# nyu-systems/Grendel-GS

Hardware: AMD Instinct MI355X
Metric: training iters/sec (fwd+bwd) (higher is better)
Workload: dtype f32

## Files before the change

### grendel-gs_amd/csrc/binning.hip

```cpp
#include "common.h"

#include <atomic>
#include <chrono>
#include <cstdlib>
#include <cstring>
#include <mutex>

#include "radix.h"
#ifndef GSR_EMIT_DECODE_BATCH
#define GSR_EMIT_DECODE_BATCH 2
#endif
#include "binning_persist.h"
#include "binning_rows.h"
#include "binning_host.h"

namespace {

__global__ void __launch_bounds__(SCAN_THREADS)
scan_gather_lookback_kernel(const uint32_t *__restrict__ src, int packed,
                            const uint32_t *__restrict__ idx, uint32_t *__restrict__ out, uint32_t *__restrict__ out2,
                            long long n, unsigned long long *__restrict__ state, uint32_t *__restrict__ ticket, int nb,
                            uint32_t *__restrict__ host_total, uint32_t seq,
                            const unsigned long long *__restrict__ early) {
    __shared__ uint32_t smem[4];
    __shared__ uint32_t s_bid;
    __shared__ unsigned long long s_excl;
    if (threadIdx.x == 0) s_bid = atomicAdd(ticket, 1u);
    __syncthreads();
    const uint32_t bid = s_bid;
    const int lane = threadIdx.x & 63, wave = threadIdx.x >> 6;
    const long long base = (long long)bid * SCAN_TILE + (long long)threadIdx.x * SCAN_ITEMS;
    uint32_t v[SCAN_ITEMS], v2[SCAN_ITEMS];
    uint32_t s = 0, s2 = 0;
#pragma unroll
    for (int k = 0; k < SCAN_ITEMS; k++) {
        const uint32_t x = (base + k < n) ? src[idx[base + k]] : 0u;
        v[k] = packed ? (x & TT_MASK) : x;
        v2[k] = packed ? (x >> TT_SHIFT) : 0u;
        s += v[k];
        s2 += v2[k];
    }
    uint32_t tot, tot2;
    const uint32_t local = block_exclusive_scan(s, smem, &tot);
    const uint32_t local2 = block_exclusive_scan(s2, smem, &tot2);
    const unsigned long long tot64 = (unsigned long long)tot | ((unsigned long long)tot2 << 31);
    if (wave == 0) {
        if (lane == 0) st_agent64(&state[bid], tot64 | (bid == 0 ? LB64_PRE : LB64_AGG));
        unsigned long long excl = 0;
        if (bid > 0) {
            long long top = (long long)bid - 1;
            while (true) {
                const long long j = top - lane;
                unsigned long long x = j >= 0 ? ld_agent64(&state[j]) : LB64_PRE;
// ... 369 lines not shown
                       tile_hist ? 1 : 0, sorted_ids, v.offsets, v.segoff, (long long)P,
                       reinterpret_cast<unsigned long long *>(v.ctrl + L.C.scan_state),
                       reinterpret_cast<uint32_t *>(v.ctrl + L.C.tickets), nbs, (uint32_t *)nullptr, seq, v.early);
    GSR_LAUNCH_CHECK();
    *ticket = seq;
    return 0;
}

int prepare_persistent(const PrepCall &c, const BinFrame &f, const BinHooks &h, BinDevice &d, uint32_t *ticket) {
    if (!(persist_effective_mode() & PERSIST_P) || g_tie_order.load(std::memory_order_relaxed) != 0) return 1;
    persist_caps(d);
    const int grid_p = lowered(h.grid_p, d.grid_p);
    long long nb = radix_blocks(c.P);
    int items = 4;
    if (nb > grid_p && (nb + 1) / 2 <= grid_p) {
        items = 8;
        nb = (nb + 1) / 2;
    }
    const int G = (int)(nb < grid_p ? nb : grid_p);
    if (G <= 0 || nb > (long long)G * h.max_tpw) return 1;
    const long long admit = persist_admit(d, c.stream);
    if (admit < 0) return 1;
    const int P = c.P;
    const PrepLayout L = prep_layout(P);
    const PrepViews v = views(L, c.prep);
    const PersistLayoutP PL = persist_layout_p(G);
    GSR_HIP(hipMemsetAsync(v.early, 0, (L.ctrl - L.early) + PL.zero_bytes, c.stream));
    uint32_t *host_total = nullptr;
    uint32_t seq = 0;
    const int rc = take_ticket(d, &host_total, &seq);
    if (rc) return rc;
    PrepPersistArgs a{};
    a.P = P; a.gx = f.gx; a.gy = f.gy;
    a.means2D = reinterpret_cast<const float2 *>(c.means2D);
    a.conic_opacity = reinterpret_cast<const float4 *>(c.conic_opacity);
    a.depths = c.depths; a.radii = c.radii; a.mask = c.compute_locally;
    a.tt = v.tt; a.kA = v.kA; a.vA = v.vA; a.kB = v.kB; a.vB = v.vB;
    a.offsets = v.offsets; a.segoff = v.segoff; a.rects = v.rects;
    a.tile_hist = f.yx ? v.thist : nullptr;
    a.cull = f.cull;
    a.hull_out = v.hull;
    a.early = v.early;
    a.zero16 = reinterpret_cast<uint4 *>(c.zero_ptr);
    a.zero16_n = c.zero_bytes / 16;
    a.sync = sync_view(v.ctrl + PL.sync, G);
    a.tstamp = timeline_buffer(h.timeline, 0, G);
    a.grp = at<uint32_t>(v.ctrl, PL.grp); a.cnt = at<uint32_t>(v.ctrl, PL.cnt);
    a.wtot = at<unsigned long long>(v.ctrl, PL.wtot); a.bins = at<uint32_t>(v.ctrl, PL.bins);
    a.depth_buckets = h.depth_buckets ? 1 : 0;
    a.host_total = host_total; a.seq = seq;
    a.done_word = d.done; a.done_seq = (uint32_t)admit;
    a.timeout_ticks = 5000000ull;
    a.force_abort = h.abort_p ? 1 : 0;
    if (items == 4) hipLaunchKernelGGL(bin_prepare_persist_kernel<4>, dim3(G), dim3(PP_THREADS), 0, c.stream, a);
    else hipLaunchKernelGGL(bin_prepare_persist_kernel<8>, dim3(G), dim3(PP_THREADS), 0, c.stream, a);
    GSR_LAUNCH_CHECK();
    *ticket = seq;
    return 0;
}

struct SortCall {
    BinFrame f;
    int P;
    const uint8_t *mask;
    PrepViews pv;
    int64_t D;
    void *scratch;
    uint32_t *point_list;
    int32_t *ranges;
    hipStream_t stream;
    bool bounded;
};

int launch_rows(const SortCall &s, const BinHooks &h, const BinDevice &d) {
    const BinFrame &f = s.f;
    const int P = s.P, gx = f.gx, gy = f.gy;
    const long long D = s.D;
    const RowsLayout R = rows_layout(D, gx, gy);
    auto u32 = [&s](size_t off) { return at<uint32_t>(s.scratch, off); };
    uint32_t *tickets = u32(R.tickets), *seg_key = u32(R.seg_key), *seg_gid = u32(R.seg_gid), *pairoff = u32(R.pairoff);
    uint32_t *tilebase = u32(R.tilebase);
    int32_t *tdiff = at<int32_t>(s.scratch, R.tdiff), *chunk_owner = at<int32_t>(s.scratch, R.chunk_owner);
    int cus = 256;
    (void)hipDeviceGetAttribute(&cus, hipDeviceAttributeMultiprocessorCount, (int)(&d - g_bin_devices));
    const uint32_t *thist = s.pv.thist, *segoff = s.pv.segoff, *offsets = s.pv.offsets;
    constexpr int TILE_B = 8 * ROWS_THREADS_B, TILE_D = 8 * ROWS_THREADS_D;
    auto tickets_of = [](long long tiles) { return (tiles + TICKET_TILES - 1) / TICKET_TILES; };
    const long long nbB = (D + TILE_B - 1) / TILE_B;
    const int fill_b = cus * 2, fill_d = cus * h.rows_fill_d;
    const int grid_b = (int)(tickets_of(nbB) < fill_b ? tickets_of(nbB) : fill_b);
    const long long nbs = (D + SEGSCAN_TILE - 1) / SEGSCAN_TILE;
    const int grid_c = (int)(tickets_of(nbs) < cus * 2 ? tickets_of(nbs) : cus * 2);
    const long long nbt = (D + TILE_D - 1) / TILE_D + gy;
    const int grid_d = (int)(tickets_of(nbt) < fill_d ? tickets_of(nbt) : fill_d);
    hipLaunchKernelGGL((seg_scatter_kernel<8, ROWS_THREADS_B>), dim3(grid_b), dim3(ROWS_THREADS_B), 0, s.stream, P, D,
                       f.ybits, s.pv.rects, s.pv.vA, offsets, segoff, thist + 2 * RADIX_DIGITS, u32(R.seg_state), tickets,
                       seg_key, seg_gid, s.bounded, s.ranges, 2 * gx * gy, s.pv.hull, tdiff,
                       RADIX_REPLICAS * gy * (gx + 1));
    hipLaunchKernelGGL(seg_scan_kernel, dim3(grid_c), dim3(SCAN_THREADS), 0, s.stream, P, D, gx, gy, offsets, segoff,
                       seg_key, pairoff, at<unsigned long long>(s.scratch, R.scan_state), tickets + 1, tdiff, thist,
                       chunk_owner, s.bounded);
    hipLaunchKernelGGL(tile_base_kernel, dim3(gy), dim3(GSR_ONE_DIM_BLOCK), 0, s.stream, P, D, gx, gy, offsets, thist,
                       tdiff, s.mask, tilebase, reinterpret_cast<int2 *>(s.ranges), s.bounded);
    hipLaunchKernelGGL((pair_scatter_kernel<8, ROWS_THREADS_D>), dim3(grid_d), dim3(ROWS_THREADS_D), 0, s.stream, P, D, gx,
                       gy, f.xbits, offsets, segoff, seg_key, seg_gid, pairoff, thist, tilebase, chunk_owner, u32(R.pair_state),
                       tickets + 2, s.point_list, s.bounded);
    GSR_LAUNCH_CHECK();
    return 0;
// ... 147 lines not shown
    if (!d->total_word) return GSR_EINVAL;
    uint32_t total = 0;
    rc = wait_total(reinterpret_cast<hipStream_t>(stream_), slot_of_ticket(*d, ticket), ticket, &total);
    if (rc) return rc;
    if (total == PAIRS_ABORTED) {
        PrepCall c = d->calls[ticket % TOTAL_SLOTS];
        if (!c.persistent) return GSR_EINVAL;
        c.persistent = false;
        uint32_t again = 0;
        rc = prepare_lookback(c, bin_frame(c.width, c.height), *d, &again);
        if (rc) return rc;
        rc = wait_total(c.stream, slot_of_ticket(*d, again), again, &total);
        if (rc) return rc;
        *num_rendered_host = (int64_t)total;
        return GSR_ERETRY;
    }
    *num_rendered_host = (int64_t)total;
    return 0;
}

extern "C" int gsr_bin_prepare(int P, int width, int height, const float *means2D, const float *depths,
                               const int32_t *radii, const float *conic_opacity, const uint8_t *compute_locally,
                               void *prep, size_t prep_bytes, int64_t *num_rendered_host, gsr_stream_t stream_) {
    if (!num_rendered_host) return GSR_EINVAL;
    *num_rendered_host = 0;
    uint32_t ticket = 0;
    const int rc = gsr_bin_prepare_async(P, width, height, means2D, depths, radii, conic_opacity, compute_locally, prep,
                                         prep_bytes, &ticket, stream_);
    if (rc) return rc;
    const int rw = gsr_bin_count_wait(ticket, num_rendered_host, stream_);
    return rw == GSR_ERETRY ? 0 : rw;
}

extern "C" int gsr_bin_sort(int P, int width, int height, const uint8_t *compute_locally, const void *prep,
                            int64_t D, void *scratch, size_t scratch_bytes, uint32_t *point_list, int32_t *ranges,
                            gsr_stream_t stream_) {
    return bin_sort_impl(P, width, height, compute_locally, prep, D, scratch, scratch_bytes, point_list, ranges,
                         reinterpret_cast<hipStream_t>(stream_), false);
}

extern "C" int gsr_bin_sort_bounded(int P, int width, int height, const uint8_t *compute_locally, const void *prep,
                                    int64_t capacity, void *scratch, size_t scratch_bytes, uint32_t *point_list,
                                    int32_t *ranges, gsr_stream_t stream_) {
    if (capacity <= 0) return GSR_EINVAL;
    return bin_sort_impl(P, width, height, compute_locally, prep, capacity, scratch, scratch_bytes, point_list, ranges,
                         reinterpret_cast<hipStream_t>(stream_), true);
}

extern "C" int gsr_bin_speculative_async(int P, int width, int height, const float *means2D, const float *depths,
                                         const int32_t *radii, const float *conic_opacity,
                                         const uint8_t *compute_locally, void *prep, size_t prep_bytes,
                                         int64_t capacity, void *scratch, size_t scratch_bytes, uint32_t *point_list,
                                         int32_t *ranges, uint32_t *ticket, int *sorted, gsr_stream_t stream_) {
    if (!ticket || !sorted) return GSR_EINVAL;
    *sorted = 0;
    if (P < 0 || width <= 0 || height <= 0) return GSR_EINVAL;
    *ticket = 0;
    if (P == 0) return 0;
    if (!means2D || !depths || !radii || !conic_opacity || !compute_locally || !prep) return GSR_EINVAL;
    if (P > RADIX_MAX_N) return GSR_EINVAL;
    if (prep_bytes < prep_bytes_needed(P)) return GSR_ENOSPACE;
    const BinFrame f = bin_frame(width, height);
    if (f.gx > 0xFFFF || f.gy > 0xFFFF) return GSR_EINVAL;
    BinDevice *d = nullptr;
    int rc = bin_device(&d);
    if (!rc) rc = persist_fault_check(*d);
    if (rc) return rc;
    const BinHooks h = read_hooks();
    hipStream_t stream = reinterpret_cast<hipStream_t>(stream_);
    const bool sort = capacity > 0 && scratch && point_list;
    const SortPlan p = sort ? plan_sort(f, capacity, scratch_bytes, true, h.rows_min) : SortPlan{GSR_EINVAL};
    PrepCall c{P, width, height, means2D, depths, radii, conic_opacity, compute_locally, prep, stream, true, nullptr, 0};
    if (!p.err) {
        c.zero_ptr = reinterpret_cast<char *>(scratch) + p.zero_off;
        c.zero_bytes = p.zero_bytes;
    }
    rc = prepare_persistent(c, f, h, *d, ticket);
    if (rc == 1) {
        c.persistent = false;
        rc = prepare_lookback(c, f, *d, ticket);
    }
    if (rc) return rc;
    d->calls[*ticket % TOTAL_SLOTS] = c;
    d->calls[*ticket % TOTAL_SLOTS].zero_ptr = nullptr;
    d->calls[*ticket % TOTAL_SLOTS].zero_bytes = 0;
    if (!sort) return 0;
    if (!ranges) return GSR_EINVAL;
    if (!f.yx) GSR_HIP(hipMemsetAsync(ranges, 0, sizeof(int32_t) * 2 * ((size_t)f.gx * f.gy + 1), stream));
    if (p.err) return p.err;
    rc = sort_run({f, P, compute_locally, views(prep_layout(P), prep), capacity, scratch, point_list, ranges, stream, true},
                  h, *d, p.form);
    if (rc) return rc;
    *sorted = 1;
    return 0;
}

extern "C" int gsr_bin_prepare_async(int P, int width, int height, const float *means2D, const float *depths,
                                     const int32_t *radii, const float *conic_opacity, const uint8_t *compute_locally,
                                     void *prep, size_t prep_bytes, uint32_t *ticket, gsr_stream_t stream_) {
    int sorted = 0;
    return gsr_bin_speculative_async(P, width, height, means2D, depths, radii, conic_opacity, compute_locally, prep,
                                     prep_bytes, 0, nullptr, 0, nullptr, nullptr, ticket, &sorted, stream_);
}

extern "C" int gsr_set_depth_tie_order(int mode) {
    if (mode != 0 && mode != 1) return GSR_EINVAL;
    g_tie_order.store(mode, std::memory_order_relaxed);
    return 0;
}

extern "C" int gsr_set_tile_cull(int mode) {
    if (mode < -1 || mode > 2) return GSR_EINVAL;
    g_tile_cull.store(mode, std::memory_order_relaxed);
    return 0;
}

extern "C" int gsr_set_bin_rowmajor(int mode) {
    if (mode < -1 || mode > 1) return GSR_EINVAL;
    g_rows_override.store(mode, std::memory_order_relaxed);
    return 0;
}

extern "C" int gsr_set_bin_persistent(int mode) {
    if (mode < -1 || mode > 3) return GSR_EINVAL;
    g_persist_override.store(mode, std::memory_order_relaxed);
    std::lock_guard<std::mutex> guard(g_bin_mutex);
    for (BinDevice &d : g_bin_devices) {
        if (!d.done) continue;
        d.solo_seen = reinterpret_cast<volatile uint32_t *>(d.done)[3];
        d.backoff = 0;
    }
    return 0;
}

extern "C" int gsr_bin_persist_status(uint32_t *out4) {
    if (!out4) return GSR_EINVAL;
    BinDevice *d = nullptr;
    const int rc = bin_device(&d);
    if (rc && rc != GSR_EINVAL) return rc;
    out4[0] = out4[1] = out4[2] = out4[3] = 0;
    if (rc || !d->done) return 0;
    const volatile uint32_t *w = d->done;
    out4[0] = w[0]; out4[1] = w[1]; out4[2] = w[2]; out4[3] = w[3];
    return 0;
}

// ... 24 lines not shown
```

### grendel-gs_amd/csrc/binning_host.h

```cpp
#pragma once

namespace {

enum { PERSIST_OFF = 0, PERSIST_P = 1, PERSIST_S = 2 };
constexpr long long PERSIST_SORT_MAX_PAIRS = 6ll << 20;
constexpr long long ROWS_MIN_PAIRS = 5ll << 20;

std::atomic<int> g_persist_override{-1};
std::atomic<int> g_rows_override{-1};
std::atomic<int> g_tile_cull{-1};
std::atomic<int> g_tie_order{0};

int persist_effective_mode() {
    const int o = g_persist_override.load(std::memory_order_relaxed);
    if (o >= 0) return o;
    static const int env_mode = [] {
        const char *e = getenv("GSR_BIN_PERSIST");
        if (!e || !*e || strcmp(e, "1") == 0) return PERSIST_P | PERSIST_S;
        if (strcmp(e, "p") == 0) return (int)PERSIST_P;
        if (strcmp(e, "s") == 0) return (int)PERSIST_S;
        return (int)PERSIST_OFF;
    }();
    return env_mode;
}
bool rows_switch_on() {
    const int mode = g_rows_override.load(std::memory_order_relaxed);
    if (mode >= 0) return mode == 1;
    static const bool env_on = [] {
        const char *e = getenv("GSR_BIN_ROWS");
        return !(e && *e == '0');
    }();
    return env_on;
}
int tile_cull_on(int tiles) {
    int mode = g_tile_cull.load(std::memory_order_relaxed);
    if (mode < 0) {
        static const int env_mode = [] {
            const char *e = getenv("GSR_TILE_CULL");
            if (!e || !*e || strcmp(e, "0") == 0) return 0;
            return strcmp(e, "auto") == 0 ? 2 : 1;
        }();
        mode = env_mode;
    }
    if (mode != 2) return mode;
    static const int min_tiles = [] {
        const char *e = getenv("GSR_TILE_CULL_TILES");
        const int v = e ? atoi(e) : 0;
        return v > 0 ? v : 16384;
    }();
    return tiles > min_tiles ? 1 : 0;
}

int lowered(int v, int dflt) { return v > 0 && v < dflt ? v : dflt; }
int env_int(const char *name) {
    const char *e = getenv(name);
    return e && *e ? atoi(e) : 0;
}
struct BinHooks {
    long long persist_maxd;
    long long rows_min;
    int rows_fill_d;
    int max_tpw;
    int owners;
    int sort_timeout_ms;
    int grid_p, grid_s;
    bool depth_buckets;
    bool abort_p, abort_s;
    bool timeline;
};
BinHooks read_hooks() {
    BinHooks h;
    const int maxd = env_int("GSR_BIN_PERSIST_MAXD");
    h.persist_maxd = maxd > 0 && maxd < 0x7fffffff ? maxd : PERSIST_SORT_MAX_PAIRS;
    const char *e = getenv("GSR_BIN_ROWS_MIN");
    const long long rows_min = e ? atoll(e) : 0;
    h.rows_min = rows_min > 0 ? rows_min : ROWS_MIN_PAIRS;
    h.rows_fill_d = lowered(env_int("GSR_ROWS_FILL_D"), 4);
    h.max_tpw = lowered(env_int("GSR_BIN_MAX_TPW"), PP_MAX_TPW + 1);
    if (h.max_tpw > PP_MAX_TPW) h.max_tpw = 1;
    h.owners = lowered(env_int("GSR_BIN_OWNERS"), PS_OWNERS);
    h.sort_timeout_ms = lowered(env_int("GSR_BIN_SORT_TIMEOUT_MS"), 250);
    h.grid_p = env_int("GSR_BIN_GRID_P");
    h.grid_s = env_int("GSR_BIN_GRID_S");
    e = getenv("GSR_BIN_DEPTH_SORT");
    h.depth_buckets = !(e && strcmp(e, "lsd") == 0);
    e = getenv("GSR_BIN_FORCE_ABORT");
    h.abort_p = e && strchr(e, 'p') != nullptr;
    h.abort_s = e && strchr(e, 's') != nullptr;
    e = getenv("GSR_BIN_TIMELINE");
    h.timeline = e && *e == '1';
    return h;
}

int bits_for(long long n) {
    int b = 1;
    while ((1ll << b) < n) b++;
    return b;
}
int tile_bits(int tiles) { return bits_for((long long)tiles + 1); }
struct BinFrame {
    int width, height, gx, gy, tiles;
    int xbits, ybits;
    bool yx;
    int cull;
};
BinFrame bin_frame(int width, int height) {
    BinFrame f;
    f.width = width; f.height = height;
    f.gx = (width + GSR_BLOCK_X - 1) / GSR_BLOCK_X;
    f.gy = (height + GSR_BLOCK_Y - 1) / GSR_BLOCK_Y;
    f.tiles = f.gx * f.gy;
    f.xbits = bits_for(f.gx); f.ybits = bits_for(f.gy);
    const char *e = getenv("GSR_BINNING");
    f.yx = !(e && strcmp(e, "generic") == 0) && f.gx <= RADIX_DIGITS && f.gy <= RADIX_DIGITS;
    f.cull = f.yx ? tile_cull_on(f.tiles) : 0;
    return f;
}

constexpr int PERSIST_MAX_GRID_P = 1024;
constexpr int PERSIST_MAX_GRID_S = 4096;
template <class T>
T *at(void *base, size_t off) { return reinterpret_cast<T *>(reinterpret_cast<char *>(base) + off); }
GridSync sync_view(void *sync, int G) {
    uint32_t *leaf = at<uint32_t>(sync, 0), *root = leaf + (size_t)((G + GB_FAN - 1) / GB_FAN) * GB_LEAF_STRIDE;
    return {leaf, root, root + GB_LEAF_STRIDE};
}
struct PersistLayoutP {
    size_t sync, grp, bins, cnt, wtot, zero_bytes, total;
};
PersistLayoutP persist_layout_p(int G) {
    PersistLayoutP L;
    const int ngroups = (G + GB_FAN - 1) / GB_FAN;
    size_t o = 0;
    L.sync = o; o += align_up(sizeof(uint32_t) * grid_sync_words(G));
    L.grp = o; o += align_up(sizeof(uint32_t) * (BK_PASS + 1) * (size_t)ngroups * RADIX_DIGITS);
    L.bins = o; o += align_up(sizeof(uint32_t) * (BK_BINS + 2));
    L.zero_bytes = o;
    L.cnt = o; o += align_up(sizeof(uint32_t) * (BK_PASS + 1) * (size_t)G * RADIX_DIGITS);
    L.wtot = o; o += align_up(sizeof(unsigned long long) * (size_t)G);
    L.total = o;
    return L;
}
struct PersistLayoutS {
// ... 97 lines not shown
    L.C = ctrl_layout(D, passes < 2 ? 2 : passes, false);
    const size_t need = persist_layout_s(persist_grid_bound(D, PERSIST_MAX_GRID_S)).total;
    o += L.C.total > need ? L.C.total : need;
    if (f.yx) {
        const size_t rows = rows_layout(D, f.gx, f.gy).total;
        if (rows > o) o = rows;
    }
    L.total = o;
    return L;
}
struct SortViews {
    uint32_t *kA, *vA, *kB, *vB, *ghist, *tickets, *state;
    char *ctrl;
};
SortViews views(const SortLayout &L, void *b) {
    return {at<uint32_t>(b, L.kA), at<uint32_t>(b, L.vA), at<uint32_t>(b, L.kB), at<uint32_t>(b, L.vB),
            at<uint32_t>(b, L.ctrl + L.C.ghist), at<uint32_t>(b, L.ctrl + L.C.tickets),
            at<uint32_t>(b, L.ctrl + L.C.radix_state), at<char>(b, L.ctrl)};
}

enum SortForm { SORT_ROWS, SORT_YX, SORT_GENERIC };
struct SortPlan {
    int err;
    SortForm form;
    size_t zero_off, zero_bytes;
};
SortPlan plan_sort(const BinFrame &f, int64_t D, size_t scratch_bytes, bool bounded, long long rows_min) {
    if (D > RADIX_MAX_N) return {GSR_EINVAL};
    const SortLayout S = sort_layout(f, D);
    if (scratch_bytes < S.total) return {GSR_ENOSPACE};
    if (bounded && !f.yx) return {GSR_EINVAL};
    if (f.yx && !f.cull && D >= rows_min && rows_switch_on()) {
        const RowsLayout R = rows_layout(D, f.gx, f.gy);
        return {0, SORT_ROWS, R.ctrl, R.ctrl_bytes};
    }
    if (!f.yx) return {0, SORT_GENERIC, S.ctrl, S.C.total};
    const size_t zp = persist_layout_s(persist_grid_bound(D, PERSIST_MAX_GRID_S)).zero_bytes;
    return {0, SORT_YX, S.ctrl, S.C.total > zp ? S.C.total : zp};
}

constexpr int TOTAL_SLOTS = 64, MAX_DEVICES = 64;

struct PrepCall {
    int P, width, height;
    const float *means2D, *depths;
    const int32_t *radii;
    const float *conic_opacity;
    const uint8_t *compute_locally;
    void *prep;
    hipStream_t stream;
    bool persistent;
    void *zero_ptr;
    size_t zero_bytes;
};

struct BinDevice {
    uint32_t *total_word;
    bool caps_init;
    int grid_p, grid_s;
    uint32_t *done;
    uint32_t faults_seen;
    uint32_t solo_seen;
    int backoff;
    bool faulted;
    uint32_t seq;
    hipStream_t stream;
    bool any;
    PrepCall calls[TOTAL_SLOTS];
};
std::mutex g_bin_mutex;
BinDevice g_bin_devices[MAX_DEVICES];
uint32_t g_ticket_seq = 0;

int bin_device(BinDevice **out) {
    int dev = 0;
    GSR_HIP(hipGetDevice(&dev));
    if (dev < 0 || dev >= MAX_DEVICES) return GSR_EINVAL;
    *out = &g_bin_devices[dev];
    return 0;
}

void persist_caps(BinDevice &d) {
    std::lock_guard<std::mutex> guard(g_bin_mutex);
    if (d.caps_init) return;
    d.caps_init = true;
    const int dev = (int)(&d - g_bin_devices);
    int cus = 0, per_p = 0, per_p8 = 0, per_s = 0;
    if (hipDeviceGetAttribute(&cus, hipDeviceAttributeMultiprocessorCount, dev) == hipSuccess && cus > 0 &&
        hipOccupancyMaxActiveBlocksPerMultiprocessor(&per_p, bin_prepare_persist_kernel<4>, PP_THREADS, 0) == hipSuccess &&
        hipOccupancyMaxActiveBlocksPerMultiprocessor(&per_p8, bin_prepare_persist_kernel<8>, PP_THREADS, 0) == hipSuccess &&
        hipOccupancyMaxActiveBlocksPerMultiprocessor(&per_s, bin_sort_persist_kernel, PS_THREADS, 0) == hipSuccess) {
        d.grid_p = (per_p >= 1 && per_p8 >= 1) ? (cus < PERSIST_MAX_GRID_P ? cus : PERSIST_MAX_GRID_P) : 0;
        const long long gs = (long long)cus * (per_s < 4 ? per_s : 4);
        d.grid_s = per_s >= 1 ? (int)(gs < PERSIST_MAX_GRID_S ? gs : PERSIST_MAX_GRID_S) : 0;
    }
    void *p = nullptr;
    if (hipHostMalloc(&p, 64, hipHostMallocDefault) == hipSuccess) {
        memset(p, 0, 64);
        d.done = reinterpret_cast<uint32_t *>(p);
    } else {
        d.grid_p = d.grid_s = 0;
    }
    (void)hipGetLastError();
}

int take_ticket(BinDevice &d, uint32_t **host, uint32_t *seq_out) {
    std::lock_guard<std::mutex> guard(g_bin_mutex);
    if (!d.total_word) {
        void *p = nullptr;
        GSR_HIP(hipHostMalloc(&p, sizeof(uint32_t) * 2 * TOTAL_SLOTS, hipHostMallocDefault));
        memset(p, 0, sizeof(uint32_t) * 2 * TOTAL_SLOTS);
        d.total_word = reinterpret_cast<uint32_t *>(p);
    }
    const uint32_t seq = ++g_ticket_seq ? g_ticket_seq : ++g_ticket_seq;
    *seq_out = seq;
    *host = d.total_word + 2 * (seq % TOTAL_SLOTS);
    return 0;
}
uint32_t *slot_of_ticket(const BinDevice &d, uint32_t seq) { return d.total_word + 2 * (seq % TOTAL_SLOTS); }
int wait_total(hipStream_t stream, uint32_t *host_total, uint32_t seq, uint32_t *total) {
    volatile uint32_t *w = host_total;
    const auto t0 = std::chrono::steady_clock::now();
    for (long spins = 0;; spins++) {
        if (w[1] == seq) {
            std::atomic_thread_fence(std::memory_order_acquire);
            *total = w[0];
            return 0;
        }
        if ((spins & 1023) == 1023 &&
            std::chrono::steady_clock::now() - t0 > std::chrono::milliseconds(2))
            break;
    }
    GSR_HIP(hipStreamSynchronize(stream));
    *total = w[0];
    return w[1] == seq ? 0 : GSR_EINVAL;
}

long long persist_admit(BinDevice &d, hipStream_t stream) {
    hipStreamCaptureStatus cs = hipStreamCaptureStatusNone;
    if (hipStreamIsCapturing(stream, &cs) == hipSuccess && cs != hipStreamCaptureStatusNone) return 0;
    (void)hipGetLastError();
    std::lock_guard<std::mutex> guard(g_bin_mutex);
    if (d.faulted) return -1;
    if (d.any && d.stream != stream) {
        const volatile uint32_t *done = reinterpret_cast<volatile uint32_t *>(d.done);
// ... 54 lines not shown
```

### grendel-gs_amd/csrc/binning_persist.h

```cpp
#pragma once

namespace {

constexpr int TT_SHIFT = 20;
constexpr uint32_t TT_MASK = (1u << TT_SHIFT) - 1u;
constexpr uint32_t GB_ABORT = 0x80000000u;
constexpr int GB_FAN = 32;
constexpr int GB_LEAF_STRIDE = 32;
constexpr uint32_t PAIRS_ABORTED = 0xFFFFFFFFu;

struct GridSync {
    uint32_t *leaf;
    uint32_t *root;
    uint32_t *flags;
};
__host__ __device__ inline size_t grid_sync_words(int G) {
    return (size_t)(2 * ((G + GB_FAN - 1) / GB_FAN) + 1) * GB_LEAF_STRIDE;
}

__device__ __forceinline__ bool grid_barrier_try_abort(const GridSync gs, uint32_t complete) {
    uint32_t r = __hip_atomic_load(gs.root, __ATOMIC_RELAXED, __HIP_MEMORY_SCOPE_AGENT);
    while (true) {
        if (r & GB_ABORT) return true;
        if (r == complete) return false;
        if (__hip_atomic_compare_exchange_strong(gs.root, &r, r | GB_ABORT, __ATOMIC_RELAXED, __ATOMIC_RELAXED,
                                                 __HIP_MEMORY_SCOPE_AGENT))
            return true;
    }
}
__device__ __forceinline__ bool grid_barrier(const GridSync gs, uint32_t G, uint32_t &epoch, uint64_t timeout_ticks,
                                             uint32_t *s_flag, bool force_abort = false) {
    asm volatile("s_waitcnt vmcnt(0)" ::: "memory");
    __syncthreads();
    if (threadIdx.x == 0) {
        epoch++;
        const uint32_t g = blockIdx.x / GB_FAN, ngroups = (G + GB_FAN - 1) / GB_FAN;
        const uint32_t gsz = min((uint32_t)GB_FAN, G - g * GB_FAN);
        const uint32_t complete = epoch * ngroups;
        if (force_abort && grid_barrier_try_abort(gs, complete))
            for (uint32_t k = 0; k < ngroups; k++) st_agent(&gs.flags[k * GB_LEAF_STRIDE], 0xFFFFFFFFu);
        const uint32_t old =
            __hip_atomic_fetch_add(&gs.leaf[g * GB_LEAF_STRIDE], 1u, __ATOMIC_RELAXED, __HIP_MEMORY_SCOPE_AGENT);
        if (old + 1u == epoch * gsz) {
            const uint32_t r = __hip_atomic_fetch_add(gs.root, 1u, __ATOMIC_RELAXED, __HIP_MEMORY_SCOPE_AGENT);
            if ((r & ~GB_ABORT) + 1u == complete)
                for (uint32_t k = 0; k < ngroups; k++)
                    st_agent(&gs.flags[k * GB_LEAF_STRIDE], (r & GB_ABORT) ? 0xFFFFFFFFu : epoch);
        }
        uint64_t t0 = __builtin_amdgcn_s_memrealtime();
        uint32_t f;
        while ((f = ld_agent(&gs.flags[g * GB_LEAF_STRIDE])) < epoch) {
            __builtin_amdgcn_s_sleep(1);
            if (__builtin_amdgcn_s_memrealtime() - t0 > timeout_ticks) {
                if (grid_barrier_try_abort(gs, complete)) {
                    for (uint32_t k = 0; k < ngroups; k++) st_agent(&gs.flags[k * GB_LEAF_STRIDE], 0xFFFFFFFFu);
                    f = 0xFFFFFFFFu;
                    break;
                }
// ... 67 lines not shown
    return (G + GB_FAN - 1) / GB_FAN <= 2 * Q && GB_FAN - 1 <= 8 * Q;
}
template <int THREADS>
__device__ __forceinline__ void counts_issue(const uint32_t *__restrict__ cnt, const uint32_t *__restrict__ grp,
                                             uint32_t G, uint32_t w, CountLoads &cl) {
    constexpr uint32_t Q = THREADS / RADIX_DIGITS;
    const uint32_t q = threadIdx.x / RADIX_DIGITS, d = threadIdx.x % RADIX_DIGITS;
    const uint32_t g = w / GB_FAN, ngroups = (G + GB_FAN - 1) / GB_FAN;
#pragma unroll
    for (int i = 0; i < 2; i++) {
        const uint32_t k = q + Q * i;
        cl.xg[i] = k < ngroups ? ld_agent(&grp[k * RADIX_DIGITS + d]) : 0u;
    }
#pragma unroll
    for (int i = 0; i < 8; i++) {
        const uint32_t k = g * GB_FAN + q + Q * i;
        cl.xc[i] = k < w ? ld_agent(&cnt[(size_t)k * RADIX_DIGITS + d]) : 0u;
    }
}
template <int THREADS>
__device__ __forceinline__ void counts_finish(const CountLoads &cl, uint32_t w, uint32_t *__restrict__ red,
                                              uint32_t &before, uint32_t &total) {
    constexpr uint32_t Q = THREADS / RADIX_DIGITS;
    const uint32_t q = threadIdx.x / RADIX_DIGITS;
    const uint32_t g = w / GB_FAN;
    uint32_t b = 0, t = 0;
#pragma unroll
    for (int i = 0; i < 2; i++) {
        t += cl.xg[i];
        if (q + Q * i < g) b += cl.xg[i];
    }
#pragma unroll
    for (int i = 0; i < 8; i++) b += cl.xc[i];
    red[threadIdx.x] = b;
    red[THREADS + threadIdx.x] = t;
    __syncthreads();
    before = total = 0;
    if (threadIdx.x < RADIX_DIGITS) {
#pragma unroll
        for (uint32_t i = 0; i < Q; i++) {
            before += red[i * RADIX_DIGITS + threadIdx.x];
            total += red[THREADS + i * RADIX_DIGITS + threadIdx.x];
        }
    }
    __syncthreads();
}

__device__ __forceinline__ void publish_counts(uint32_t *__restrict__ cnt, uint32_t *__restrict__ grp, uint32_t w,
                                               uint32_t d, uint32_t c) {
    st_agent(&cnt[(size_t)w * RADIX_DIGITS + d], c);
    if (c) __hip_atomic_fetch_add(&grp[(w / GB_FAN) * RADIX_DIGITS + d], c, __ATOMIC_RELAXED, __HIP_MEMORY_SCOPE_AGENT);
}

struct alignas(16) TileRect {
    uint32_t xs, ys;
    unsigned long long mask;
};
static_assert(sizeof(TileRect) == 16, "one 16-byte gather");

__device__ __forceinline__ unsigned long long gsr_full_mask(int n) { return n >= 64 ? ~0ull : ((1ull << n) - 1ull); }

__device__ __forceinline__ unsigned long long gsr_tile_mask(const float2 xy, const float4 co, int minx, int miny, int maxx,
                                                            int maxy) {
    const int w = maxx - minx, h = maxy - miny;
    if (w * h > 64) return ~0ull;
    const unsigned long long all = gsr_full_mask(w * h);
    const float A = co.x, B = co.y, C = co.z;
    const float det = A * C - B * B;
    if (!(A > 0.f && C > 0.f && det > 1e-6f * A * C) || !(co.w >= 1.0f / 255.0f)) return all;
    const float lim = (2.0f * 0.6931471805599453f) * __builtin_amdgcn_logf(255.0f * co.w) * 1.002f + 0.01f;
    const float rA = __builtin_amdgcn_rcpf(A), rC = __builtin_amdgcn_rcpf(C);
    const float dxs = __builtin_amdgcn_sqrtf(lim * C * __builtin_amdgcn_rcpf(det));
    const float dys = B * dxs * rC;
    unsigned long long mask = 0ull;
    for (int r = 0; r < h; r++) {
        const float t0 = (float)((miny + r) * GSR_BLOCK_Y) - xy.y, t1 = t0 + (float)(GSR_BLOCK_Y - 1);
        float dxR, dxL;
        bool emptyR = false, emptyL = false;
        if (-dys >= t0 && -dys <= t1) {
            dxR = dxs;
        } else {
            const float t = -dys < t0 ? t0 : t1;
            const float disc = lim * A - det * t * t;
            emptyR = disc < 0.f;
            dxR = (-B * t + __builtin_amdgcn_sqrtf(fmaxf(disc, 0.f))) * rA;
        }
        if (dys >= t0 && dys <= t1) {
            dxL = -dxs;
        } else {
            const float t = dys < t0 ? t0 : t1;
            const float disc = lim * A - det * t * t;
            emptyL = disc < 0.f;
            dxL = (-B * t - __builtin_amdgcn_sqrtf(fmaxf(disc, 0.f))) * rA;
        }
        int xa = 0, xb = w;
        if (emptyR && emptyL) continue;
        if (!emptyR && !emptyL) {
            dxR += 0.02f + 1e-4f * fabsf(dxR);
            dxL -= 0.02f + 1e-4f * fabsf(dxL);
            xa = minx;
            xb = maxx;
            gsr_clamp_span(xy.x + dxL, xy.x + dxR, xa, xb);
            xa -= minx;
            xb -= minx;
            if (xb <= xa) continue;
        }
        mask |= gsr_full_mask(xb - xa) << (r * w + xa);
    }
    return mask & all;
}

__device__ __forceinline__ uint32_t gsr_select_bit(unsigned long long m, uint32_t t) {
    uint32_t v = (uint32_t)m, base = 0;
    const uint32_t c = __popc(v);
    if (t >= c) { t -= c; v = (uint32_t)(m >> 32); base = 32; }
    const uint32_t c16 = __popc(v & 0xFFFFu);
    if (t >= c16) { t -= c16; v >>= 16; base += 16; }
    const uint32_t c8 = __popc(v & 0xFFu);
    if (t >= c8) { t -= c8; v >>= 8; base += 8; }
    const uint32_t c4 = __popc(v & 0xFu);
    if (t >= c4) { t -= c4; v >>= 4; base += 4; }
    const uint32_t c2 = __popc(v & 3u);
    if (t >= c2) { t -= c2; v >>= 2; base += 2; }
    if (t >= (v & 1u)) base += 1;
    return base;
}

__device__ __forceinline__ uint32_t gsr_rect_tiles(const float2 xy, const float4 co, int minx, int miny, int maxx, int maxy,
                                                   bool cull, int32_t (*dxy)[RADIX_DIGITS + 1], TileRect &out) {
    const int w = maxx - minx, h = maxy - miny;
    out.xs = (uint32_t)minx | ((uint32_t)maxx << 16);
    out.ys = (uint32_t)miny | ((uint32_t)maxy << 16);
    out.mask = ~0ull;
    if (!cull || w * h > 64) {
        if (dxy) {
            atomicAdd(&dxy[0][minx], h);
            atomicAdd(&dxy[0][maxx], -h);
            atomicAdd(&dxy[1][miny], w);
            atomicAdd(&dxy[1][maxy], -w);
            atomicAdd(&dxy[2][miny], 1);
            atomicAdd(&dxy[2][maxy], -1);
        }
        return (uint32_t)(w * h);
    }
    const unsigned long long mask = gsr_tile_mask(xy, co, minx, miny, maxx, maxy);
    out.mask = mask;
    if (dxy) {
        const unsigned long long rowm = gsr_full_mask(w);
        int prev_cnt = 0, run_a0 = 0, run_len = 0, run_mult = 0;
        for (int r = 0; r < h; r++) {
            unsigned long long bits = (mask >> (r * w)) & rowm;
            const int cnt = __popcll(bits);
            if (cnt != prev_cnt) atomicAdd(&dxy[1][miny + r], cnt - prev_cnt);
            prev_cnt = cnt;
            while (bits) {
                const int a0 = __ffsll((long long)bits) - 1;
                const unsigned long long rest = ~(bits >> a0);
                const int len = rest ? __ffsll((long long)rest) - 1 : 64 - a0;
                if (run_mult && a0 == run_a0 && len == run_len) {
                    run_mult++;
                } else {
                    if (run_mult) {
                        atomicAdd(&dxy[0][minx + run_a0], run_mult);
                        atomicAdd(&dxy[0][minx + run_a0 + run_len], -run_mult);
                    }
                    run_a0 = a0; run_len = len; run_mult = 1;
                }
                bits &= ~(gsr_full_mask(len) << a0);
            }
        }
        if (run_mult) {
            atomicAdd(&dxy[0][minx + run_a0], run_mult);
            atomicAdd(&dxy[0][minx + run_a0 + run_len], -run_mult);
        }
        if (prev_cnt) atomicAdd(&dxy[1][maxy], -prev_cnt);
    }
    return (uint32_t)__popcll(mask);
}

template <int ITEMS, int THREADS>
struct PersistSmem {
    uint16_t wtab[THREADS / 64][RADIX_DIGITS];
    uint32_t gbase[RADIX_DIGITS];
    unsigned long long scan64[THREADS / 64];
    uint32_t scan_tmp[THREADS / 64];
    uint32_t flag;
    uint32_t skey[ITEMS * THREADS], sval[ITEMS * THREADS];
};

template <int ITEMS, int THREADS>
__device__ __forceinline__ void clear_wtab(PersistSmem<ITEMS, THREADS> &sm) {
    uint32_t *p = reinterpret_cast<uint32_t *>(&sm.wtab[0][0]);
    for (int i = threadIdx.x; i < (THREADS / 64) * RADIX_DIGITS / 2; i += THREADS) p[i] = 0u;
}

// ... 145 lines not shown

__device__ __forceinline__ uint32_t clamp_pair_count(unsigned long long d) {
    return d >= 0xFFFFFFFEull ? 0xFFFFFFFEu : (uint32_t)d;
}
__device__ __forceinline__ void publish_pair_count(unsigned long long *early, unsigned long long mine, uint32_t nwg,
                                                   uint32_t *host_total, uint32_t seq) {
    __hip_atomic_fetch_add(early, mine, __ATOMIC_RELAXED, __HIP_MEMORY_SCOPE_AGENT);
    uint32_t *ticket = reinterpret_cast<uint32_t *>(early + 1);
    const uint32_t t = __hip_atomic_fetch_add(ticket, 1u, __ATOMIC_ACQ_REL, __HIP_MEMORY_SCOPE_AGENT);
    if (t + 1u == nwg && host_total) {
        const unsigned long long d = __hip_atomic_load(early, __ATOMIC_RELAXED, __HIP_MEMORY_SCOPE_AGENT);
        __hip_atomic_store(host_total, clamp_pair_count(d), __ATOMIC_RELAXED, __HIP_MEMORY_SCOPE_SYSTEM);
        __hip_atomic_store(host_total + 1, seq, __ATOMIC_RELEASE, __HIP_MEMORY_SCOPE_SYSTEM);
    }
}

#define GSR_TS(k)                                                                                       \
    do {                                                                                                \
        if (a.tstamp && threadIdx.x == 0) a.tstamp[(size_t)blockIdx.x * 32 + (k)] = __builtin_amdgcn_s_memrealtime(); \
    } while (0)

constexpr int PP_THREADS = 1024, PP_WAVES = PP_THREADS / 64;
constexpr int PP_MAX_TPW = 8;

struct PrepPersistArgs {
    int P, gx, gy;
    const float2 *means2D;
    const float *depths;
    const int32_t *radii;
    const float4 *conic_opacity;
    const uint8_t *mask;
    uint32_t *tt, *kA, *vA, *kB, *vB, *offsets;
    uint32_t *segoff;
    TileRect *rects;
    uint32_t *tile_hist;
    int cull;
    int32_t *hull_out;
    unsigned long long *early;
    uint4 *zero16;
    size_t zero16_n;
    GridSync sync;
    uint32_t *cnt;
    uint32_t *grp;
    unsigned long long *wtot;
    uint32_t *bins;
    int depth_buckets;
    uint32_t *host_total;
    uint32_t seq;
    uint32_t *done_word;
    uint32_t done_seq;
    uint64_t timeout_ticks;
    int force_abort;
    unsigned long long *tstamp;
};

struct PPExtra {
    int32_t dxy[3][RADIX_DIGITS + 1];
    int s_lo, s_hi;
};

constexpr int BK_ITEMS = 8;
constexpr int BK_CAP = BK_ITEMS * PP_THREADS;
constexpr int BK_PASS = RADIX_MAX_PASSES;
struct PPBucket {
    uint8_t map[BK_BINS];
    uint32_t lo, n, live;
};

template <int ITEMS, int THREADS>
__device__ __forceinline__ void bucket_scatter_write(PersistSmem<ITEMS, THREADS> &sm, long long n, const BucketDigit digit,
                                                     uint32_t first, uint32_t run, uint32_t *__restrict__ keys_out,
                                                     uint32_t *__restrict__ vals_out, uint32_t *__restrict__ ids_out) {
    constexpr int TILE = ITEMS * THREADS;
    if (threadIdx.x < RADIX_DIGITS) sm.gbase[threadIdx.x] = first - run;
    __syncthreads();
    const int count = n < TILE ? (int)n : TILE;
#pragma unroll
    for (int r = 0; r < ITEMS; r++) {
        const int i = r * THREADS + threadIdx.x;
        if (i < count) {
            const uint32_t k = sm.skey[i];
            const uint32_t dg = digit(k);
            const uint32_t dst = sm.gbase[dg] + (uint32_t)i;
            if (dg == BK_TAIL) {
                ids_out[dst] = sm.sval[i];
            } else {
                st_agent(&keys_out[dst], k);
                st_agent(&vals_out[dst], sm.sval[i]);
            }
        }
    }
    __syncthreads();
}

template <int THREADS>
__device__ __forceinline__ void bucket_sort_span(PersistSmem<BK_ITEMS, THREADS> &s, const uint32_t *__restrict__ kin,
                                                 const uint32_t *__restrict__ vin, uint32_t lo, uint32_t n,
                                                 uint32_t *__restrict__ red) {
    constexpr int WAVES = THREADS / 64;
    const int lane = threadIdx.x & 63, wave = threadIdx.x >> 6;
    const uint32_t wbase = (uint32_t)wave * (BK_ITEMS * 64);
    uint32_t key[BK_ITEMS], val[BK_ITEMS];
    uint32_t mn = 0xFFFFFFFFu, mx = 0u;
#pragma unroll
    for (int r = 0; r < BK_ITEMS; r++) {
        const uint32_t i = wbase + r * 64 + lane;
// ... 9 lines not shown
    }
#pragma unroll
    for (int d = 32; d >= 1; d >>= 1) {
        mn = min(mn, (uint32_t)__shfl_xor(mn, d, 64));
        mx = max(mx, (uint32_t)__shfl_xor(mx, d, 64));
    }
    if (lane == 0) {
        red[wave] = mn;
        red[WAVES + wave] = mx;
    }
    __syncthreads();
#pragma unroll
    for (int wv = 0; wv < WAVES; wv++) {
        mn = min(mn, red[wv]);
        mx = max(mx, red[WAVES + wv]);
    }
    const uint32_t diff = mx > mn ? mx - mn : 0u;
    const int nbits = diff ? 32 - __clz(diff) : 0;
#pragma unroll
    for (int r = 0; r < BK_ITEMS; r++) key[r] -= mn;
    if (nbits == 0) {
#pragma unroll
        for (int r = 0; r < BK_ITEMS; r++) {
            const uint32_t i = wbase + r * 64 + lane;
            if (i < n) s.sval[i] = val[r];
        }
        __syncthreads();
        return;
    }
    const int passes = (nbits + 7) / 8, pb = (nbits + passes - 1) / passes;
    for (int shift = 0; shift < nbits; shift += pb) {
        clear_wtab(s);
        __syncthreads();
        count_wave_digits(s, key, (long long)wbase, (long long)n, shift, (1u << pb) - 1u);
        __syncthreads();
        uint32_t tot, run;
        scatter_rank(s, key, val, 0ll, (long long)n, shift, pb, tot, run);
        __syncthreads();
        if (shift + pb < nbits) {
#pragma unroll
            for (int r = 0; r < BK_ITEMS; r++) {
                const uint32_t i = wbase + r * 64 + lane;
                if (i < n) {
                    key[r] = s.skey[i];
                    val[r] = s.sval[i];
                }
            }
            __syncthreads();
        }
    }
}


template <int PP_ITEMS>
__global__ void __launch_bounds__(PP_THREADS)
bin_prepare_persist_kernel(const PrepPersistArgs a) {
    constexpr int PP_TILE = PP_THREADS * PP_ITEMS;
    __shared__ PersistSmem<BK_ITEMS, PP_THREADS> sm8;
    PersistSmem<PP_ITEMS, PP_THREADS> &sm = *reinterpret_cast<PersistSmem<PP_ITEMS, PP_THREADS> *>(&sm8);
    __shared__ PPExtra ex;
    __shared__ PPBucket bk;
    __shared__ uint32_t red2[2 * PP_THREADS];
    const uint32_t G = gridDim.x, w = blockIdx.x;
    const int lane = threadIdx.x & 63, wave = threadIdx.x >> 6;
    const long long P = a.P;
    const long long nb = (P + PP_TILE - 1) / PP_TILE;
    const long long t0 = (long long)w * nb / G, t1 = (long long)(w + 1) * nb / G;
    const bool keep = (t1 - t0) == 1;
    const bool try_buckets = a.depth_buckets && nb == (long long)G && counts_fit_registers<PP_THREADS>(G);
    const uint32_t d = threadIdx.x;
    uint32_t epoch = 0;
    GSR_TS(0);
    uint32_t key[PP_ITEMS], val[PP_ITEMS];
    for (size_t i = (size_t)w * PP_THREADS + threadIdx.x; i < a.zero16_n; i += (size_t)G * PP_THREADS)
        a.zero16[i] = make_uint4(0u, 0u, 0u, 0u);

    if (threadIdx.x <= RADIX_DIGITS) ex.dxy[0][threadIdx.x] = ex.dxy[1][threadIdx.x] = ex.dxy[2][threadIdx.x] = 0;
    if (threadIdx.x == 0) { ex.s_lo = a.gy; ex.s_hi = 0; }
    clear_wtab(sm);
    __syncthreads();
    {
        const int total = a.gx * a.gy;
        const int per = (total + PP_THREADS - 1) / PP_THREADS;
        const int b0 = threadIdx.x * per, b1 = min(b0 + per, total);
        int first = 0x7fffffff, last = -1;
#pragma unroll 8
        for (int b = b0; b < b1; b++) {
            const int on = a.mask[b] != 0;
            first = min(first, on ? b : 0x7fffffff);
            last = max(last, on ? b : -1);
        }
        if (last >= 0) {
            atomicMin(&ex.s_lo, first / a.gx);
            atomicMax(&ex.s_hi, last / a.gx + 1);
        }
    }
    __syncthreads();
    const int hull0 = ex.s_lo, hull1 = ex.s_hi;
    if (w == 0 && threadIdx.x == 0) {
        a.hull_out[0] = hull1 > hull0 ? hull0 : 0;
        a.hull_out[1] = hull1 > hull0 ? hull1 : 0;
    }
    uint32_t mytot = 0;
    unsigned long long nsum = 0;
    uint32_t kmn = 0xFFFFFFFFu, kmx = 0u;
    for (long long t = t0; t < t1; t++) {
        const long long wbase = t * PP_TILE + (long long)wave * (PP_ITEMS * 64);
#pragma unroll
        for (int r0 = 0; r0 < PP_ITEMS; r0 += 4) {
        int rad[4];
        float2 xy[4];
        float4 co[4];
        float dep[4];
#pragma unroll
        for (int q4 = 0; q4 < 4; q4++) {
            const int r = r0 + q4;
            const long long i = wbase + r * 64 + lane;
            const long long ic = i < P ? i : P - 1;
            rad[q4] = a.radii[ic];
            xy[q4] = a.means2D[ic];
            co[q4] = a.conic_opacity[ic];
            dep[q4] = a.depths[ic];
        }
#pragma unroll
        for (int q4 = 0; q4 < 4; q4++) {
            const int r = r0 + q4;
            const long long i = wbase + r * 64 + lane;
            key[r] = 0xFFFFFFFFu;
            val[r] = (uint32_t)i;
            if (i < P) {
                uint32_t n = 0;
                TileRect rect{0u, 0u, 0ull};
                if (rad[q4] > 0) {
                    float exx, eyy;
                    if (gsr_alpha_extent(co[q4], exx, eyy)) {
                        int minx, miny, maxx, maxy;
                        gsr_get_rect(xy[q4].x, xy[q4].y, rad[q4], a.gx, a.gy, minx, miny, maxx, maxy);
                        miny = max(miny, hull0);
                        maxy = min(maxy, hull1);
                        gsr_narrow_span(xy[q4].x, exx, minx, maxx);
                        gsr_narrow_span(xy[q4].y, eyy, miny, maxy);
                        if (maxx > minx && maxy > miny)
                            n = gsr_rect_tiles(xy[q4], co[q4], minx, miny, maxx, maxy, a.cull != 0,
                                               a.tile_hist ? ex.dxy : nullptr, rect);
                    }
                }
                if (n) {
                    key[r] = __float_as_uint(dep[q4]);
                    kmn = min(kmn, key[r]);
                    kmx = max(kmx, key[r]);
                }
                nsum += n;
                st_agent(&a.tt[i], (a.tile_hist && n) ? (n | (((rect.ys >> 16) - (rect.ys & 0xFFFFu)) << TT_SHIFT)) : n);
                a.rects[i] = rect;
                if (!keep) {
                    st_agent(&a.kA[i], key[r]);
                    st_agent(&a.vA[i], val[r]);
                }
            }
        }
        }
        if (try_buckets) continue;
        count_wave_digits(sm, key, wbase, P, 0, 0xFFu);
        __syncthreads();
        if (d < RADIX_DIGITS) {
#pragma unroll
            for (int wv = 0; wv < PP_WAVES; wv++) mytot += sm.wtab[wv][d];
        }
        if (!keep) {
            __syncthreads();
            clear_wtab(sm);
            __syncthreads();
        }
    }
    if (!try_buckets && d < RADIX_DIGITS) publish_counts(a.cnt, a.grp, w, d, mytot);
    {
        nsum = wave_sum64_local(nsum);
        {
            const int ol = opaque_lane();
#pragma unroll
            for (int o = 32; o >= 1; o >>= 1) {
                kmn = min(kmn, xor_lane(kmn, ol, o));
                kmx = max(kmx, xor_lane(kmx, ol, o));
            }
        }
        __syncthreads();
        if (lane == 0) {
            sm.scan64[wave] = nsum;
            red2[wave] = kmn;
            red2[PP_WAVES + wave] = kmx;
        }
        __syncthreads();
        if (threadIdx.x == 0) {
            unsigned long long tot = 0;
            for (int wv = 0; wv < PP_WAVES; wv++) {
                tot += sm.scan64[wv];
                kmn = min(kmn, red2[wv]);
                kmx = max(kmx, red2[PP_WAVES + wv]);
            }
            if (tot) __hip_atomic_fetch_add(a.early, tot, __ATOMIC_RELAXED, __HIP_MEMORY_SCOPE_AGENT);
            if (try_buckets && kmn <= kmx) {
                __hip_atomic_fetch_max(&a.bins[BK_BINS], ~kmn, __ATOMIC_RELAXED, __HIP_MEMORY_SCOPE_AGENT);
                __hip_atomic_fetch_max(&a.bins[BK_BINS + 1], kmx, __ATOMIC_RELAXED, __HIP_MEMORY_SCOPE_AGENT);
            }
        }
    }
    if (a.tile_hist) {
        const uint32_t xcc = __builtin_amdgcn_s_getreg(20 | (3 << 11)) & 7u;
        for (int p = 0; p < 3; p++) {
            const uint32_t v = threadIdx.x < RADIX_DIGITS ? (uint32_t)ex.dxy[p][threadIdx.x] : 0u;
            uint32_t all;
            const uint32_t c = block_exclusive_scan_n<PP_WAVES>(v, sm.scan_tmp, &all) + v;
            if (threadIdx.x < RADIX_DIGITS && c)
                __hip_atomic_fetch_add(&a.tile_hist[(xcc * RADIX_MAX_PASSES + p) * RADIX_DIGITS + threadIdx.x], c,
                                       __ATOMIC_RELAXED, __HIP_MEMORY_SCOPE_WORKGROUP);
        }
    }
    GSR_TS(1);
    if (!grid_barrier(a.sync, G, epoch, a.timeout_ticks, &sm.flag, a.force_abort != 0)) {
        if (threadIdx.x == 0) {
            a.offsets[P] = PAIRS_ABORTED;
            __hip_atomic_store(a.host_total, PAIRS_ABORTED, __ATOMIC_RELAXED, __HIP_MEMORY_SCOPE_SYSTEM);
            __hip_atomic_store(a.host_total + 1, a.seq, __ATOMIC_RELEASE, __HIP_MEMORY_SCOPE_SYSTEM);
            if (a.done_seq) __hip_atomic_store(a.done_word, a.done_seq, __ATOMIC_RELEASE, __HIP_MEMORY_SCOPE_SYSTEM);
        }
        return;
    }
    GSR_TS(2);
    if (w == 0 && threadIdx.x == 0) {
        const unsigned long long dsum = __hip_atomic_load(a.early, __ATOMIC_RELAXED, __HIP_MEMORY_SCOPE_AGENT);
        __hip_atomic_store(a.host_total, clamp_pair_count(dsum), __ATOMIC_RELAXED, __HIP_MEMORY_SCOPE_SYSTEM);
        __hip_atomic_store(a.host_total + 1, a.seq, __ATOMIC_RELEASE, __HIP_MEMORY_SCOPE_SYSTEM);
    }
    const uint64_t forever = 100000000ull;
    const uint32_t ngroups = (G + GB_FAN - 1) / GB_FAN;
    if (try_buckets) {
        static_assert(BK_BINS == 4 * PP_THREADS, "four bins per thread");
        const long long wbase0 = t0 * PP_TILE + (long long)wave * (PP_ITEMS * 64);
        const uint32_t kmin = ~ld_agent(&a.bins[BK_BINS]), kmax = ld_agent(&a.bins[BK_BINS + 1]);
        const uint32_t NB = min(G, BK_TAIL);
        bool buckets = kmin <= kmax && kmax != 0xFFFFFFFFu;
        if (buckets) {
            const uint32_t range = kmax - kmin;
            const int sh = max((range ? 32 - __clz(range) : 0) - BK_BIN_BITS, 0);
            const BucketDigit digit{bk.map, kmin, sh};
            uint32_t *const lbin = sm8.skey;
            for (int i = threadIdx.x; i < BK_BINS; i += PP_THREADS) lbin[i] = 0u;
            __syncthreads();
#pragma unroll
            for (int r = 0; r < PP_ITEMS; r++)
                if (key[r] != 0xFFFFFFFFu) atomicAdd(&lbin[(key[r] - kmin) >> sh], 1u);
            __syncthreads();
            for (int i = threadIdx.x; i < BK_BINS; i += PP_THREADS) {
                const uint32_t c = lbin[i];
                if (c) __hip_atomic_fetch_add(&a.bins[i], c, __ATOMIC_RELAXED, __HIP_MEMORY_SCOPE_AGENT);
            }
            GSR_TS(21);
            if (!grid_barrier(a.sync, G, epoch, forever, &sm.flag)) { barrier_fault(a.done_word, 0x200u + epoch); return; }
            GSR_TS(22);
            {
                uint32_t c4[4], s4 = 0, live;
#pragma unroll
                for (int k = 0; k < 4; k++) {
                    c4[k] = ld_agent(&a.bins[threadIdx.x * 4 + k]);
                    s4 += c4[k];
                }
                uint32_t start = block_exclusive_scan_n<PP_WAVES>(s4, sm.scan_tmp, &live);
#pragma unroll
                for (int k = 0; k < 4; k++) {
                    bk.map[threadIdx.x * 4 + k] = (uint8_t)(start * NB / live);
                    start += c4[k];
                }
            }
            __syncthreads();
            count_wave_digits(sm, key, wbase0, P, digit);
            __syncthreads();
            if (d < RADIX_DIGITS) {
                mytot = 0;
#pragma unroll
                for (int wv = 0; wv < PP_WAVES; wv++) mytot += sm.wtab[wv][d];
                publish_counts(a.cnt + (size_t)BK_PASS * G * RADIX_DIGITS, a.grp + (size_t)BK_PASS * ngroups * RADIX_DIGITS, w,
                               d, mytot);
            }
            GSR_TS(23);
            if (!grid_barrier(a.sync, G, epoch, forever, &sm.flag)) { barrier_fault(a.done_word, 0x200u + epoch); return; }
            GSR_TS(24);
            uint32_t tot, run, before, total, all;
            counts_before<PP_THREADS>(a.cnt + (size_t)BK_PASS * G * RADIX_DIGITS,
                                      a.grp + (size_t)BK_PASS * ngroups * RADIX_DIGITS, G, w,
                                      reinterpret_cast<uint32_t *>(red2), before, total);
            if (__syncthreads_or(d < BK_TAIL && total > (uint32_t)BK_CAP)) {
                buckets = false;
            } else {
                scatter_rank(sm, key, val, t0 * PP_TILE, P, digit, 8, tot, run);
                const uint32_t dstart = block_exclusive_scan_n<PP_WAVES>(total, sm.scan_tmp, &all);
                if (d == w) {
                    bk.lo = dstart;
                    bk.n = w < NB ? total : 0u;
                }
                if (d == BK_TAIL) bk.live = dstart;
                bucket_scatter_write(sm, P - t0 * PP_TILE, digit, dstart + before, run, a.kB, a.vB, a.vA);
            }
        }
        if (buckets) {
            GSR_TS(25);
            if (!grid_barrier(a.sync, G, epoch, forever, &sm.flag)) { barrier_fault(a.done_word, 0x200u + epoch); return; }
            GSR_TS(26);
            const uint32_t lo = bk.lo, n = bk.n, live = bk.live;
            bucket_sort_span<PP_THREADS>(sm8, a.kB, a.vB, lo, n, reinterpret_cast<uint32_t *>(red2));
#pragma unroll
            for (int r = 0; r < BK_ITEMS; r++) {
                const uint32_t i = r * PP_THREADS + threadIdx.x;
// ... 618 lines not shown
```

### grendel-gs_amd/csrc/build.py

```python
import os
import subprocess
import sys
from concurrent.futures import ThreadPoolExecutor

HERE = os.path.dirname(os.path.abspath(__file__))
ROOT = os.path.dirname(HERE)
OUT_DIR = os.path.join(ROOT, "diff_gaussian_rasterization")
SO = os.path.join(OUT_DIR, "libgsraster.so")
UNITS = ["preprocess", "binning", "composite", "contrib", "invdepth", "features", "absgrad", "loss", "bilagrid", "metrics", "optim", "activations", "filter3d", "knn", "compact", "mcmc", "exchange", "api"]
HEADERS = [os.path.join(HERE, "common.h"), os.path.join(HERE, "composite_math.h"), os.path.join(HERE, "radix.h"), os.path.join(HERE, "binning_persist.h"), os.path.join(HERE, "binning_rows.h"), os.path.join(HERE, "binning_host.h"),
           os.path.join(os.path.dirname(ROOT), "include", "gsraster.h")]
FLAGS = ["--offload-arch=gfx950", "-O3", "-std=c++17", "-fPIC", "-munsafe-fp-atomics", "-Wall",
         "-Wno-unused-function"]


def _hipcc():
    for c in (os.environ.get("HIPCC"), "/opt/rocm/bin/hipcc", "hipcc"):
        if c and (os.path.isabs(c) and os.path.exists(c) or not os.path.isabs(c)):
            return c
    return "hipcc"


def _stale(target, deps):
    if not os.path.exists(target):
        return True
    t = os.path.getmtime(target)
    return any(os.path.getmtime(d) > t for d in deps if os.path.exists(d))


def build(force=False, verbose=False):
    units = [u for u in UNITS if os.path.exists(os.path.join(HERE, u + ".hip"))]
    hipcc = _hipcc()
    extra = os.environ.get("GSR_DEFINES", "").split()
    if extra:
        force = True

    def compile_one(u):
        src, obj = os.path.join(HERE, u + ".hip"), os.path.join(HERE, u + ".o")
        if force or _stale(obj, [src] + HEADERS):
            cmd = [hipcc] + FLAGS + extra + ["-c", src, "-o", obj]
            if verbose:
                print(" ".join(cmd), flush=True)
            r = subprocess.run(cmd, capture_output=True, text=True)
            if r.returncode != 0:
                raise RuntimeError(f"hipcc failed on {u}.hip:\n{r.stdout}\n{r.stderr}")
            if verbose and r.stderr.strip():
                print(r.stderr, file=sys.stderr)
        return obj

    with ThreadPoolExecutor(max_workers=len(units)) as ex:
        objs = list(ex.map(compile_one, units))
    if force or _stale(SO, objs):
        cmd = [hipcc, "--offload-arch=gfx950", "-shared", "-fPIC"] + objs + ["-o", SO]
        if verbose:
            print(" ".join(cmd), flush=True)
        r = subprocess.run(cmd, capture_output=True, text=True)
        if r.returncode != 0:
            raise RuntimeError(f"link failed:\n{r.stdout}\n{r.stderr}")
    return SO


if __name__ == "__main__":
    print(build(force="--force" in sys.argv, verbose=True))
# ... 1 lines not shown
```

### grendel-gs_amd/csrc/common.h

```cpp
#pragma once
#include <hip/hip_runtime.h>
#include <stdint.h>

#include "../../include/gsraster.h"

#define GSR_WAVE 64

#define GSR_LAUNCH_CHECK()                         \
    do {                                           \
        hipError_t e__ = hipGetLastError();        \
        if (e__ != hipSuccess) return (int)e__;    \
    } while (0)

#define GSR_HIP(expr)                              \
    do {                                           \
        hipError_t e__ = (expr);                   \
        if (e__ != hipSuccess) return (int)e__;    \
    } while (0)

static inline int gsr_div_up(long long a, long long b) { return (int)((a + b - 1) / b); }

__device__ __forceinline__ int gsr_xcd_span_of_block(int b, int nwg) {
#ifdef GSR_NO_XCD_MAP
    return b;
#else
    const int xcd = b & 7, q = nwg >> 3, r = nwg & 7;
    return (xcd < r ? xcd * (q + 1) : r * (q + 1) + (xcd - r) * q) + (b >> 3);
#endif
}

__device__ __forceinline__ int gsr_xcd_span_of_block_band(int b, int nwg, int first, int hull) {
#ifdef GSR_NO_XCD_MAP
    return b;
#else
    const int xcd = b & 7, j = b >> 3;
    const int hl = (hull - xcd + 7) >> 3;
    const int hs = xcd * (hull >> 3) + min(xcd, hull & 7);
    if (j < hl) return first + hs + j;
    const int ts = xcd * (nwg >> 3) + min(xcd, nwg & 7);
    const int n = (ts - hs) + (j - hl);
    return n < first ? n : n + hull;
#endif
}

__device__ __forceinline__ void gsr_get_rect(float px, float py, int radius, int gx, int gy, int &minx, int &miny,
                                             int &maxx, int &maxy) {
    const float r = (float)radius;
    minx = min(gx, max(0, (int)((px - r) / GSR_BLOCK_X)));
    miny = min(gy, max(0, (int)((py - r) / GSR_BLOCK_Y)));
    maxx = min(gx, max(0, (int)((px + r + (GSR_BLOCK_X - 1)) / GSR_BLOCK_X)));
    maxy = min(gy, max(0, (int)((py + r + (GSR_BLOCK_Y - 1)) / GSR_BLOCK_Y)));
}

__device__ __forceinline__ bool gsr_alpha_extent(const float4 co, float &ex, float &ey) {
    ex = ey = 1e30f;
    if (!(co.w >= 1.0f / 255.0f)) return false;
    const float tau = __logf(255.0f * co.w);
    const float det = co.x * co.z - co.y * co.y;
    if (det > 0.f && tau >= 0.f) {
        const float s = 2.0f * tau / det;
        ex = sqrtf(s * co.z) * 1.01f + 0.5f;
        ey = sqrtf(s * co.x) * 1.01f + 0.5f;
    }
    return true;
}

__device__ __forceinline__ void gsr_clamp_span(float left, float right, int &lo, int &hi) {
    if (left != left || right != right) return;
    const float flo = (float)lo, fhi = (float)hi;
    const float a = ceilf((left - (float)(GSR_BLOCK_X - 1)) * (1.0f / GSR_BLOCK_X));
    const float b = floorf(right * (1.0f / GSR_BLOCK_X)) + 1.0f;
    lo = (int)fminf(fmaxf(a, flo), fhi);
    hi = (int)fminf(fmaxf(b, flo), fhi);
}
static_assert(GSR_BLOCK_X == GSR_BLOCK_Y, "gsr_clamp_span serves both axes");
__device__ __forceinline__ void gsr_narrow_span(float c, float e, int &lo, int &hi) {
    if (e < 1e30f) gsr_clamp_span(c - e, c + e, lo, hi);
}

__device__ __forceinline__ float gsr_edge_min_q(float a, float b, float c, float rc, float u, float v0, float v1) {
    const float vs = fminf(v1, fmaxf(v0, -b * u * rc));
    return a * u * u + (2.0f * b * u + c * vs) * vs;
}
__device__ __forceinline__ bool gsr_can_touch_box(const float2 xy, const float4 co, float x0, float y0, float x1,
                                                  float y1) {
    if (!(co.w >= 1.0f / 255.0f)) return false;
    const float lim = (2.0f * 0.6931471805599453f) * __builtin_amdgcn_logf(255.0f * co.w) * 1.002f + 0.01f;
    const float l = x0 - xy.x, r = x1 - xy.x, t = y0 - xy.y, bt = y1 - xy.y;
    if (l <= 0.f && r >= 0.f && t <= 0.f && bt >= 0.f) return true;
    if (!(co.x > 0.f && co.z > 0.f)) return true;
    const float rcz = __builtin_amdgcn_rcpf(co.z), rcx = __builtin_amdgcn_rcpf(co.x);
    float q = gsr_edge_min_q(co.x, co.y, co.z, rcz, l, t, bt);
    q = fminf(q, gsr_edge_min_q(co.x, co.y, co.z, rcz, r, t, bt));
    q = fminf(q, gsr_edge_min_q(co.z, co.y, co.x, rcx, t, l, r));
    q = fminf(q, gsr_edge_min_q(co.z, co.y, co.x, rcx, bt, l, r));
    return !(q > lim);
}

__device__ __forceinline__ void gsr_adam1(float &p, float g, float &m, float &v, float lr_c, float b1, float b2,
                                          float omb1, float omb2, float inv_sqrt_bc2, float eps) {
    m = __builtin_fmaf(b1, m, __fmul_rn(omb1, g));
    v = __builtin_fmaf(b2, v, __fmul_rn(__fmul_rn(omb2, g), g));
    const float denom = __builtin_fmaf(__fsqrt_rn(v), inv_sqrt_bc2, eps);
    p = __builtin_fmaf(-lr_c, __fdiv_rn(m, denom), p);
}

int gsr_launch_preprocess_forward(int P, int D, int M, const float *means3D, const float *scales, float scale_modifier,
                                  const float *rotations, const float *shs, const float *shs_rest,
                                  const float *opacities,
                                  const float *viewmatrix, const float *projmatrix, const float *campos, int W, int H,
                                  float tanfovx, float tanfovy, float *means2D, float *depths, int32_t *radii,
                                  float *cov3D, float *conic_opacity, float *rgb, uint8_t *clamped, int aa,
                                  hipStream_t stream);
int gsr_launch_preprocess_backward(int P, int D, int M, const float *means3D, const float *scales,
                                   float scale_modifier, const float *rotations, const float *shs,
// ... 60 lines not shown
```

### grendel-gs_amd/csrc/preprocess.hip

```cpp
#include "common.h"

#include <atomic>
#include <initializer_list>
#include <type_traits>

#pragma clang fp contract(off)

namespace {

__constant__ const float SH_C0 = 0.28209479177387814f;
__constant__ const float SH_C1 = 0.4886025119029199f;
__constant__ const float SH_C2[5] = {1.0925484305920792f, -1.0925484305920792f, 0.31539156525252005f,
                                     -1.0925484305920792f, 0.5462742152960396f};
__constant__ const float SH_C3[7] = {-0.5900435899266435f, 2.890611442640554f, -0.4570457994644658f,
                                     0.3731763325901154f, -0.4570457994644658f, 1.445305721320277f,
                                     -0.5900435899266435f};

struct Cam {
    float v[16];
    float p[16];
    float c[3];
};

__device__ __forceinline__ Cam load_cam(const float *__restrict__ view, const float *__restrict__ proj,
                                        const float *__restrict__ campos) {
    Cam cam;
#pragma unroll
    for (int i = 0; i < 16; i++) {
        cam.v[i] = view[i];
        cam.p[i] = proj[i];
    }
    cam.c[0] = campos[0];
    cam.c[1] = campos[1];
    cam.c[2] = campos[2];
    return cam;
}

__device__ __forceinline__ void quat_to_R(const float4 q, float R[3][3]) {
    const float r = q.x, x = q.y, y = q.z, z = q.w;
    R[0][0] = 1.f - 2.f * (y * y + z * z);
    R[0][1] = 2.f * (x * y - r * z);
    R[0][2] = 2.f * (x * z + r * y);
    R[1][0] = 2.f * (x * y + r * z);
    R[1][1] = 1.f - 2.f * (x * x + z * z);
    R[1][2] = 2.f * (y * z - r * x);
    R[2][0] = 2.f * (x * z - r * y);
    R[2][1] = 2.f * (y * z + r * x);
    R[2][2] = 1.f - 2.f * (x * x + y * y);
}

__device__ __forceinline__ void compute_T(const float t[3], const float *v, float fx, float fy, float tanfovx,
                                          float tanfovy, float T[2][3], float tc[3], bool &xin, bool &yin) {
    const float limx = 1.3f * tanfovx, limy = 1.3f * tanfovy;
// ... 999 lines not shown
    if (i < P)
        preprocess_backward_body<DEG, true, true, AA>(in, sp, sg, i, s_rest + threadIdx.x * REST_W,
                                                      s_rest + threadIdx.x * REST_W, 16, scale_modifier, f_dc, view,
                                                      proj, campos, W, H, tanfovx, tanfovy, nullptr, nullptr, nullptr,
                                                      nullptr, nullptr);
    __syncthreads();
    rest_adam_out(s_rest, f_rest, ad, P);
    __syncthreads();
    k11_adam_small_lds(s_rest, ad, P, i, xyz, scaling, rotation, f_dc, opacity, sp, sg);
}
template <int DEG, bool AA>
__global__ void __launch_bounds__(K11_BLOCK, K11_WAVES_PER_EU)
preprocess_backward_adam_kernel(int P, float *__restrict__ xyz, float *__restrict__ scaling, float scale_modifier,
                                float *__restrict__ rotation, float *__restrict__ f_dc, float *__restrict__ f_rest,
                                float *__restrict__ opacity, const float *__restrict__ view,
                                const float *__restrict__ proj, const float *__restrict__ campos, int W, int H,
                                float tanfovx, float tanfovy, const int32_t *__restrict__ radii,
                                const float *__restrict__ cov3D, const uint8_t *__restrict__ clamped,
                                const float *__restrict__ dL_dmeans2D, const float *__restrict__ dL_dconic_opacity,
                                const float *__restrict__ dL_drgb, int gstride, const K11Adam ad_in) {
    preprocess_backward_adam_body<DEG, AA>(P, xyz, scaling, scale_modifier, rotation, f_dc, f_rest, opacity, view, proj,
                                           campos, W, H, tanfovx, tanfovy, radii, cov3D, clamped, dL_dmeans2D,
                                           dL_dconic_opacity, dL_drgb, gstride, GradNone{}, ad_in);
}
template <int DEG, bool AA>
__global__ void __launch_bounds__(K11_BLOCK, K11_WAVES_PER_EU)
preprocess_backward_adam_sums_kernel(int P, float *__restrict__ xyz, float *__restrict__ scaling, float scale_modifier,
                                     float *__restrict__ rotation, float *__restrict__ f_dc,
                                     float *__restrict__ f_rest, float *__restrict__ opacity,
                                     const float *__restrict__ view, const float *__restrict__ proj,
                                     const float *__restrict__ campos, int W, int H, float tanfovx, float tanfovy,
                                     const int32_t *__restrict__ radii, const float *__restrict__ cov3D,
                                     const uint8_t *__restrict__ clamped, const GradSums sums, const K11Adam ad_in) {
    preprocess_backward_adam_body<DEG, AA>(P, xyz, scaling, scale_modifier, rotation, f_dc, f_rest, opacity, view, proj,
                                           campos, W, H, tanfovx, tanfovy, radii, cov3D, clamped, nullptr, nullptr,
                                           nullptr, 0, sums, ad_in);
}

constexpr int CAM_STRIDE = 40;

__device__ __forceinline__ Cam load_cam_packed(const float *__restrict__ c) {
    Cam cam;
#pragma unroll
    for (int i = 0; i < 16; i++) {
        cam.v[i] = c[i];
        cam.p[i] = c[16 + i];
    }
    cam.c[0] = c[32];
    cam.c[1] = c[33];
    cam.c[2] = c[34];
    return cam;
}

template <int DEG, bool AA>
__global__ void __launch_bounds__(GSR_ONE_DIM_BLOCK)
preprocess_forward_batched_kernel(int P, int B, int M, const float *__restrict__ xyz, const float *__restrict__ scaling,
                                  float scale_modifier, const float *__restrict__ rotation,
                                  const float *__restrict__ f_dc, const float *__restrict__ f_rest,
                                  const float *__restrict__ opacity, const float *__restrict__ cams, int W, int H,
                                  float2 *__restrict__ means2D, float *__restrict__ depths,
                                  int32_t *__restrict__ radii, float *__restrict__ cov3D,
                                  float4 *__restrict__ conic_opacity, float *__restrict__ rgb,
                                  uint8_t *__restrict__ clamped) {
    const int i = blockIdx.x * blockDim.x + threadIdx.x;
    constexpr int NC = (DEG + 1) * (DEG + 1);
    if (i >= P) return;
    const int gx = (W + GSR_BLOCK_X - 1) / GSR_BLOCK_X, gy = (H + GSR_BLOCK_Y - 1) / GSR_BLOCK_Y;
    const float p[3] = {xyz[3 * (size_t)i], xyz[3 * (size_t)i + 1], xyz[3 * (size_t)i + 2]};
    float qnr, qn;
    const float4 q = quat_normalize(*reinterpret_cast<const float4 *>(rotation + 4 * (size_t)i), qnr, qn);
    const float s[3] = {scale_modifier * expf(scaling[3 * (size_t)i]), scale_modifier * expf(scaling[3 * (size_t)i + 1]),
                        scale_modifier * expf(scaling[3 * (size_t)i + 2])};
    const float op = sigmoidf(opacity[i]);
    float S[3][3];
    cov3d_from_scale_rot(q, s, S);
    cov3D[6 * (size_t)i + 0] = S[0][0]; cov3D[6 * (size_t)i + 1] = S[0][1]; cov3D[6 * (size_t)i + 2] = S[0][2];
    cov3D[6 * (size_t)i + 3] = S[1][1]; cov3D[6 * (size_t)i + 4] = S[1][2]; cov3D[6 * (size_t)i + 5] = S[2][2];
    float shl[NC * 3];
    shl[0] = f_dc[3 * (size_t)i];
    shl[1] = f_dc[3 * (size_t)i + 1];
    shl[2] = f_dc[3 * (size_t)i + 2];
    {
        const float *rp = f_rest + (size_t)i * (M - 1) * 3;
#pragma unroll
        for (int k = 3; k < NC * 3; k++) shl[k] = rp[k - 3];
    }
    for (int bc = 0; bc < B; bc++) {
        const float *cp = cams + (size_t)bc * CAM_STRIDE;
        const Cam cam = load_cam_packed(cp);
        const float tanfovx = cp[35], tanfovy = cp[36];
        const float fx = W / (2.0f * tanfovx), fy = H / (2.0f * tanfovy);
        int radius = 0;
        float2 xy = make_float2(0.f, 0.f);
        float depth = 0.f;
        float4 co = make_float4(0.f, 0.f, 0.f, 0.f);
        float col[3] = {0.f, 0.f, 0.f};
        bool cl[3] = {false, false, false};
        float t[3];
        view_transform(cam.v, p, t);
        do {
            if (t[2] <= 0.2f) break;
            Geom2D g;
            if (!project_geometry<AA>(cam, tanfovx, tanfovy, fx, fy, W, H, gx, gy, p, t, S, g)) break;
            shade<DEG>(cam.c, p, shl, col, cl);
            radius = g.rad;
            xy = g.xy;
            depth = t[2];
            co = make_float4(g.conic[0], g.conic[1], g.conic[2], AA ? op * g.rho : op);
        } while (false);
        const size_t o = (size_t)bc * P + i;
        radii[o] = radius;
        means2D[o] = xy;
        depths[o] = depth;
        conic_opacity[o] = co;
#pragma unroll
        for (int k = 0; k < 3; k++) {
            rgb[3 * o + k] = col[k];
            clamped[3 * o + k] = cl[k] ? 1 : 0;
        }
    }
}

#ifndef GSR_K11_CAMQ
#define GSR_K11_CAMQ 2
#endif
constexpr int K11_CAMQ = GSR_K11_CAMQ;
#ifndef GSR_K11B_WAVES
#define GSR_K11B_WAVES 2
#endif
constexpr int K11B_WAVES_PER_EU = GSR_K11B_WAVES;
struct K11CamSH {
    int32_t rad;
    float grgb[3];
    uint8_t cl[3];
};
struct K11CamGeo {
    int32_t rad;
    float4 gco;
    float2 g2;
};
__device__ __forceinline__ K11CamSH k11_cam_load_sh(size_t o, const int32_t *__restrict__ radii,
                                                    const uint8_t *__restrict__ clamped,
                                                    const float *__restrict__ dL_drgb, int gstride) {
    K11CamSH c;
    c.rad = radii[o];
#pragma unroll
    for (int e = 0; e < 3; e++) {
        c.grgb[e] = dL_drgb[(gstride ? gstride : 3) * o + e];
        c.cl[e] = clamped[3 * o + e];
    }
    return c;
}
__device__ __forceinline__ K11CamGeo k11_cam_load_geo(size_t o, const int32_t *__restrict__ radii,
                                                      const float *__restrict__ dL_dmeans2D,
                                                      const float *__restrict__ dL_dconic_opacity, int gstride) {
    K11CamGeo c;
    c.rad = radii[o];
    c.gco = grad_ld4(dL_dconic_opacity, o, gstride);
    c.g2 = grad_ld2(dL_dmeans2D, o, gstride);
    return c;
}
__device__ __forceinline__ K11CamSH k11_cam_load_sh_sums(size_t o, bool live, const uint8_t *__restrict__ clamped,
                                                         const double *__restrict__ a) {
    K11CamSH c;
    c.rad = live ? 1 : 0;
#pragma unroll
    for (int e = 0; e < 3; e++) {
        c.grgb[e] = 0.f;
        c.cl[e] = 0;
    }
    if (live) {
#pragma unroll
        for (int e = 0; e < 3; e++) {
// ... 700 lines not shown
#undef GSR_FWD
    GSR_LAUNCH_CHECK();
    return 0;
}

int gsr_launch_preprocess_backward(int P, int D, int M, const float *means3D, const float *scales,
                                   float scale_modifier, const float *rotations, const float *shs,
                                   const float *shs_rest, const float *opacities_raw, const float *viewmatrix, const float *projmatrix, const float *campos, int W,
                                   int H, float tanfovx, float tanfovy, const int32_t *radii, const float *cov3D,
                                   const uint8_t *clamped, const float *dL_dmeans2D, const float *dL_dconic_opacity,
                                   const float *dL_drgb, int grad_row_stride, float *dL_dmeans3D, float *dL_dscales, float *dL_drotations,
                                   float *dL_dshs, float *dL_dshs_rest, float *dL_dopacities, int aa,
                                   hipStream_t stream) {
    if (P == 0) return 0;
    const dim3 grid(gsr_div_up(P, K11_BLOCK)), block(K11_BLOCK);
#define GSR_BWD(RAWF)                                                                                              \
    GSR_DISPATCH_DEG_AA(D, aa, hipLaunchKernelGGL((preprocess_backward_kernel<DEG, RAWF, AA>), grid, block, 0,     \
                                           stream, P, M,                                                           \
                                           means3D, scales, scale_modifier, rotations, shs, shs_rest,              \
                                           opacities_raw, viewmatrix, projmatrix, campos, W, H, tanfovx, tanfovy,  \
                                           radii, cov3D, clamped, dL_dmeans2D, dL_dconic_opacity, dL_drgb,           \
                                           grad_row_stride,                                                          \
                                           dL_dmeans3D, dL_dscales, reinterpret_cast<float4 *>(dL_drotations),     \
                                           dL_dshs, dL_dshs_rest, dL_dopacities))
    if (shs_rest) { GSR_BWD(true); } else { GSR_BWD(false); }
#undef GSR_BWD
    GSR_LAUNCH_CHECK();
    return 0;
}

int gsr_launch_local2j(int P, int W, int H, int ws, const float *means2D, const int32_t *radii, const int32_t *div,
                       uint8_t *out, hipStream_t stream) {
    if (P == 0) return 0;
    hipLaunchKernelGGL(local2j_kernel, dim3(gsr_div_up(P, GSR_ONE_DIM_BLOCK)), dim3(GSR_ONE_DIM_BLOCK), 0, stream, P,
                       W, H, ws, reinterpret_cast<const float2 *>(means2D), radii, div, out);
    GSR_LAUNCH_CHECK();
    return 0;
}

extern "C" int gsr_preprocess_forward_raw_batched(int P, int B, int sh_degree, int sh_coeffs, const float *xyz,
                                                  const float *scaling, float scale_modifier, const float *rotation,
                                                  const float *features_dc, const float *features_rest,
                                                  const float *opacity, const float *cams, int width, int height,
                                                  float *means2D, float *depths, int32_t *radii, float *cov3D,
                                                  float *conic_opacity, float *rgb, uint8_t *clamped,
                                                  gsr_stream_t stream) {
    if (P < 0 || B < 1 || sh_degree < 0 || sh_degree > 3 || sh_coeffs < 2 ||
        sh_coeffs < (sh_degree + 1) * (sh_degree + 1) || width <= 0 || height <= 0)
        return GSR_EINVAL;
    if (P == 0) return 0;
    if (!xyz || !scaling || !rotation || !features_dc || !features_rest || !opacity || !cams || !means2D || !depths ||
        !radii || !cov3D || !conic_opacity || !rgb || !clamped)
        return GSR_EINVAL;
    const dim3 grid(gsr_div_up(P, GSR_ONE_DIM_BLOCK)), block(GSR_ONE_DIM_BLOCK);
    GSR_DISPATCH_DEG_AA(sh_degree, gsr_antialiasing_mode(),
                     hipLaunchKernelGGL((preprocess_forward_batched_kernel<DEG, AA>), grid, block, 0,
                                        reinterpret_cast<hipStream_t>(stream), P, B, sh_coeffs, xyz, scaling,
                                        scale_modifier, rotation, features_dc, features_rest, opacity, cams, width,
                                        height, reinterpret_cast<float2 *>(means2D), depths, radii, cov3D,
                                        reinterpret_cast<float4 *>(conic_opacity), rgb, clamped));
    GSR_LAUNCH_CHECK();
    return 0;
}

extern "C" int gsr_preprocess_backward_raw_batched(int P, int B, int sh_degree, int sh_coeffs, const float *xyz,
                                                   const float *scaling, float scale_modifier, const float *rotation,
                                                   const float *features_dc, const float *features_rest,
                                                   const float *opacity, const float *cams, int width, int height,
                                                   const int32_t *radii, const float *cov3D, const uint8_t *clamped,
                                                   const float *dL_dmeans2D, const float *dL_dconic_opacity,
                                                   const float *dL_drgb, int grad_row_stride, float *dL_dxyz, float *dL_dscaling,
                                                   float *dL_drotation, float *dL_dfeatures_dc,
                                                   float *dL_dfeatures_rest, float *dL_dopacity, gsr_stream_t stream) {
    if (P < 0 || B < 1 || sh_degree < 0 || sh_degree > 3 || sh_coeffs < 2 ||
        sh_coeffs < (sh_degree + 1) * (sh_degree + 1) || width <= 0 || height <= 0)
        return GSR_EINVAL;
    if (P == 0) return 0;
    if (!xyz || !scaling || !rotation || !features_dc || !features_rest || !opacity || !cams || !radii || !cov3D ||
        !clamped || !dL_dmeans2D || !dL_dconic_opacity || !dL_drgb || !dL_dxyz || !dL_dscaling || !dL_drotation ||
        !dL_dfeatures_dc || !dL_dfeatures_rest || !dL_dopacity)
        return GSR_EINVAL;
    const dim3 grid(gsr_div_up(P, K11_BLOCK)), block(K11_BLOCK);
    GSR_DISPATCH_DEG_AA(sh_degree, gsr_antialiasing_mode(),
                     hipLaunchKernelGGL((preprocess_backward_batched_kernel<DEG, AA>), grid, block, 0,
                                        reinterpret_cast<hipStream_t>(stream), P, B, sh_coeffs, xyz, scaling,
                                        scale_modifier, rotation, features_dc, features_rest, opacity, cams, width,
                                        height, radii, cov3D, clamped, dL_dmeans2D, dL_dconic_opacity, dL_drgb,
                                        grad_row_stride, dL_dxyz,
                                        dL_dscaling, reinterpret_cast<float4 *>(dL_drotation), dL_dfeatures_dc,
                                        dL_dfeatures_rest, dL_dopacity));
    GSR_LAUNCH_CHECK();
    return 0;
}

static bool k11_adam_fill(K11Adam &ad, std::initializer_list<const void *> device_arrays, float *const *exp_avgs,
                          float *const *exp_avg_sqs, const double *lrs, const double *beta1s, const double *beta2s,
                          const double *epss, const int64_t *steps, float grad_scale, const float *dyn_dev,
                          const uint32_t *skip_flag_dev) {
    for (const void *a : device_arrays)
        if (!a) return true;
    if (!exp_avgs || !exp_avg_sqs || !beta1s || !beta2s || !epss || (!dyn_dev && (!lrs || !steps))) return true;
    ad.dyn = dyn_dev;
    ad.skip = skip_flag_dev;
    ad.grad_scale = grad_scale;
    for (int t = 0; t < 6; t++) {
        if (!exp_avgs[t] || !exp_avg_sqs[t] || (!dyn_dev && steps[t] < 1)) return true;
        const double bc1 = dyn_dev ? 1.0 : 1.0 - pow(beta1s[t], (double)steps[t]);
        const double bc2 = dyn_dev ? 1.0 : 1.0 - pow(beta2s[t], (double)steps[t]);
        ad.m[t] = exp_avgs[t];
        ad.v[t] = exp_avg_sqs[t];
        ad.lr_c[t] = dyn_dev ? 0.f : (float)(lrs[t] / bc1);
        ad.b1[t] = (float)beta1s[t];
        ad.b2[t] = (float)beta2s[t];
        ad.omb1[t] = (float)(1.0 - beta1s[t]);
        ad.omb2[t] = (float)(1.0 - beta2s[t]);
        ad.inv_sqrt_bc2[t] = (float)(1.0 / sqrt(bc2));
// ... 202 lines not shown
```

### grendel-gs_amd/diff_gaussian_rasterization/__init__.py

```python
import contextlib
import ctypes
import os
from typing import NamedTuple

import torch
import torch.nn as nn
import torch.utils._pytree

from . import _lib
from ._lib import check, lib

__all__ = ["GaussianRasterizationSettings", "GaussianRasterizer", "_C", "load_image_tiles_by_pos",
           "merge_image_tiles_by_pos", "set_timing_mode", "fused_l1_ssim_band", "fused_band_loss", "fused_band_loss_exposure", "fused_activations", "pack_camera",
           "preprocess_gaussians_raw_batched", "knn_mean_dist2", "group_rows", "gather_rows", "densify_plan", "densify_move", "exchange_need",
           "exchange_count", "exchange_pack", "exchange_pack_slab", "exchange_unpack", "zeros_async", "scatter_add_rows", "absgrad_rows", "densify_stats",
           "set_tie_order", "scatter_rows", "local_pixels", "GraphCapture", "capturing", "image_metrics", "metrics_from_sums",
           "bilagrid_slice", "bilagrid_tv"]

BLOCK_X, BLOCK_Y, ONE_DIM_BLOCK_SIZE = 16, 16, 256

_TIMING_MODE = "auto"
_last_backward_ms = 0.0


# ... 684 lines not shown
                cache = {}
            need = int(lib.gsr_sparse_step_workspace_bytes(P))
            ws = cache.get("sparse_ws")
            if ws is None or ws[0] != P or ws[1].device != xyz.device or ws[1].numel() * 8 < need:
                ws = (P, torch.empty((need + 7) // 8, dtype=torch.int64, device=xyz.device),
                      torch.zeros(1, dtype=torch.int32, device=xyz.device))
                cache["sparse_ws"] = ws
                cache["num_active"] = ws[2]
            name, timed = "gsr_preprocess_backward_adam_raw_batched_sparse", "preprocess_backward_adam_sparse"
            args += [dyn, flag, _ptr(ws[1]), ws[1].numel() * 8, None, _ptr(ws[2])]
        elif cap_ctx is not None:
            name, timed = "gsr_preprocess_backward_adam_raw_batched_dyn", None
            args += [tf, dyn, flag]
        else:
            name, timed = "gsr_preprocess_backward_adam_raw_batched", "preprocess_backward_adam"
            args += [tf]
        _lib_antialiasing(_meta_aa(self.meta))
        with _on(xyz.device), (kernel_timer.range(timed, N=P, B=B, M=M) if cap_ctx is None else _NULL_RANGE):
            check(getattr(lib, name)(*args, _stream()), name)


def _launch_k11(params, cams, radii, cov3D, clamped, g_means2D, g_conic_opacity, g_rgb, gstride, meta, tanfov0,
                cuda_args_list):
    xyz, scaling, rotation, f_dc, f_rest, opacity = params
    deg, smod, W, H, M = meta[:5]
    _lib_antialiasing(_meta_aa(meta))
    P, B = xyz.shape[0], cams.shape[0]
    dev = xyz.device
    d_xyz = torch.empty((P, 3), dtype=torch.float32, device=dev)
    d_scaling = torch.empty((P, 3), dtype=torch.float32, device=dev)
    d_rot = torch.empty((P, 4), dtype=torch.float32, device=dev)
    d_dc = torch.empty((P, 1, 3), dtype=torch.float32, device=dev)
    d_rest = torch.empty((P, M - 1, 3), dtype=torch.float32, device=dev)
    d_opac = torch.empty((P, 1), dtype=torch.float32, device=dev)
    with _on(dev), kernel_timer.range("preprocess_backward", N=P, B=B, M=M), \
            zhx_range(cuda_args_list, "b20 preprocess time"):
        if B == 1 and tanfov0 is not None:
            base = cams.data_ptr()
            check(lib.gsr_preprocess_backward_raw(
                P, deg, M, _ptr(xyz), _ptr(scaling), smod, _ptr(rotation), _ptr(f_dc), _ptr(f_rest),
                _ptr(opacity), ctypes.c_void_p(base), ctypes.c_void_p(base + 64), ctypes.c_void_p(base + 128), W,
                H, float(tanfov0[0]), float(tanfov0[1]), _ptr(radii), _ptr(cov3D), _ptr(clamped),
                _ptr(g_means2D), _ptr(g_conic_opacity), _ptr(g_rgb), gstride, _ptr(d_xyz), _ptr(d_scaling),
                _ptr(d_rot), _ptr(d_dc), _ptr(d_rest), _ptr(d_opac), _stream()), "gsr_preprocess_backward_raw")
        else:
            check(lib.gsr_preprocess_backward_raw_batched(
                P, B, deg, M, _ptr(xyz), _ptr(scaling), smod, _ptr(rotation), _ptr(f_dc), _ptr(f_rest),
                _ptr(opacity), _ptr(cams), W, H, _ptr(radii), _ptr(cov3D), _ptr(clamped), _ptr(g_means2D),
                _ptr(g_conic_opacity), _ptr(g_rgb), gstride, _ptr(d_xyz), _ptr(d_scaling), _ptr(d_rot),
                _ptr(d_dc), _ptr(d_rest), _ptr(d_opac), _stream()), "gsr_preprocess_backward_raw_batched")
    return d_xyz, d_scaling, d_rot, d_dc, d_rest, d_opac


class _PreprocessGaussiansRawBatched(torch.autograd.Function):

    @staticmethod
    def forward(ctx, xyz, scaling, rotation, features_dc, features_rest, opacity, cams, sh_degree, scale_modifier,
                width, height, tanfov0, cuda_args_list=None):
        xyz, scaling, rotation = _f32c(xyz, "xyz"), _f32c(scaling, "scaling"), _f32c(rotation, "rotation")
        features_dc, features_rest = _f32c(features_dc, "features_dc"), _f32c(features_rest, "features_rest")
        opacity, cams = _f32c(opacity, "opacity"), _f32c(cams, "cams")
        ctx.tanfov0 = tanfov0
        ctx.cuda_args_list = cuda_args_list
        ctx.set_materialize_grads(False)
        P, B = xyz.shape[0], cams.shape[0]
        if cams.dim() != 2 or cams.shape[1] != 40:
            raise ValueError("cams must be [B, 40]")
        M = 1 + features_rest.shape[1]
        dev = xyz.device
        aa = _ANTIALIASING[0]
        if aa and ctx.needs_input_grad[6]:
            _refuse_camera_grad_under_antialiasing("preprocess_gaussians_raw_batched")
        _lib_antialiasing(aa)
        means2D = torch.empty((B, P, 2), dtype=torch.float32, device=dev)
        depths = torch.empty((B, P), dtype=torch.float32, device=dev)
        radii = torch.empty((B, P), dtype=torch.int32, device=dev)
        cov3D = torch.empty((P, 6), dtype=torch.float32, device=dev)
        conic_opacity = torch.empty((B, P, 4), dtype=torch.float32, device=dev)
        rgb = torch.empty((B, P, 3), dtype=torch.float32, device=dev)
        clamped = torch.empty((B, P, 3), dtype=torch.uint8, device=dev)
        with _on(dev), kernel_timer.range("preprocess_forward", N=P, B=B, M=M), \
                zhx_range(cuda_args_list, "10 preprocess time"):
            check(lib.gsr_preprocess_forward_raw_batched(
                P, B, int(sh_degree), M, _ptr(xyz), _ptr(scaling), float(scale_modifier), _ptr(rotation),
                _ptr(features_dc), _ptr(features_rest), _ptr(opacity), _ptr(cams), int(width), int(height),
                _ptr(means2D), _ptr(depths), _ptr(radii), _ptr(cov3D), _ptr(conic_opacity), _ptr(rgb), _ptr(clamped),
                _stream()), "gsr_preprocess_forward_raw_batched")
        ctx.meta = (int(sh_degree), float(scale_modifier), int(width), int(height), M, aa)
        ctx.m2_ptr = means2D.data_ptr()
        ctx.save_for_backward(xyz, scaling, rotation, features_dc, features_rest, opacity, cams, radii, cov3D, clamped)
        outs = []
        for k in range(B):
            outs += [means2D[k], rgb[k], conic_opacity[k], radii[k], depths[k]]
        ctx.mark_non_differentiable(*[o for i, o in enumerate(outs) if i % 5 >= 3])
        return tuple(outs)

    @staticmethod
    def backward(ctx, *grads):
        xyz, scaling, rotation, f_dc, f_rest, opacity, cams, radii, cov3D, clamped = ctx.saved_tensors
        deg, smod, W, H, M = ctx.meta[:5]
        P, B = xyz.shape[0], cams.shape[0]
        dev = xyz.device

        def assemble(col, cols):
            gs = [grads[5 * k + col] for k in range(B)]
            if B == 1:
                return torch.zeros((1, P, cols), dtype=torch.float32, device=dev) if gs[0] is None \
                    else gs[0].float().contiguous()
            if all(g is not None and g.dtype == torch.float32 and g.is_contiguous() for g in gs):
                base, step = gs[0]._base, P * cols * 4
                if base is not None and all(g._base is base and g.data_ptr() == gs[0].data_ptr() + k * step
                                            for k, g in enumerate(gs)):
                    return gs[0]
            out = torch.zeros((B, P, cols), dtype=torch.float32, device=dev)
            for k, g in enumerate(gs):
                if g is not None:
                    out[k].copy_(g)
            return out

        params = (xyz, scaling, rotation, f_dc, f_rest, opacity)
        entries = [_take_deferred(ctx.m2_ptr + 8 * k * P, grads[5 * k]) if _DEFERRED else None for k in range(B)]
        deferred = None
        if any(e is not None for e in entries):
            for k, e in enumerate(entries):
                for col, (off, cols) in enumerate(((0, 2), (2, 3), (5, 4))):
                    g = grads[5 * k + col]
                    if e is not None and g is not None and not e.is_view(g, off, cols):
                        raise RuntimeError(
                            "diff_gaussian_rasterization: the rounding of a view's gradient record was deferred, but "
                            "another gradient reached means2D / rgb / conic_opacity of that view and autograd has added "
                            "it to the unrounded record; call set_deferred_rounding(False) for such a graph")
            whole = all(e is not None and all(grads[5 * k + c] is not None for c in range(3))
                        for k, e in enumerate(entries))
            sink = deferred_backward_sink()
            if whole and not ctx.needs_input_grad[6] and B <= DEFER_MAX_CAMERAS and M == 16 and sink is not None and \
                    not getattr(sink, "sparse", False) and deferred_rounding() and sink.accepts(params):
                deferred = entries
            else:
                for e in entries:
                    if e is not None:
# ... 121 lines not shown


class GraphCapture:

    def __init__(self, flag, dyn, pair_slack=1.25):
        self.flag, self.dyn, self.pair_slack = flag, dyn, pair_slack
        self.pairs = []
        self.counts = None
        self.slab_caps_dev = None
        self._words, self._next = torch.zeros((8192,), dtype=torch.int32).pin_memory(), 0
        self.stamp_ring = None
        self.stamps = []

    def stamp(self, kind, tag):
        if self.stamp_ring is None:
            return
        ring, slots, per = self.stamp_ring
        idx = len(self.stamps)
        if idx >= per:
            raise RuntimeError("graph capture: out of timestamp words")
        check(lib.gsr_stamp(self.dyn.data_ptr() + 48, ring.data_ptr(), slots, per, idx, _stream()), "gsr_stamp")
        self.stamps.append((kind, tag))

    def take_pinned(self, n):
        if self._next + n > self._words.numel():
            raise RuntimeError("graph capture: out of pinned result words")
        v = self._words[self._next:self._next + n]
        self._next += n
        return v

    def pair_capacity(self, dev):
        idx = dev.index if dev.index is not None else torch.cuda.current_device()
        seen = max([v for (d, _s), v in _MAX_PAIRS.items() if d == idx], default=0)
        if seen <= 0:
            raise RuntimeError("graph capture: no eager iteration has sorted a view on this device yet")
        return _bucket(4 * int(seen * self.pair_slack + 4096)) // 4


def capturing():
    return _CAPTURE[0]


_DEBUG_RANGES = []


def _debug_overlap(name, t):
    a0, a1 = t.data_ptr(), t.data_ptr() + t.numel() * t.element_size()
    for n, p, sz in _DEBUG_RANGES:
        if a0 < p + sz and p < a1:
            print(f"[graphed] OVERLAP: eager {name} [{a0:#x}, {a1:#x}) with captured {n} [{p:#x}, {p + sz:#x})",
                  file=__import__("sys").stderr, flush=True)


def _bin_workspaces(means2D, depths, radii, conic_opacity, compute_locally, width, height):
    P = means2D.shape[0]
    dev = means2D.device
    tiles = ((width + BLOCK_X - 1) // BLOCK_X) * ((height + BLOCK_Y - 1) // BLOCK_Y)
    ranges = torch.empty((tiles + 1, 2), dtype=torch.int32, device=dev)[:tiles]
    prep_bytes = lib.gsr_bin_prepare_bytes(P, width, height)
    prep = torch.empty((max(prep_bytes, 4),), dtype=torch.uint8, device=dev)
    args = (P, width, height, _ptr(means2D), _ptr(depths), _ptr(radii), _ptr(conic_opacity), _ptr(compute_locally),
            _ptr(prep), prep_bytes)
    return P, dev, ranges, prep, args


def _bin_gaussians_captured(cap_ctx, means2D, depths, radii, conic_opacity, compute_locally, width, height):
    P, dev, ranges, prep, args = _bin_workspaces(means2D, depths, radii, conic_opacity, compute_locally, width, height)
    stream = _stream()
    ticket = ctypes.c_uint32(0)
    check(lib.gsr_bin_prepare_async(*args, ctypes.byref(ticket), stream), "gsr_bin_prepare_async")
    cap = cap_ctx.pair_capacity(dev)
    if int(lib.gsr_bin_sort_capacity(P, lib.gsr_bin_sort_bytes(P, cap, width, height), width, height)) < cap:
        raise RuntimeError("graph capture: frames above 256 x 256 tiles have no bounded tile sort")
    sort_bytes = lib.gsr_bin_sort_bytes(P, cap, width, height)
    scratch = torch.empty((max(sort_bytes, 4),), dtype=torch.uint8, device=dev)
    point_list = torch.empty((cap,), dtype=torch.int32, device=dev)
    check(lib.gsr_bin_sort_bounded(P, width, height, _ptr(compute_locally), _ptr(prep), cap, _ptr(scratch), sort_bytes,
                                   _ptr(point_list), _ptr(ranges), stream), "gsr_bin_sort_bounded")
    off = int(lib.gsr_bin_total_offset(P, width, height))
    host = cap_ctx.take_pinned(1)
    check(lib.gsr_flag_if_greater(prep.data_ptr() + off, cap, _ptr(cap_ctx.flag), FLAG_PAIRS, host.data_ptr(), stream),
          "gsr_flag_if_greater")
    cap_ctx.pairs.append((host, cap))
    if os.environ.get("GSR_GRAPH_DEBUG") == "1":
        _DEBUG_RANGES.extend([("prep", prep.data_ptr(), prep.numel()), ("scratch", scratch.data_ptr(), scratch.numel()),
                              ("point_list", point_list.data_ptr(), 4 * point_list.numel())])
    return point_list, ranges, cap


class PendingPairs:

    def __init__(self, ticket, sorted_, cap, P, width, height, mask, prep, ranges, dev, stream, key, cuda_args):
        self.ticket, self.sorted, self.cap = ticket, sorted_, cap
        self.P, self.width, self.height = P, width, height
        self.mask, self.prep, self.ranges = mask, prep, ranges
        self.dev, self.stream, self.key, self.cuda_args = dev, stream, key, cuda_args
        self.D = None

    def finish(self):
        same = (not _NO_STREAM_CACHE) and self.stream is current_stream(self.dev)
        with _on(self.dev), (_NULL_RANGE if same else torch.cuda.stream(self.stream)):
            stream = _stream()
            D = ctypes.c_int64(0)
            rc = lib.gsr_bin_count_wait(self.ticket, ctypes.byref(D), stream)
            if rc != GSR_ERETRY:
                check(rc, "gsr_bin_count_wait")
            self.D = D = int(D.value)
            if D > _MAX_PAIRS.get(self.key, 0):
                _MAX_PAIRS[self.key] = D
            if rc == 0 and self.sorted and D <= self.cap:
                self.prep = None
                return D, None
            sort_bytes = lib.gsr_bin_sort_bytes(self.P, D, self.width, self.height)
            scratch = _sort_scratch(max(sort_bytes, 4), self.dev)
            point_list = torch.empty((_bucket(max(D, 1) * 4) // 4,), dtype=torch.int32, device=self.dev)[:max(D, 1)]
            with zhx_range(self.cuda_args, "50 SortPairs time"):
                check(lib.gsr_bin_sort(self.P, self.width, self.height, _ptr(self.mask), _ptr(self.prep), D,
                                       _ptr(scratch), sort_bytes, _ptr(point_list), _ptr(self.ranges), stream),
                      "gsr_bin_sort")
            self.prep = None
            return D, point_list


def bin_gaussians(means2D, depths, radii, conic_opacity, compute_locally, width, height, cuda_args=None, defer=False):
    if _CAPTURE[0] is not None:
        return _bin_gaussians_captured(_CAPTURE[0], means2D, depths, radii, conic_opacity, compute_locally, width, height)
    P, dev, ranges, prep, args = _bin_workspaces(means2D, depths, radii, conic_opacity, compute_locally, width, height)
    if _DEBUG_RANGES:
        _debug_overlap("prep", prep)
        _debug_overlap("means2D", means2D)
    stream = _stream()
    key = (dev.index if dev.index is not None else torch.cuda.current_device(), int(stream.value or 0))
    cap, point_list = 0, None
    kept = _SORT_SCRATCH.get(key)
    if _SPECULATIVE_SORT[0] and kept is not None:
        cap = min(int(lib.gsr_bin_sort_capacity(P, kept.numel(), width, height)), _bucket(4 * _MAX_PAIRS.get(key, 0)) // 4)
        if cap > 0:
            point_list = torch.empty((cap,), dtype=torch.int32, device=dev)
    ticket, sorted_ = ctypes.c_uint32(0), ctypes.c_int(0)
    if _zhx_on(cuda_args):
        with zhx_range(cuda_args, "24 updateDistributedStatLocally.updateTileTouched time"):
            check(lib.gsr_bin_prepare_async(*args, ctypes.byref(ticket), stream), "gsr_bin_prepare_async")
        if cap > 0 and ticket.value != 0:
            with zhx_range(cuda_args, "50 SortPairs time"):
                check(lib.gsr_bin_sort_bounded(P, width, height, _ptr(compute_locally), _ptr(prep), cap, _ptr(kept),
                                               kept.numel(), _ptr(point_list), _ptr(ranges), stream),
                      "gsr_bin_sort_bounded")
            sorted_.value = 1
    else:
        check(lib.gsr_bin_speculative_async(*args, cap if cap > 0 else 0, _ptr(kept) if cap > 0 else None,
                                            kept.numel() if cap > 0 else 0, _ptr(point_list) if cap > 0 else None,
                                            _ptr(ranges), ctypes.byref(ticket), ctypes.byref(sorted_), stream),
              "gsr_bin_speculative_async")
    pend = PendingPairs(ticket.value, bool(sorted_.value), cap, P, width, height, compute_locally, prep, ranges, dev,
                        current_stream(dev), key, cuda_args)
    if kernel_timer.enabled and ticket.value:
        off = int(lib.gsr_bin_segments_offset(P, width, height))
        _LAST_SEGMENTS[0] = int(prep[off:off + 4].view(torch.int32).item())
    if defer and sorted_.value:
        return point_list, ranges, pend
    D, again = pend.finish()
    if again is not None:
        return again, ranges, D
    return point_list[:max(D, 1)], ranges, D


class _RenderGaussians(torch.autograd.Function):
    @staticmethod
    def forward(ctx, means2D, conic_opacity, rgb, depths, radii, compute_locally, raster_settings, cuda_args,
                token=None):
        ctx.set_materialize_grads(False)
        rs = raster_settings
        means2D, conic_opacity, rgb = _f32c(means2D, "means2D"), _f32c(conic_opacity, "conic_opacity"), _f32c(rgb, "rgb")
        depths = _f32c(depths, "depths")
        if not radii.is_cuda:
            raise RuntimeError("diff_gaussian_rasterization: `radii` must live on the gfx950 device")
        radii = radii.to(torch.int32).contiguous()
        H, W = int(rs.image_height), int(rs.image_width)
        gx, gy = (W + BLOCK_X - 1) // BLOCK_X, (H + BLOCK_Y - 1) // BLOCK_Y
        P = means2D.shape[0]
        dev = means2D.device
        if compute_locally is None:
            mask = torch.ones((gy * gx,), dtype=torch.uint8, device=dev)
        else:
            if compute_locally.numel() != gx * gy:
                raise ValueError(f"compute_locally must have TILE_Y*TILE_X = {gy}x{gx} entries")
            mask = compute_locally.to(device=dev).contiguous().view(-1)
            mask = mask.view(torch.uint8) if mask.dtype == torch.bool else mask.to(torch.uint8)
        bg = _f32c(rs.bg, "bg")
        timing = (cuda_args.get("_gsr_timing") if isinstance(cuda_args, dict) else None) or _timing_mode()
        if _CAPTURE[0] is not None:
            timing = "off"
        stats = cuda_args.get("stats_collector") if isinstance(cuda_args, dict) else None
        contrib = cuda_args.get("contributions") if isinstance(cuda_args, dict) else None
        if contrib is not None:
            if _CAPTURE[0] is not None:
                raise RuntimeError("diff_gaussian_rasterization: cuda_args['contributions'] is not available under graph "
                                   "capture (the statistics need the view's final lists)")
            if not isinstance(contrib, ContributionStats) or contrib.P != P or \
                    contrib.hits.get_device() != means2D.get_device():
                raise ValueError(f"cuda_args['contributions'] must be a ContributionStats of {P} rows on {dev}")
        invd = bool(cuda_args.get("invdepth")) if isinstance(cuda_args, dict) else False
        if invd and _CAPTURE[0] is not None:
            raise RuntimeError("diff_gaussian_rasterization: cuda_args['invdepth'] is not available under graph capture "
                               "(the map needs the view's final lists)")
        feat = bool(cuda_args.get("features")) if isinstance(cuda_args, dict) else False
# ... 1452 lines not shown
```

### grendel-gs_amd/diff_gaussian_rasterization/_lib.py

```python
import ctypes
import os

_HERE = os.path.dirname(os.path.abspath(__file__))
LIB_PATH = os.environ.get("GSRASTER_LIB") or os.path.join(_HERE, "libgsraster.so")

c_int, c_float, c_void_p, c_size_t, c_int64 = (ctypes.c_int, ctypes.c_float, ctypes.c_void_p, ctypes.c_size_t,
                                                ctypes.c_int64)

_K11_ADAM_PREFIX = ([c_int] * 4 + [c_void_p, c_void_p, c_float] + [c_void_p] * 5 + [c_int, c_int] + [c_void_p] * 6 +
                    [c_int] + [c_void_p] * 7 + [c_float])

SIGNATURES = {
    "gsr_error_string": (ctypes.c_char_p, [c_int]),
    "gsr_abi_version": (c_int, []),
    "gsr_get_block_xy": (c_int, [ctypes.POINTER(c_int)] * 3),
    "gsr_preprocess_forward": (c_int, [c_int, c_int, c_int, c_void_p, c_void_p, c_float, c_void_p, c_void_p, c_void_p,
                                       c_void_p, c_void_p, c_void_p, c_int, c_int, c_float, c_float, c_void_p,
                                       c_void_p, c_void_p, c_void_p, c_void_p, c_void_p, c_void_p, c_void_p]),
    "gsr_preprocess_backward": (c_int, [c_int, c_int, c_int, c_void_p, c_void_p, c_float, c_void_p, c_void_p,
                                        c_void_p, c_void_p, c_void_p, c_int, c_int, c_float, c_float] +
                                [c_void_p] * 6 + [c_int] + [c_void_p] * 6),
    "gsr_set_antialiasing": (c_int, [c_int]),
    "gsr_preprocess_backward_aa": (c_int, [c_int, c_int, c_int, c_void_p, c_void_p, c_float, c_void_p, c_void_p,
                                           c_void_p, c_void_p, c_void_p, c_void_p, c_int, c_int, c_float, c_float] +
# ... 51 lines not shown
    "gsr_scatter_add_rows": (c_int, [c_int64, c_void_p, c_void_p, c_void_p, c_void_p]),
    "gsr_knn_workspace_bytes": (c_size_t, [c_int]),
    "gsr_knn_mean_dist2": (c_int, [c_int, c_void_p, c_void_p, c_void_p, c_size_t, c_void_p]),
    "gsr_densify_stats": (c_int, [c_int64, c_void_p, c_void_p, c_int64, c_void_p, c_void_p, c_void_p, c_void_p]),
    "gsr_group_rows_bytes": (c_size_t, [c_int64]),
    "gsr_group_rows": (c_int, [c_int64, c_int, c_void_p, c_void_p, c_void_p, c_void_p, c_size_t, c_void_p]),
    "gsr_gather_rows": (c_int, [c_int64, c_void_p, c_int, c_void_p, c_void_p, c_void_p, c_void_p, c_void_p,
                                c_void_p]),
    "gsr_scatter_rows": (c_int, [c_int64, c_void_p, c_int, c_void_p, c_void_p, c_void_p, c_void_p, c_void_p,
                                 c_void_p]),
    "gsr_densify_plan_bytes": (c_size_t, [c_int64]),
    "gsr_densify_plan": (c_int, [c_int64, c_void_p, c_void_p, c_void_p, c_void_p, c_void_p, c_size_t, c_void_p]),
    "gsr_densify_move": (c_int, [c_int64, c_void_p, c_void_p, c_int64, c_int64, c_int64, c_int64, c_int, c_int] +
                         [c_void_p] * 7 + [c_int64, c_void_p, c_void_p, c_void_p]),
    "gsr_mcmc_relocate_bytes": (c_size_t, [c_int64]),
    "gsr_mcmc_relocate_plan": (c_int, [c_int64, c_int64, c_void_p, c_float, ctypes.c_uint64, ctypes.c_uint32, c_void_p,
                                       c_void_p, c_void_p, c_void_p, c_size_t, c_void_p]),
    "gsr_mcmc_relocate_apply": (c_int, [c_int64, c_int64, c_void_p, c_void_p, c_void_p, c_float, c_int, c_int] +
                                [c_void_p] * 5),
    "gsr_mcmc_noise": (c_int, [c_int64, c_void_p, c_void_p, c_void_p, c_void_p, c_float, c_void_p, ctypes.c_uint64,
                               ctypes.c_uint32, c_void_p]),
    "gsr_mcmc_normals": (c_int, [c_int64, ctypes.c_uint64, ctypes.c_uint32, c_void_p, c_void_p]),
    "gsr_mcmc_reg_grad": (c_int, [c_int64, c_void_p, c_void_p, c_float, c_float, c_void_p, c_void_p, c_void_p]),
    "gsr_adam_step": (c_int, [c_int64, c_void_p, c_void_p, c_void_p, c_void_p, ctypes.c_double, ctypes.c_double,
                              ctypes.c_double, ctypes.c_double, c_int64, c_float, c_void_p]),
    "gsr_adam_step_multi": (c_int, [c_int] + [c_void_p] * 10 + [c_float, c_void_p]),
    "gsr_preprocess_forward_raw": (c_int, [c_int, c_int, c_int, c_void_p, c_void_p, c_float] + [c_void_p] * 7 +
                                   [c_int, c_int, c_float, c_float] + [c_void_p] * 8),
    "gsr_preprocess_backward_raw": (c_int, [c_int, c_int, c_int, c_void_p, c_void_p, c_float] + [c_void_p] * 7 +
                                    [c_int, c_int, c_float, c_float] + [c_void_p] * 6 + [c_int] + [c_void_p] * 7),
    "gsr_preprocess_forward_raw_batched": (c_int, [c_int, c_int, c_int, c_int, c_void_p, c_void_p, c_float] +
                                           [c_void_p] * 5 + [c_int, c_int] + [c_void_p] * 8),
    "gsr_preprocess_backward_raw_batched": (c_int, [c_int, c_int, c_int, c_int, c_void_p, c_void_p, c_float] +
                                            [c_void_p] * 5 + [c_int, c_int] + [c_void_p] * 6 + [c_int] +
                                            [c_void_p] * 7),
    "gsr_preprocess_backward_adam_raw_batched": (c_int, _K11_ADAM_PREFIX + [c_void_p, c_void_p]),
    "gsr_preprocess_backward_adam_raw_batched_dyn": (c_int, _K11_ADAM_PREFIX + [c_void_p] * 4),
    "gsr_preprocess_backward_adam_raw_batched_sums": (c_int, [c_int] * 4 + [c_void_p, c_void_p, c_float] +
                                                      [c_void_p] * 5 + [c_int, c_int] + [c_void_p] * 12 + [c_float] +
                                                      [c_void_p] * 4),
    "gsr_sparse_step_workspace_bytes": (c_size_t, [c_int]),
    "gsr_preprocess_backward_adam_raw_batched_sparse": (c_int, _K11_ADAM_PREFIX + [c_void_p, c_void_p, c_void_p,
                                                                                    c_size_t, c_void_p, c_void_p,
                                                                                    c_void_p]),
    "gsr_preprocess_backward_cams_bytes": (c_size_t, [c_int, c_int]),
    "gsr_preprocess_backward_cams": (c_int, [c_int, c_int, c_int, c_int, c_void_p, c_void_p, c_int, c_void_p, c_int,
                                             c_void_p, c_int, c_int] + [c_void_p] * 6 + [c_int, c_void_p, c_size_t,
                                                                                         c_void_p, c_void_p]),
    "gsr_bin_total_offset": (c_size_t, [c_int, c_int, c_int]),
    "gsr_bin_segments_offset": (c_size_t, [c_int, c_int, c_int]),
    "gsr_bin_speculative_async": (c_int, [c_int, c_int, c_int, c_void_p, c_void_p, c_void_p, c_void_p, c_void_p,
                                          c_void_p, c_size_t, c_int64, c_void_p, c_size_t, c_void_p, c_void_p,
                                          ctypes.POINTER(ctypes.c_uint32), ctypes.POINTER(c_int), c_void_p]),
    "gsr_set_bin_persistent": (c_int, [c_int]),
    "gsr_set_tile_cull": (c_int, [c_int]),
    "gsr_set_bin_rowmajor": (c_int, [c_int]),
    "gsr_bin_persist_status": (c_int, [ctypes.POINTER(ctypes.c_uint32)]),
    "gsr_bin_timeline": (c_int, [c_int, c_void_p, c_int, ctypes.POINTER(c_int)]),
    "gsr_flag_if_greater": (c_int, [c_void_p, ctypes.c_uint32, c_void_p, ctypes.c_uint32, c_void_p, c_void_p]),
    "gsr_render_seg_bytes": (c_size_t, [c_int, c_int]),
    "gsr_render_forward": (c_int, [c_int, c_int, c_int] + [c_void_p] * 11 + [c_size_t, c_int, c_int, c_void_p, c_size_t,
                                                                           c_void_p]),
    "gsr_render_backward": (c_int, [c_int, c_int, c_int] + [c_void_p] * 13 + [c_size_t, c_int, c_int, c_int, c_void_p,
                                                                            c_void_p, c_void_p]),
    "gsr_render_backward_sums": (c_int, [c_int, c_int, c_int] + [c_void_p] * 12 + [c_size_t, c_int, c_int, c_void_p,
                                                                                 c_void_p, c_void_p]),
    "gsr_render_record_materialize": (c_int, [c_int, c_void_p, c_void_p, c_void_p, c_int, c_void_p]),
    "gsr_set_deferred_rounding": (c_int, [c_int]),
    "gsr_deferred_rounding": (c_int, []),
    "gsr_composite_walked": (c_int, [ctypes.POINTER(ctypes.c_ulonglong), c_int]),
    "gsr_render_contrib": (c_int, [c_int, c_int, c_int] + [c_void_p] * 6 + [c_int, c_int] + [c_void_p] * 4),
    "gsr_contrib_merge_rows": (c_int, [c_int64] + [c_void_p] * 8),
    "gsr_render_invdepth": (c_int, [c_int, c_int, c_int] + [c_void_p] * 7 + [c_int, c_int, c_void_p, c_void_p]),
    "gsr_render_invdepth_backward": (c_int, [c_int, c_int, c_int] + [c_void_p] * 10 + [c_int, c_int] + [c_void_p] * 3),
    "gsr_depth_backward_means3d": (c_int, [c_int] + [c_void_p] * 3 + [c_int, c_void_p, c_int, c_void_p]),
    "gsr_render_features": (c_int, [c_int] * 4 + [c_void_p] * 7 + [c_int, c_int, c_void_p, c_void_p]),
    "gsr_render_features_backward": (c_int, [c_int] * 4 + [c_void_p] * 9 + [c_int, c_int] + [c_void_p] * 4),
    "gsr_render_absgrad": (c_int, [c_int, c_int, c_int] + [c_void_p] * 10 + [c_int, c_int] + [c_void_p] * 3),
    "gsr_absgrad_merge_rows": (c_int, [c_int64] + [c_void_p] * 4),
    "gsr_publish_flag": (c_int, [c_void_p, c_void_p, c_void_p, ctypes.c_uint32, c_void_p]),
    "gsr_exchange_check": (c_int, [c_void_p, c_void_p, c_int, c_int, c_int, ctypes.c_uint64, c_int, c_void_p,
                                   ctypes.c_uint32, ctypes.c_uint32, c_void_p, c_void_p]),
    "gsr_activate_forward": (c_int, [c_int, c_int] + [c_void_p] * 10),
    "gsr_activate_backward": (c_int, [c_int, c_int] + [c_void_p] * 13),
    "gsr_filter3d_num_partials": (c_int, [c_int]),
    "gsr_filter3d_distance": (c_int, [c_int, c_int, c_void_p, c_void_p, c_int, c_int] + [c_void_p] * 4),
    "gsr_filter3d_finalize": (c_int, [c_int] + [c_void_p] * 3 + [c_int, c_void_p, c_float, c_void_p, c_void_p]),
    "gsr_filter3d_apply_forward": (c_int, [c_int] + [c_void_p] * 6),
    "gsr_filter3d_apply_backward": (c_int, [c_int] + [c_void_p] * 8),
    "gsr_bilagrid_slice_forward": (c_int, [c_int] * 4 + [c_void_p, c_int64, c_void_p, c_int, c_int, c_int, c_void_p,
                                           c_int64, c_void_p]),
    "gsr_bilagrid_num_partials": (c_int64, [c_int] * 5),
    "gsr_bilagrid_slice_backward": (c_int, [c_int] * 4 + [c_void_p, c_int64, c_void_p, c_int, c_int, c_int, c_void_p,
                                            c_int64, c_void_p, c_int64, c_void_p, c_void_p, c_void_p]),
    "gsr_bilagrid_tv_num_partials": (c_int, [c_int] * 4),
    "gsr_bilagrid_tv": (c_int, [c_int] * 4 + [c_void_p, c_float, c_void_p, c_void_p, c_void_p, c_void_p]),
}

ABI_VERSION = 15


def _load():
    if not os.path.exists(LIB_PATH):
        raise ImportError(
            f"{LIB_PATH} not found: the gfx950 HIP library has not been built "
            "(run `python __graft_entry__.py build` or `python grendel-gs_amd/csrc/build.py`). "
# ... 20 lines not shown
```

### grendel-gs_amd/gaussian_renderer/__init__.py

```python
import math
import os

import numpy as np
import torch
import torch.distributed as dist

import utils.general_utils as utils
from diff_gaussian_rasterization import GaussianRasterizationSettings, GaussianRasterizer

import diff_gaussian_rasterization as _dgr

import contextlib

_NULL = contextlib.nullcontext()


def _keep_grad_view(t):
    import weakref
    ref, first = weakref.ref(t), [True]

    def hook(g):
        x = ref()
        if x is not None:
            g = _dgr.lazy_record_view(g)
# ... 702 lines not shown
        ca["_gsr_timing"] = timing
        cuda_args_list.append(ca)
        settings = GaussianRasterizationSettings(
            image_height=int(camera.image_height),
            image_width=int(camera.image_width),
            tanfovx=math.tan(camera.FoVx * 0.5),
            tanfovy=math.tan(camera.FoVy * 0.5),
            bg=bg_color,
            scale_modifier=scaling_modifier,
            viewmatrix=camera.world_view_transform,
            projmatrix=camera.full_proj_transform,
            sh_degree=pc.active_sh_degree,
            campos=camera.camera_center,
            prefiltered=False,
            debug=pipe.debug,
        )
        rasterizers.append(GaussianRasterizer(raster_settings=settings))
    if len({(r.raster_settings.image_height, r.raster_settings.image_width) for r in rasterizers}) != 1:
        raise ValueError("all cameras of a batch must have one image size (the reference keeps ONE global image size, "
                         "utils/general_utils.py:89-93, set from the first training camera, scene/__init__.py:93-97)")
    packed = []
    pose_grad = False
    for camera, rast in zip(batched_viewpoint_cameras, rasterizers):
        if _dgr._camera_requires_grad(rast.raster_settings):
            pose_grad = True
            packed.append(_dgr.pack_camera(rast.raster_settings))
            continue
        rs_k = rast.raster_settings
        key = (float(rs_k.tanfovx), float(rs_k.tanfovy)) + tuple(
            (t.data_ptr(), t._version) for t in (rs_k.viewmatrix, rs_k.projmatrix, rs_k.campos))
        cached = getattr(camera, "_gsr_packed", None)
        if cached is None or cached[0] != key or cached[1].device != raw[0].device:
            cached = (key, _dgr.pack_camera(rast.raster_settings))
            try:
                camera._gsr_packed = cached
            except AttributeError:
                pass
        packed.append(cached[1])
    rs0 = rasterizers[0].raster_settings
    if len(packed) == 1:
        cams_block = packed[0].view(1, -1)
    elif pose_grad or _dgr.capturing() is not None:
        cams_block = torch.stack(packed)
    else:
        skey = tuple(id(t) for t in packed)
        hit = _CAMERA_BLOCKS.get(skey)
        if hit is not None and all(a is b and a._version == v for a, b, v in zip(hit[1], packed, hit[2])):
            cams_block = hit[0]
        else:
            cams_block = torch.stack(packed)
            if len(_CAMERA_BLOCKS) > 1024:
                _CAMERA_BLOCKS.clear()
            _CAMERA_BLOCKS[skey] = (cams_block, tuple(packed), tuple(t._version for t in packed))
    m2_all, rgb_all, co_all, radii_all, depths_all = _dgr.preprocess_gaussians_raw_batched(
        *raw, cams_block, pc.active_sh_degree,
        scaling_modifier, rs0.image_width, rs0.image_height, tanfov0=(rs0.tanfovx, rs0.tanfovy),
        cuda_args_list=cuda_args_list)
    for k in range(len(rasterizers)):
        means2D = m2_all[k]
        if mode == "train":
            _keep_grad_view(means2D)
        params.append([means2D, rgb_all[k], co_all[k], radii_all[k], depths_all[k]])
    if timers is not None:
        timers.stop("forward_preprocess_gaussians")

    pkg = {
        "batched_locally_preprocessed_mean2D": [p[0] for p in params],
        "batched_locally_preprocessed_visibility_filter": _LazyPerCamera([p[3] for p in params], lambda r: r > 0),
        "batched_locally_preprocessed_radii": [p[3] for p in params],
        "batched_rasterizers": rasterizers,
        "batched_cuda_args": cuda_args_list,
    }
    W = utils.DEFAULT_GROUP.size()
    if W == 1 and not (_EXCHANGE_OPTIONS["forced"] and dist.is_initialized()):
        redistributed = tuple([p[c] for p in params] for c in range(5))
        sizes = [[[p[0].shape[0] for p in params]]]
        _fill(pkg, redistributed, sizes)
        if mode == "train" and not pose_grad and not _INVDEPTH[0] and not _FILTER3D[0] and not _FEATURES[0] and \
                len(cuda_args_list) <= _dgr.DEFER_MAX_CAMERAS:
            for ca in cuda_args_list:
                ca["_gsr_defer_record"] = True
        if _INVDEPTH[0]:
            pkg["_invdepth_xyz"] = raw[0]
        if feats is not None:
            pkg["_features_rows"] = feats
        return pkg
    if W * len(params) > 512:
        raise ValueError(f"world size x batch size = {W * len(params)} exceeds the 512 (destination, camera) segments "
                         "one exchange launch carries (include/gsraster.h: gsr_exchange_count)")
    if timers is not None:
        timers.start("forward_all_to_all_communication")
    mine = [k for k, st in enumerate(batched_strategies) if utils.GLOBAL_RANK in st.gpu_ids]

    def exchange(known=None):
        *redistributed, sizes, (events, token), pending = _batched_exchange_final(
            [p[0] for p in params], rgb_all, co_all, radii_all, depths_all, rasterizers, batched_strategies,
            speculate=False if _legacy else None, pipeline=False if _legacy else None, _known=known)
        _fill(pkg, redistributed, sizes)
        pkg["_exchange_events"] = events
        for ca in cuda_args_list:
            ca.pop("_exchange_token", None)
        if token is not None and mine:
            cuda_args_list[mine[-1]]["_exchange_token"] = token
        pkg["_exchange_token"] = token
        if _ABSGRAD[0]:
            pkg["_absgrad_routes"] = _LAST_ROUTES[0]
# ... 24 lines not shown
    if timers is not None:
        timers.stop("forward_all_to_all_communication")
    return pkg


def _fill(pkg, redistributed, sizes):
    for name, value in zip(("means2D", "rgb", "conic_opacity", "radii", "depths"), redistributed):
        pkg[f"batched_{name}_redistributed"] = value
    pkg["gpui_to_gpuj_imgk_size"] = sizes


def _render_cameras(pkg, batched_strategies):
    timers = utils.get_timers()
    images, masks, late = [], [], []
    invdepth = [None] * len(batched_strategies)
    features = [None] * len(batched_strategies)
    mine = [k for k, st in enumerate(batched_strategies) if utils.GLOBAL_RANK in st.gpu_ids]
    dev0 = pkg["batched_means2D_redistributed"][mine[0]].device if mine else None
    two = (_EXCHANGE_OPTIONS["camera_streams"] > 1 and len(mine) > 1 and dev0 is not None and dev0.type == "cuda"
           and _dgr.capturing() is None)
    if two:
        main = torch.cuda.current_stream(dev0)
        sides = [_side_stream(dev0, "camera0"), _side_stream(dev0, "camera1")]
        for s_ in sides:
            s_.wait_stream(main)
    turn = 0
    for k, strategy in enumerate(batched_strategies):
        if utils.GLOBAL_RANK not in strategy.gpu_ids:
            images.append(None)
            masks.append(None)
            continue
        compute_locally = strategy.get_compute_locally()
        extended = strategy.get_extended_compute_locally()
        cuda_args = pkg["batched_cuda_args"][k]
        with (torch.cuda.stream(sides[turn & 1]) if two else _NULL):
            turn += 1
            ev = pkg.get("_exchange_events", None)
            if ev is not None and ev[k] is not None:
                _dgr.current_stream().wait_event(ev[k])
            means2D = pkg["batched_means2D_redistributed"][k]
            rgb = pkg["batched_rgb_redistributed"][k]
            conic_opacity = pkg["batched_conic_opacity_redistributed"][k]
            if timers is not None:
                timers.start("forward_render_gaussians")
            if means2D.shape[0] < 10:
                image = means2D.sum() + conic_opacity.sum() + rgb.sum()
                if cuda_args.get("_exchange_token") is not None:
                    image = image + 0.0 * cuda_args["_exchange_token"].sum()
                st = cuda_args["stats_collector"]
                st["forward_render_time"] = st["backward_render_time"] = st["forward_loss_time"] = 0.0
            else:
                rows_of = getattr(strategy, "_my_rows", None)
                cuda_args["_gsr_band"] = rows_of() if rows_of is not None else None
                cuda_args["_gsr_pending"] = late
                try:
                    image, _, _, _ = pkg["batched_rasterizers"][k].render_gaussians(
                        means2D=means2D, conic_opacity=conic_opacity, rgb=rgb,
                        depths=pkg["batched_depths_redistributed"][k], radii=pkg["batched_radii_redistributed"][k],
                        compute_locally=compute_locally, extended_compute_locally=extended, cuda_args=cuda_args)
                finally:
                    cuda_args.pop("_gsr_pending", None)
                if cuda_args.get("invdepth"):
                    invdepth[k] = _invdepth_map(pkg, k, cuda_args, means2D, conic_opacity)
                    if two:
                        invdepth[k].record_stream(main)
                if cuda_args.get("features"):
                    features[k] = pkg["batched_rasterizers"][k].render_features(means2D, conic_opacity,
                                                                                 pkg["_features_rows"], cuda_args)
                    if two:
                        features[k].record_stream(main)
            if two:
                image.record_stream(main)
            if timers is not None:
                timers.stop("forward_render_gaussians")
        images.append(image)
        masks.append(compute_locally)
    if two:
        for s_ in sides:
            main.wait_stream(s_)
    if any(ca.get("invdepth") for ca in pkg["batched_cuda_args"]):
        pkg["batched_invdepth"] = invdepth
    if any(ca.get("features") for ca in pkg["batched_cuda_args"]):
        pkg["batched_features"] = features
    return images, masks, late


def _settle(late):
    for settle in late:
        settle()
    del late[:]


settle = _settle


def render_final(batched_screenspace_pkg, batched_strategies, tile_size=16, late=None):
    pkg = batched_screenspace_pkg
    images, masks, mine = _render_cameras(pkg, batched_strategies)
    if late is not None and pkg.get("_exchange_pending") is None:
        late.extend(mine)
        return images, masks
    late = mine
    _settle(late)
    verify = pkg.get("_exchange_pending")
    if verify is not None and not verify():
        images, masks, late = _render_cameras(pkg, batched_strategies)
# ... 99 lines not shown
```

### include/gsraster.h

```cpp
#ifndef GSRASTER_H
#define GSRASTER_H

#include <stddef.h>
#include <stdint.h>

#ifdef __cplusplus
extern "C" {
#endif

#define GSR_BLOCK_X 16
#define GSR_BLOCK_Y 16
#define GSR_ONE_DIM_BLOCK 256

#define GSR_EINVAL (-1)
#define GSR_ENOSPACE (-2)
#define GSR_ERETRY (-3)
#define GSR_EFAULT (-4)

typedef void *gsr_stream_t;

const char *gsr_error_string(int code);

int gsr_abi_version(void);

int gsr_get_block_xy(int *block_x, int *block_y, int *one_dim_block);

int gsr_preprocess_forward(int P, int sh_degree, int sh_coeffs, const float *means3D, const float *scales,
                           float scale_modifier, const float *rotations, const float *shs, const float *opacities,
                           const float *viewmatrix, const float *projmatrix, const float *campos, int width,
                           int height, float tanfovx, float tanfovy, float *means2D, float *depths, int32_t *radii,
                           float *cov3D, float *conic_opacity, float *rgb, uint8_t *clamped, gsr_stream_t stream);

int gsr_preprocess_backward(int P, int sh_degree, int sh_coeffs, const float *means3D, const float *scales,
                            float scale_modifier, const float *rotations, const float *shs, const float *viewmatrix,
                            const float *projmatrix, const float *campos, int width, int height, float tanfovx,
                            float tanfovy, const int32_t *radii, const float *cov3D, const uint8_t *clamped,
                            const float *dL_dmeans2D, const float *dL_dconic_opacity, const float *dL_drgb,
                            int grad_row_stride, float *dL_dmeans3D, float *dL_dscales, float *dL_drotations,
                            float *dL_dshs, float *dL_dopacities, gsr_stream_t stream);

int gsr_set_antialiasing(int mode);
int gsr_preprocess_backward_aa(int P, int sh_degree, int sh_coeffs, const float *means3D, const float *scales,
                               float scale_modifier, const float *rotations, const float *shs, const float *opacities,
                               const float *viewmatrix, const float *projmatrix, const float *campos, int width,
                               int height, float tanfovx, float tanfovy, const int32_t *radii, const float *cov3D,
                               const uint8_t *clamped, const float *dL_dmeans2D, const float *dL_dconic_opacity,
                               const float *dL_drgb, int grad_row_stride, float *dL_dmeans3D, float *dL_dscales,
                               float *dL_drotations, float *dL_dshs, float *dL_dopacities, gsr_stream_t stream);

int gsr_get_local2j_ids_bool(int P, int width, int height, int world_size, const float *means2D,
                             const int32_t *radii, const int32_t *dist_global_strategy, uint8_t *out,
                             gsr_stream_t stream);

size_t gsr_bin_prepare_bytes(int P, int width, int height);
int gsr_bin_prepare(int P, int width, int height, const float *means2D, const float *depths, const int32_t *radii,
                    const float *conic_opacity, const uint8_t *compute_locally, void *prep, size_t prep_bytes,
                    int64_t *num_rendered_host, gsr_stream_t stream);
size_t gsr_bin_sort_bytes(int P, int64_t num_rendered, int width, int height);
int gsr_bin_sort(int P, int width, int height, const uint8_t *compute_locally, const void *prep,
                 int64_t num_rendered, void *scratch, size_t scratch_bytes, uint32_t *point_list, int32_t *ranges,
                 gsr_stream_t stream);
int gsr_set_depth_tie_order(int mode);
int gsr_bin_prepare_async(int P, int width, int height, const float *means2D, const float *depths, const int32_t *radii,
                          const float *conic_opacity, const uint8_t *compute_locally, void *prep, size_t prep_bytes,
                          uint32_t *ticket, gsr_stream_t stream);
int gsr_bin_count_wait(uint32_t ticket, int64_t *num_rendered_host, gsr_stream_t stream);
int64_t gsr_bin_sort_capacity(int P, size_t scratch_bytes, int width, int height);
int gsr_bin_speculative_async(int P, int width, int height, const float *means2D, const float *depths,
                              const int32_t *radii, const float *conic_opacity, const uint8_t *compute_locally, void *prep,
                              size_t prep_bytes, int64_t capacity, void *scratch, size_t scratch_bytes,
                              uint32_t *point_list, int32_t *ranges, uint32_t *ticket, int *sorted, gsr_stream_t stream);
int gsr_set_bin_persistent(int mode);
int gsr_set_bin_rowmajor(int mode);
int gsr_set_tile_cull(int mode);
int gsr_bin_persist_status(uint32_t *out4);
int gsr_bin_timeline(int which, unsigned long long *out, int max_words, int *grid);
size_t gsr_bin_total_offset(int P, int width, int height);
size_t gsr_bin_segments_offset(int P, int width, int height);

int gsr_stamp(const uint32_t *seq_dev, uint64_t *host_ring_pinned, uint32_t slots, uint32_t per_slot, uint32_t index,
              gsr_stream_t stream);
int gsr_band_mask(int grid_x, int grid_y, int B, const int32_t *band_rows_dev, int stride_words, uint8_t *mask,
                  gsr_stream_t stream);
int gsr_publish_flag(const uint32_t *flag_dev, const uint32_t *seq_dev, uint32_t *host_ring_pinned, uint32_t slots,
                     gsr_stream_t stream);
int gsr_flag_if_greater(const uint32_t *value_dev, uint32_t limit, uint32_t *flag_dev, uint32_t bit,
                        uint32_t *host_copy_pinned, gsr_stream_t stream);
int gsr_exchange_check(const int32_t *all_counts_dev, const int32_t *caps_dev, int W, int B, int me,
                       uint64_t rendered_mask, int few, uint32_t *flag_dev, uint32_t bit_over, uint32_t bit_few,
                       int32_t *host_copy_pinned, gsr_stream_t stream);
int gsr_bin_sort_bounded(int P, int width, int height, const uint8_t *compute_locally, const void *prep,
                         int64_t capacity, void *scratch, size_t scratch_bytes, uint32_t *point_list, int32_t *ranges,
                         gsr_stream_t stream);

size_t gsr_render_seg_bytes(int width, int height);
int gsr_render_forward(int P, int width, int height, const int32_t *ranges, const uint32_t *point_list,
                       const float *means2D, const float *conic_opacity, const float *rgb,
                       const uint8_t *compute_locally, const float *bg, float *out_color, float *final_T,
                       int32_t *n_contrib, void *seg_ws, size_t seg_bytes, int row_lo, int row_hi, void *zero_ptr,
                       size_t zero_bytes, gsr_stream_t stream);
int gsr_render_backward(int P, int width, int height, const int32_t *ranges, const uint32_t *point_list,
                        const float *means2D, const float *conic_opacity, const float *rgb,
                        const uint8_t *compute_locally, const float *bg, const float *final_T,
                        const int32_t *n_contrib, const float *dL_dpixels, float *dL_record, const float *out_color,
                        void *seg_ws, size_t seg_bytes, int row_lo, int row_hi, int record_is_zero, double *acc64,
                        uint8_t *touched, gsr_stream_t stream);
int gsr_render_backward_sums(int P, int width, int height, const int32_t *ranges, const uint32_t *point_list,
                             const float *means2D, const float *conic_opacity, const float *rgb,
                             const uint8_t *compute_locally, const float *bg, const float *final_T,
                             const int32_t *n_contrib, const float *dL_dpixels, const float *out_color, void *seg_ws,
                             size_t seg_bytes, int row_lo, int row_hi, double *acc64, uint8_t *touched,
                             gsr_stream_t stream);
int gsr_render_record_materialize(int P, const double *acc64, const uint8_t *touched, float *dL_record,
                                  int record_is_zero, gsr_stream_t stream);
int gsr_set_deferred_rounding(int mode);
int gsr_deferred_rounding(void);
int gsr_composite_walked(unsigned long long *out2, int reset);

int gsr_render_contrib(int P, int width, int height, const int32_t *ranges, const uint32_t *point_list,
                       const float *means2D, const float *conic_opacity, const uint8_t *compute_locally,
                       const int32_t *n_contrib, int row_lo, int row_hi, int64_t *hits, float *wmax, double *wsum,
                       gsr_stream_t stream);
int gsr_contrib_merge_rows(int64_t n, const int32_t *idx, const int64_t *src_hits, const float *src_wmax,
                           const double *src_wsum, int64_t *dst_hits, float *dst_wmax, double *dst_wsum,
// ... 135 lines not shown
#define GSR_DENSIFY_ROLE_MOMENT 1
#define GSR_DENSIFY_ROLE_XYZ 2
#define GSR_DENSIFY_ROLE_SCALING 3
size_t gsr_densify_plan_bytes(int64_t P);
int gsr_densify_plan(int64_t P, const uint8_t *cls, int32_t *ranks, int32_t *split_rows, int64_t *counts,
                     void *workspace, size_t workspace_bytes, gsr_stream_t stream);
int gsr_densify_move(int64_t P, const uint8_t *cls, const int32_t *ranks, int64_t n_orig, int64_t n_clone,
                     int64_t n_child, int64_t n_split, int copies, int num_tensors, const void *const *srcs,
                     void *const *dsts, const void *const *alts, const int32_t *widths, const int32_t *roles,
                     const int64_t *src_strides, const int64_t *dst_strides, int64_t dst_rows, const float *rotation,
                     const float *samples, gsr_stream_t stream);

#define GSR_MCMC_ROLE_COPY 0
#define GSR_MCMC_ROLE_MOMENT 1
#define GSR_MCMC_ROLE_OPACITY 2
#define GSR_MCMC_ROLE_SCALING 3
#define GSR_MCMC_N_MAX 51
size_t gsr_mcmc_relocate_bytes(int64_t rows);
int gsr_mcmc_relocate_plan(int64_t P, int64_t n_add, const float *opacity_act, float min_opacity, uint64_t seed,
                           uint32_t event, int32_t *src, int32_t *count, int64_t *totals, void *workspace,
                           size_t workspace_bytes, gsr_stream_t stream);
int gsr_mcmc_relocate_apply(int64_t P, int64_t n_add, const int32_t *src, const int32_t *count,
                            const float *opacity_act, float min_opacity, int n_max, int num_tensors,
                            void *const *tensors, const int32_t *widths, const int64_t *strides, const int32_t *roles,
                            gsr_stream_t stream);
int gsr_mcmc_noise(int64_t P, float *xyz, const float *scaling_raw, const float *rotation_raw,
                   const float *opacity_raw, float scaler, const float *xi, uint64_t seed, uint32_t step,
                   gsr_stream_t stream);
int gsr_mcmc_normals(int64_t n, uint64_t seed, uint32_t step, float *out, gsr_stream_t stream);
int gsr_mcmc_reg_grad(int64_t P, const float *opacity_raw, const float *scaling_raw, float c_opacity, float c_scale,
                      float *grad_opacity, float *grad_scaling, gsr_stream_t stream);

int gsr_preprocess_forward_raw(int P, int sh_degree, int sh_coeffs, const float *xyz, const float *scaling,
                               float scale_modifier, const float *rotation, const float *features_dc,
                               const float *features_rest, const float *opacity, const float *viewmatrix,
                               const float *projmatrix, const float *campos, int width, int height, float tanfovx,
                               float tanfovy, float *means2D, float *depths, int32_t *radii, float *cov3D,
                               float *conic_opacity, float *rgb, uint8_t *clamped, gsr_stream_t stream);
int gsr_preprocess_backward_raw(int P, int sh_degree, int sh_coeffs, const float *xyz, const float *scaling,
                                float scale_modifier, const float *rotation, const float *features_dc,
                                const float *features_rest, const float *opacity, const float *viewmatrix,
                                const float *projmatrix, const float *campos, int width, int height, float tanfovx,
                                float tanfovy, const int32_t *radii, const float *cov3D, const uint8_t *clamped,
                                const float *dL_dmeans2D, const float *dL_dconic_opacity, const float *dL_drgb,
                                int grad_row_stride, float *dL_dxyz, float *dL_dscaling, float *dL_drotation, float *dL_dfeatures_dc,
                                float *dL_dfeatures_rest, float *dL_dopacity, gsr_stream_t stream);

int gsr_preprocess_forward_raw_batched(int P, int B, int sh_degree, int sh_coeffs, const float *xyz,
                                       const float *scaling, float scale_modifier, const float *rotation,
                                       const float *features_dc, const float *features_rest, const float *opacity,
                                       const float *cams, int width, int height, float *means2D, float *depths,
                                       int32_t *radii, float *cov3D, float *conic_opacity, float *rgb,
                                       uint8_t *clamped, gsr_stream_t stream);
int gsr_preprocess_backward_raw_batched(int P, int B, int sh_degree, int sh_coeffs, const float *xyz,
                                        const float *scaling, float scale_modifier, const float *rotation,
                                        const float *features_dc, const float *features_rest, const float *opacity,
                                        const float *cams, int width, int height, const int32_t *radii,
                                        const float *cov3D, const uint8_t *clamped, const float *dL_dmeans2D,
                                        const float *dL_dconic_opacity, const float *dL_drgb, int grad_row_stride, float *dL_dxyz,
                                        float *dL_dscaling, float *dL_drotation, float *dL_dfeatures_dc,
                                        float *dL_dfeatures_rest, float *dL_dopacity, gsr_stream_t stream);

size_t gsr_preprocess_backward_cams_bytes(int P, int B);
int gsr_preprocess_backward_cams(int P, int B, int sh_degree, int sh_coeffs, const float *means3D, const float *sh_dc,
                                 int sh_dc_stride, const float *sh_rest, int sh_rest_stride, const float *cams,
                                 int width, int height, const int32_t *radii, const float *cov3D,
                                 const uint8_t *clamped, const float *dL_dmeans2D, const float *dL_dconic_opacity,
                                 const float *dL_drgb, int grad_row_stride, void *workspace, size_t workspace_bytes,
                                 float *dL_dcams, gsr_stream_t stream);

int gsr_preprocess_backward_adam_raw_batched(int P, int B, int sh_degree, int sh_coeffs, float *xyz, float *scaling,
                                             float scale_modifier, float *rotation, float *features_dc,
                                             float *features_rest, float *opacity, const float *cams, int width,
                                             int height, const int32_t *radii, const float *cov3D,
                                             const uint8_t *clamped, const float *dL_dmeans2D,
                                             const float *dL_dconic_opacity, const float *dL_drgb,
                                             int grad_row_stride, float *const *exp_avgs, float *const *exp_avg_sqs,
                                             const double *lrs, const double *beta1s, const double *beta2s,
                                             const double *epss, const int64_t *steps, float grad_scale,
                                             const float *tanfov0, gsr_stream_t stream);
int gsr_preprocess_backward_adam_raw_batched_dyn(int P, int B, int sh_degree, int sh_coeffs, float *xyz, float *scaling,
                                                 float scale_modifier, float *rotation, float *features_dc,
                                                 float *features_rest, float *opacity, const float *cams, int width,
                                                 int height, const int32_t *radii, const float *cov3D,
                                                 const uint8_t *clamped, const float *dL_dmeans2D,
                                                 const float *dL_dconic_opacity, const float *dL_drgb,
                                                 int grad_row_stride, float *const *exp_avgs,
                                                 float *const *exp_avg_sqs, const double *lrs, const double *beta1s,
                                                 const double *beta2s, const double *epss, const int64_t *steps,
                                                 float grad_scale, const float *tanfov0, const float *dyn_dev,
                                                 const uint32_t *skip_flag_dev, gsr_stream_t stream);
int gsr_preprocess_backward_adam_raw_batched_sums(int P, int B, int sh_degree, int sh_coeffs, float *xyz, float *scaling,
                                                  float scale_modifier, float *rotation, float *features_dc,
                                                  float *features_rest, float *opacity, const float *cams, int width,
                                                  int height, const int32_t *radii, const float *cov3D,
                                                  const uint8_t *clamped, const double *const *acc64,
                                                  const uint8_t *const *touched, float *const *exp_avgs,
                                                  float *const *exp_avg_sqs, const double *lrs, const double *beta1s,
                                                  const double *beta2s, const double *epss, const int64_t *steps,
                                                  float grad_scale, const float *tanfov0, const float *dyn_dev,
                                                  const uint32_t *skip_flag_dev, gsr_stream_t stream);

size_t gsr_sparse_step_workspace_bytes(int P);
int gsr_preprocess_backward_adam_raw_batched_sparse(int P, int B, int sh_degree, int sh_coeffs, float *xyz,
                                                    float *scaling, float scale_modifier, float *rotation,
                                                    float *features_dc, float *features_rest, float *opacity,
// ... 47 lines not shown
```

Baseline: 852.0.

## Record tile rects and counts in preprocess to skip recompute in binning prepare

The forward preprocess kernel now writes each Gaussian's tile rectangle, tile-count word, and per-block key min/max and pair-count rows straight into the binning prep buffer. A new REC variant of the persistent prepare kernel reduces those rows instead of redoing rect and extent math and the row-hull scan, and builds the depth-bucket histogram in the same pass. This removes repeated per-Gaussian geometry work and a reduction phase from binning. In exchange it adds extra preprocess writes, Python-side plumbing that applies only to single-camera, single-rank cases, and a new template instance that can affect grid sizing.

```diff
diff --git a/grendel-gs_amd/csrc/binning.hip b/grendel-gs_amd/csrc/binning.hip
--- a/grendel-gs_amd/csrc/binning.hip
+++ b/grendel-gs_amd/csrc/binning.hip
@@ -1,4 +1,5 @@
 #include "common.h"
+#include "tile_rect.h"
 
 #include <atomic>
 #include <chrono>
@@ -474,8 +475,16 @@
     a.done_word = d.done; a.done_seq = (uint32_t)admit;
     a.timeout_ticks = 5000000ull;
     a.force_abort = h.abort_p ? 1 : 0;
-    if (items == 4) hipLaunchKernelGGL(bin_prepare_persist_kernel<4>, dim3(G), dim3(PP_THREADS), 0, c.stream, a);
-    else hipLaunchKernelGGL(bin_prepare_persist_kernel<8>, dim3(G), dim3(PP_THREADS), 0, c.stream, a);
+    if (use_k1_record(c, f, h, nb, G)) {
+        a.k1_rows = reinterpret_cast<const uint4 *>(c.k1_rows);
+        a.k1_nrows = c.k1_nrows;
+        if (items == 4) hipLaunchKernelGGL((bin_prepare_persist_kernel<4, true>), dim3(G), dim3(PP_THREADS), 0, c.stream, a);
+        else hipLaunchKernelGGL((bin_prepare_persist_kernel<8, true>), dim3(G), dim3(PP_THREADS), 0, c.stream, a);
+    } else if (items == 4) {
+        hipLaunchKernelGGL(bin_prepare_persist_kernel<4>, dim3(G), dim3(PP_THREADS), 0, c.stream, a);
+    } else {
+        hipLaunchKernelGGL(bin_prepare_persist_kernel<8>, dim3(G), dim3(PP_THREADS), 0, c.stream, a);
+    }
     GSR_LAUNCH_CHECK();
     *ticket = seq;
     return 0;
@@ -729,6 +738,17 @@
                                          const uint8_t *compute_locally, void *prep, size_t prep_bytes,
                                          int64_t capacity, void *scratch, size_t scratch_bytes, uint32_t *point_list,
                                          int32_t *ranges, uint32_t *ticket, int *sorted, gsr_stream_t stream_) {
+    return gsr_bin_speculative_record_async(P, width, height, means2D, depths, radii, conic_opacity, compute_locally, prep,
+                                            prep_bytes, capacity, scratch, scratch_bytes, point_list, ranges, ticket,
+                                            sorted, nullptr, 0, stream_);
+}
+
+extern "C" int gsr_bin_speculative_record_async(int P, int width, int height, const float *means2D, const float *depths,
+                                                const int32_t *radii, const float *conic_opacity,
+                                                const uint8_t *compute_locally, void *prep, size_t prep_bytes,
+                                                int64_t capacity, void *scratch, size_t scratch_bytes,
+                                                uint32_t *point_list, int32_t *ranges, uint32_t *ticket, int *sorted,
+                                                const uint32_t *record_rows, int record_rows_n, gsr_stream_t stream_) {
     if (!ticket || !sorted) return GSR_EINVAL;
     *sorted = 0;
     if (P < 0 || width <= 0 || height <= 0) return GSR_EINVAL;
@@ -747,7 +767,8 @@
     hipStream_t stream = reinterpret_cast<hipStream_t>(stream_);
     const bool sort = capacity > 0 && scratch && point_list;
     const SortPlan p = sort ? plan_sort(f, capacity, scratch_bytes, true, h.rows_min) : SortPlan{GSR_EINVAL};
-    PrepCall c{P, width, height, means2D, depths, radii, conic_opacity, compute_locally, prep, stream, true, nullptr, 0};
+    PrepCall c{P, width, height, means2D, depths, radii, conic_opacity, compute_locally, prep, stream, true, nullptr, 0,
+               record_rows, record_rows_n};
     if (!p.err) {
         c.zero_ptr = reinterpret_cast<char *>(scratch) + p.zero_off;
         c.zero_bytes = p.zero_bytes;
@@ -761,6 +782,8 @@
     d->calls[*ticket % TOTAL_SLOTS] = c;
     d->calls[*ticket % TOTAL_SLOTS].zero_ptr = nullptr;
     d->calls[*ticket % TOTAL_SLOTS].zero_bytes = 0;
+    d->calls[*ticket % TOTAL_SLOTS].k1_rows = nullptr;
+    d->calls[*ticket % TOTAL_SLOTS].k1_nrows = 0;
     if (!sort) return 0;
     if (!ranges) return GSR_EINVAL;
     if (!f.yx) GSR_HIP(hipMemsetAsync(ranges, 0, sizeof(int32_t) * 2 * ((size_t)f.gx * f.gy + 1), stream));
@@ -769,6 +792,16 @@
                   h, *d, p.form);
     if (rc) return rc;
     *sorted = 1;
+    return 0;
+}
+
+extern "C" int gsr_bin_record_offsets(int P, int width, int height, size_t *offsets) {
+    if (P < 0 || width <= 0 || height <= 0 || !offsets) return GSR_EINVAL;
+    const int gx = (width + GSR_BLOCK_X - 1) / GSR_BLOCK_X, gy = (height + GSR_BLOCK_Y - 1) / GSR_BLOCK_Y;
+    if (gx > RADIX_DIGITS || gy > RADIX_DIGITS) return GSR_EINVAL;
+    const PrepLayout L = prep_layout(P);
+    offsets[0] = L.rects;
+    offsets[1] = L.tt;
     return 0;
 }
 
diff --git a/grendel-gs_amd/csrc/binning_host.h b/grendel-gs_amd/csrc/binning_host.h
--- a/grendel-gs_amd/csrc/binning_host.h
+++ b/grendel-gs_amd/csrc/binning_host.h
@@ -67,6 +67,7 @@
     bool depth_buckets;
     bool abort_p, abort_s;
     bool timeline;
+    bool k1_record;
 };
 BinHooks read_hooks() {
     BinHooks h;
@@ -89,6 +90,8 @@
     h.abort_s = e && strchr(e, 's') != nullptr;
     e = getenv("GSR_BIN_TIMELINE");
     h.timeline = e && *e == '1';
+    e = getenv("GSR_BIN_K1_RECORD");
+    h.k1_record = !(e && *e == '0');
     return h;
 }
 
@@ -292,7 +295,13 @@
     bool persistent;
     void *zero_ptr;
     size_t zero_bytes;
-};
+    const uint32_t *k1_rows;
+    int k1_nrows;
+};
+bool use_k1_record(const PrepCall &c, const BinFrame &f, const BinHooks &h, long long tiles, int G) {
+    return c.k1_rows && h.k1_record && f.yx && !f.cull && tiles == (long long)G &&
+           c.k1_nrows == (c.P + GSR_ONE_DIM_BLOCK - 1) / GSR_ONE_DIM_BLOCK;
+}
 
 struct BinDevice {
     uint32_t *total_word;
@@ -325,12 +334,14 @@
     if (d.caps_init) return;
     d.caps_init = true;
     const int dev = (int)(&d - g_bin_devices);
-    int cus = 0, per_p = 0, per_p8 = 0, per_s = 0;
+    int cus = 0, per_p = 0, per_p8 = 0, per_r = 0, per_r8 = 0, per_s = 0;
     if (hipDeviceGetAttribute(&cus, hipDeviceAttributeMultiprocessorCount, dev) == hipSuccess && cus > 0 &&
         hipOccupancyMaxActiveBlocksPerMultiprocessor(&per_p, bin_prepare_persist_kernel<4>, PP_THREADS, 0) == hipSuccess &&
         hipOccupancyMaxActiveBlocksPerMultiprocessor(&per_p8, bin_prepare_persist_kernel<8>, PP_THREADS, 0) == hipSuccess &&
+        hipOccupancyMaxActiveBlocksPerMultiprocessor(&per_r, bin_prepare_persist_kernel<4, true>, PP_THREADS, 0) == hipSuccess &&
+        hipOccupancyMaxActiveBlocksPerMultiprocessor(&per_r8, bin_prepare_persist_kernel<8, true>, PP_THREADS, 0) == hipSuccess &&
         hipOccupancyMaxActiveBlocksPerMultiprocessor(&per_s, bin_sort_persist_kernel, PS_THREADS, 0) == hipSuccess) {
-        d.grid_p = (per_p >= 1 && per_p8 >= 1) ? (cus < PERSIST_MAX_GRID_P ? cus : PERSIST_MAX_GRID_P) : 0;
+        d.grid_p = (per_p >= 1 && per_p8 >= 1 && per_r >= 1 && per_r8 >= 1) ? (cus < PERSIST_MAX_GRID_P ? cus : PERSIST_MAX_GRID_P) : 0;
         const long long gs = (long long)cus * (per_s < 4 ? per_s : 4);
         d.grid_s = per_s >= 1 ? (int)(gs < PERSIST_MAX_GRID_S ? gs : PERSIST_MAX_GRID_S) : 0;
     }
diff --git a/grendel-gs_amd/csrc/binning_persist.h b/grendel-gs_amd/csrc/binning_persist.h
--- a/grendel-gs_amd/csrc/binning_persist.h
+++ b/grendel-gs_amd/csrc/binning_persist.h
@@ -2,8 +2,6 @@
 
 namespace {
 
-constexpr int TT_SHIFT = 20;
-constexpr uint32_t TT_MASK = (1u << TT_SHIFT) - 1u;
 constexpr uint32_t GB_ABORT = 0x80000000u;
 constexpr int GB_FAN = 32;
 constexpr int GB_LEAF_STRIDE = 32;
@@ -177,11 +175,7 @@
     if (c) __hip_atomic_fetch_add(&grp[(w / GB_FAN) * RADIX_DIGITS + d], c, __ATOMIC_RELAXED, __HIP_MEMORY_SCOPE_AGENT);
 }
 
-struct alignas(16) TileRect {
-    uint32_t xs, ys;
-    unsigned long long mask;
-};
-static_assert(sizeof(TileRect) == 16, "one 16-byte gather");
+static_assert(RADIX_DIGITS + 1 == 257, "gsr_rect_hist's difference arrays");
 
 __device__ __forceinline__ unsigned long long gsr_full_mask(int n) { return n >= 64 ? ~0ull : ((1ull << n) - 1ull); }
 
@@ -254,18 +248,9 @@
 __device__ __forceinline__ uint32_t gsr_rect_tiles(const float2 xy, const float4 co, int minx, int miny, int maxx, int maxy,
                                                    bool cull, int32_t (*dxy)[RADIX_DIGITS + 1], TileRect &out) {
     const int w = maxx - minx, h = maxy - miny;
-    out.xs = (uint32_t)minx | ((uint32_t)maxx << 16);
-    out.ys = (uint32_t)miny | ((uint32_t)maxy << 16);
-    out.mask = ~0ull;
+    gsr_rect_pack(minx, miny, maxx, maxy, out);
     if (!cull || w * h > 64) {
-        if (dxy) {
-            atomicAdd(&dxy[0][minx], h);
-            atomicAdd(&dxy[0][maxx], -h);
-            atomicAdd(&dxy[1][miny], w);
-            atomicAdd(&dxy[1][maxy], -w);
-            atomicAdd(&dxy[2][miny], 1);
-            atomicAdd(&dxy[2][maxy], -1);
-        }
+        if (dxy) gsr_rect_hist(dxy, minx, miny, maxx, maxy);
         return (uint32_t)(w * h);
     }
     const unsigned long long mask = gsr_tile_mask(xy, co, minx, miny, maxx, maxy);
@@ -517,6 +502,8 @@
     uint64_t timeout_ticks;
     int force_abort;
     unsigned long long *tstamp;
+    const uint4 *k1_rows;
+    int k1_nrows;
 };
 
 struct PPExtra {
@@ -632,7 +619,7 @@
 }
 
 
-template <int PP_ITEMS>
+template <int PP_ITEMS, bool REC = false>
 __global__ void __launch_bounds__(PP_THREADS)
 bin_prepare_persist_kernel(const PrepPersistArgs a) {
     constexpr int PP_TILE = PP_THREADS * PP_ITEMS;
@@ -658,8 +645,49 @@
     if (threadIdx.x <= RADIX_DIGITS) ex.dxy[0][threadIdx.x] = ex.dxy[1][threadIdx.x] = ex.dxy[2][threadIdx.x] = 0;
     if (threadIdx.x == 0) { ex.s_lo = a.gy; ex.s_hi = 0; }
     clear_wtab(sm);
-    __syncthreads();
-    {
+    uint32_t rkmn = 0xFFFFFFFFu, rkmx = 0u;
+    unsigned long long rsum = 0;
+    int rsh = 0;
+    bool rec_bins = false;
+    uint32_t *const lbin = sm8.skey;
+    if (REC) {
+        for (int r = threadIdx.x; r < a.k1_nrows; r += PP_THREADS) {
+            const uint4 x = a.k1_rows[r];
+            rkmn = min(rkmn, x.x);
+            rkmx = max(rkmx, x.y);
+            rsum += (unsigned long long)x.z | ((unsigned long long)x.w << 32);
+        }
+        rsum = wave_sum64_local(rsum);
+        {
+            const int ol = opaque_lane();
+#pragma unroll
+            for (int o = 32; o >= 1; o >>= 1) {
+                rkmn = min(rkmn, xor_lane(rkmn, ol, o));
+                rkmx = max(rkmx, xor_lane(rkmx, ol, o));
+            }
+        }
+        if (lane == 0) {
+            sm.scan64[wave] = rsum;
+            red2[wave] = rkmn;
+            red2[PP_WAVES + wave] = rkmx;
+        }
+        __syncthreads();
+        rsum = 0;
+        for (int wv = 0; wv < PP_WAVES; wv++) {
+            rsum += sm.scan64[wv];
+            rkmn = min(rkmn, red2[wv]);
+            rkmx = max(rkmx, red2[PP_WAVES + wv]);
+        }
+        rec_bins = try_buckets && rkmn <= rkmx && rkmx != 0xFFFFFFFFu;
+        if (rec_bins) {
+            const uint32_t range = rkmx - rkmn;
+            rsh = max((range ? 32 - __clz(range) : 0) - BK_BIN_BITS, 0);
+            for (int i = threadIdx.x; i < BK_BINS; i += PP_THREADS) lbin[i] = 0u;
+        }
+        GSR_TS(30);
+    }
+    __syncthreads();
+    if (!REC) {
         const int total = a.gx * a.gy;
         const int per = (total + PP_THREADS - 1) / PP_THREADS;
         const int b0 = threadIdx.x * per, b1 = min(b0 + per, total);
@@ -676,7 +704,7 @@
         }
     }
     __syncthreads();
-    const int hull0 = ex.s_lo, hull1 = ex.s_hi;
+    const int hull0 = REC ? 0 : ex.s_lo, hull1 = REC ? a.gy : ex.s_hi;
     if (w == 0 && threadIdx.x == 0) {
         a.hull_out[0] = hull1 > hull0 ? hull0 : 0;
         a.hull_out[1] = hull1 > hull0 ? hull1 : 0;
@@ -688,6 +716,41 @@
         const long long wbase = t * PP_TILE + (long long)wave * (PP_ITEMS * 64);
 #pragma unroll
         for (int r0 = 0; r0 < PP_ITEMS; r0 += 4) {
+        if constexpr (REC) {
+            uint2 rc[4];
+            uint32_t tw[4];
+            float dep[4];
+#pragma unroll
+            for (int q4 = 0; q4 < 4; q4++) {
+                const long long i = wbase + (r0 + q4) * 64 + lane;
+                const long long ic = i < P ? i : P - 1;
+                rc[q4] = *reinterpret_cast<const uint2 *>(&a.rects[ic]);
+                tw[q4] = a.tt[ic];
+                dep[q4] = a.depths[ic];
+            }
+#pragma unroll
+            for (int q4 = 0; q4 < 4; q4++) {
+                const int r = r0 + q4;
+                const long long i = wbase + r * 64 + lane;
+                key[r] = 0xFFFFFFFFu;
+                val[r] = (uint32_t)i;
+                if (i < P) {
+                    const uint32_t n = a.tile_hist ? (tw[q4] & TT_MASK) : tw[q4];
+                    if (n) {
+                        key[r] = __float_as_uint(dep[q4]);
+                        if (a.tile_hist)
+                            gsr_rect_hist(ex.dxy, (int)(rc[q4].x & 0xFFFFu), (int)(rc[q4].y & 0xFFFFu),
+                                          (int)(rc[q4].x >> 16), (int)(rc[q4].y >> 16));
+                        if (rec_bins) atomicAdd(&lbin[(key[r] - rkmn) >> rsh], 1u);
+                    }
+                    if (!keep) {
+                        st_agent(&a.kA[i], key[r]);
+                        st_agent(&a.vA[i], val[r]);
+                    }
+                }
+            }
+            continue;
+        }
         int rad[4];
         float2 xy[4];
         float4 co[4];
@@ -712,18 +775,10 @@
                 uint32_t n = 0;
                 TileRect rect{0u, 0u, 0ull};
                 if (rad[q4] > 0) {
-                    float exx, eyy;
-                    if (gsr_alpha_extent(co[q4], exx, eyy)) {
-                        int minx, miny, maxx, maxy;
-                        gsr_get_rect(xy[q4].x, xy[q4].y, rad[q4], a.gx, a.gy, minx, miny, maxx, maxy);
-                        miny = max(miny, hull0);
-                        maxy = min(maxy, hull1);
-                        gsr_narrow_span(xy[q4].x, exx, minx, maxx);
-                        gsr_narrow_span(xy[q4].y, eyy, miny, maxy);
-                        if (maxx > minx && maxy > miny)
-                            n = gsr_rect_tiles(xy[q4], co[q4], minx, miny, maxx, maxy, a.cull != 0,
-                                               a.tile_hist ? ex.dxy : nullptr, rect);
-                    }
+                    int minx, miny, maxx, maxy;
+                    if (gsr_k3_rect(xy[q4], co[q4], rad[q4], a.gx, a.gy, hull0, hull1, minx, miny, maxx, maxy))
+                        n = gsr_rect_tiles(xy[q4], co[q4], minx, miny, maxx, maxy, a.cull != 0,
+                                           a.tile_hist ? ex.dxy : nullptr, rect);
                 }
                 if (n) {
                     key[r] = __float_as_uint(dep[q4]);
@@ -731,7 +786,7 @@
                     kmx = max(kmx, key[r]);
                 }
                 nsum += n;
-                st_agent(&a.tt[i], (a.tile_hist && n) ? (n | (((rect.ys >> 16) - (rect.ys & 0xFFFFu)) << TT_SHIFT)) : n);
+                st_agent(&a.tt[i], gsr_tt_word(n, rect, a.tile_hist != nullptr));
                 a.rects[i] = rect;
                 if (!keep) {
                     st_agent(&a.kA[i], key[r]);
@@ -754,7 +809,17 @@
         }
     }
     if (!try_buckets && d < RADIX_DIGITS) publish_counts(a.cnt, a.grp, w, d, mytot);
-    {
+    if (REC) {
+        if (rec_bins) {
+            __syncthreads();
+            for (int i = threadIdx.x; i < BK_BINS; i += PP_THREADS) {
+                const uint32_t c = lbin[i];
+                if (c) __hip_atomic_fetch_add(&a.bins[i], c, __ATOMIC_RELAXED, __HIP_MEMORY_SCOPE_AGENT);
+            }
+        }
+        if (w == 0 && threadIdx.x == 0 && rsum)
+            __hip_atomic_fetch_add(a.early, rsum, __ATOMIC_RELAXED, __HIP_MEMORY_SCOPE_AGENT);
+    } else {
         nsum = wave_sum64_local(nsum);
         {
             const int ol = opaque_lane();
@@ -808,7 +873,7 @@
     }
     GSR_TS(2);
     if (w == 0 && threadIdx.x == 0) {
-        const unsigned long long dsum = __hip_atomic_load(a.early, __ATOMIC_RELAXED, __HIP_MEMORY_SCOPE_AGENT);
+        const unsigned long long dsum = REC ? rsum : __hip_atomic_load(a.early, __ATOMIC_RELAXED, __HIP_MEMORY_SCOPE_AGENT);
         __hip_atomic_store(a.host_total, clamp_pair_count(dsum), __ATOMIC_RELAXED, __HIP_MEMORY_SCOPE_SYSTEM);
         __hip_atomic_store(a.host_total + 1, a.seq, __ATOMIC_RELEASE, __HIP_MEMORY_SCOPE_SYSTEM);
     }
@@ -817,14 +882,14 @@
     if (try_buckets) {
         static_assert(BK_BINS == 4 * PP_THREADS, "four bins per thread");
         const long long wbase0 = t0 * PP_TILE + (long long)wave * (PP_ITEMS * 64);
-        const uint32_t kmin = ~ld_agent(&a.bins[BK_BINS]), kmax = ld_agent(&a.bins[BK_BINS + 1]);
+        const uint32_t kmin = REC ? rkmn : ~ld_agent(&a.bins[BK_BINS]), kmax = REC ? rkmx : ld_agent(&a.bins[BK_BINS + 1]);
         const uint32_t NB = min(G, BK_TAIL);
         bool buckets = kmin <= kmax && kmax != 0xFFFFFFFFu;
         if (buckets) {
             const uint32_t range = kmax - kmin;
             const int sh = max((range ? 32 - __clz(range) : 0) - BK_BIN_BITS, 0);
             const BucketDigit digit{bk.map, kmin, sh};
-            uint32_t *const lbin = sm8.skey;
+            if (!REC) {
             for (int i = threadIdx.x; i < BK_BINS; i += PP_THREADS) lbin[i] = 0u;
             __syncthreads();
 #pragma unroll
@@ -838,6 +903,7 @@
             GSR_TS(21);
             if (!grid_barrier(a.sync, G, epoch, forever, &sm.flag)) { barrier_fault(a.done_word, 0x200u + epoch); return; }
             GSR_TS(22);
+            }
             {
                 uint32_t c4[4], s4 = 0, live;
 #pragma unroll
diff --git a/grendel-gs_amd/csrc/build.py b/grendel-gs_amd/csrc/build.py
--- a/grendel-gs_amd/csrc/build.py
+++ b/grendel-gs_amd/csrc/build.py
@@ -8,7 +8,7 @@
 OUT_DIR = os.path.join(ROOT, "diff_gaussian_rasterization")
 SO = os.path.join(OUT_DIR, "libgsraster.so")
 UNITS = ["preprocess", "binning", "composite", "contrib", "invdepth", "features", "absgrad", "loss", "bilagrid", "metrics", "optim", "activations", "filter3d", "knn", "compact", "mcmc", "exchange", "api"]
-HEADERS = [os.path.join(HERE, "common.h"), os.path.join(HERE, "composite_math.h"), os.path.join(HERE, "radix.h"), os.path.join(HERE, "binning_persist.h"), os.path.join(HERE, "binning_rows.h"), os.path.join(HERE, "binning_host.h"),
+HEADERS = [os.path.join(HERE, "common.h"), os.path.join(HERE, "tile_rect.h"),os.path.join(HERE, "composite_math.h"), os.path.join(HERE, "radix.h"), os.path.join(HERE, "binning_persist.h"), os.path.join(HERE, "binning_rows.h"), os.path.join(HERE, "binning_host.h"),
            os.path.join(os.path.dirname(ROOT), "include", "gsraster.h")]
 FLAGS = ["--offload-arch=gfx950", "-O3", "-std=c++17", "-fPIC", "-munsafe-fp-atomics", "-Wall",
          "-Wno-unused-function"]
diff --git a/grendel-gs_amd/csrc/common.h b/grendel-gs_amd/csrc/common.h
--- a/grendel-gs_amd/csrc/common.h
+++ b/grendel-gs_amd/csrc/common.h
@@ -56,11 +56,15 @@
     ex = ey = 1e30f;
     if (!(co.w >= 1.0f / 255.0f)) return false;
     const float tau = __logf(255.0f * co.w);
-    const float det = co.x * co.z - co.y * co.y;
+    float det;
+    {
+#pragma clang fp contract(off)
+        det = co.x * co.z - co.y * co.y;
+    }
     if (det > 0.f && tau >= 0.f) {
         const float s = 2.0f * tau / det;
-        ex = sqrtf(s * co.z) * 1.01f + 0.5f;
-        ey = sqrtf(s * co.x) * 1.01f + 0.5f;
+        ex = __builtin_fmaf(sqrtf(s * co.z), 1.01f, 0.5f);
+        ey = __builtin_fmaf(sqrtf(s * co.x), 1.01f, 0.5f);
     }
     return true;
 }
diff --git a/grendel-gs_amd/csrc/preprocess.hip b/grendel-gs_amd/csrc/preprocess.hip
--- a/grendel-gs_amd/csrc/preprocess.hip
+++ b/grendel-gs_amd/csrc/preprocess.hip
@@ -1,4 +1,5 @@
 #include "common.h"
+#include "tile_rect.h"
 
 #include <atomic>
 #include <initializer_list>
@@ -1104,6 +1105,40 @@
     return cam;
 }
 
+struct K1Record {
+    TileRect *rects;
+    uint32_t *tt;
+    uint4 *rows;
+};
+__device__ __forceinline__ void k1_record_row(const K1Record rec, uint32_t n, uint32_t key) {
+    __shared__ uint32_t s_mn[GSR_ONE_DIM_BLOCK / GSR_WAVE], s_mx[GSR_ONE_DIM_BLOCK / GSR_WAVE];
+    __shared__ unsigned long long s_sum[GSR_ONE_DIM_BLOCK / GSR_WAVE];
+    uint32_t mn = n ? key : 0xFFFFFFFFu, mx = n ? key : 0u;
+    unsigned long long sum = n;
+#pragma unroll
+    for (int o = 32; o >= 1; o >>= 1) {
+        mn = min(mn, (uint32_t)__shfl_xor(mn, o, GSR_WAVE));
+        mx = max(mx, (uint32_t)__shfl_xor(mx, o, GSR_WAVE));
+        sum += __shfl_xor(sum, o, GSR_WAVE);
+    }
+    const int wave = threadIdx.x / GSR_WAVE;
+    if ((threadIdx.x & (GSR_WAVE - 1)) == 0) {
+        s_mn[wave] = mn;
+        s_mx[wave] = mx;
+        s_sum[wave] = sum;
+    }
+    __syncthreads();
+    if (threadIdx.x == 0) {
+#pragma unroll
+        for (int wv = 1; wv < GSR_ONE_DIM_BLOCK / GSR_WAVE; wv++) {
+            mn = min(mn, s_mn[wv]);
+            mx = max(mx, s_mx[wv]);
+            sum += s_sum[wv];
+        }
+        rec.rows[blockIdx.x] = make_uint4(mn, mx, (uint32_t)sum, (uint32_t)(sum >> 32));
+    }
+}
+
 template <int DEG, bool AA>
 __global__ void __launch_bounds__(GSR_ONE_DIM_BLOCK)
 preprocess_forward_batched_kernel(int P, int B, int M, const float *__restrict__ xyz, const float *__restrict__ scaling,
@@ -1171,6 +1206,86 @@
             clamped[3 * o + k] = cl[k] ? 1 : 0;
         }
     }
+}
+
+template <int DEG, bool AA>
+__global__ void __launch_bounds__(GSR_ONE_DIM_BLOCK, 4)
+preprocess_forward_record_kernel(int P, int M, const float *__restrict__ xyz, const float *__restrict__ scaling,
+                                 float scale_modifier, const float *__restrict__ rotation,
+                                 const float *__restrict__ f_dc, const float *__restrict__ f_rest,
+                                 const float *__restrict__ opacity, const float *__restrict__ cp, int W, int H,
+                                 float2 *__restrict__ means2D, float *__restrict__ depths,
+                                 int32_t *__restrict__ radii, float *__restrict__ cov3D,
+                                 float4 *__restrict__ conic_opacity, float *__restrict__ rgb,
+                                 uint8_t *__restrict__ clamped, const K1Record rec) {
+    const int i = blockIdx.x * blockDim.x + threadIdx.x;
+    constexpr int NC = (DEG + 1) * (DEG + 1);
+    uint32_t rec_n = 0, rec_key = 0;
+    if (i < P) {
+        const int gx = (W + GSR_BLOCK_X - 1) / GSR_BLOCK_X, gy = (H + GSR_BLOCK_Y - 1) / GSR_BLOCK_Y;
+        const float p[3] = {xyz[3 * (size_t)i], xyz[3 * (size_t)i + 1], xyz[3 * (size_t)i + 2]};
+        float qnr, qn;
+        const float4 q = quat_normalize(*reinterpret_cast<const float4 *>(rotation + 4 * (size_t)i), qnr, qn);
+        const float s[3] = {scale_modifier * expf(scaling[3 * (size_t)i]),
+                            scale_modifier * expf(scaling[3 * (size_t)i + 1]),
+                            scale_modifier * expf(scaling[3 * (size_t)i + 2])};
+        const float op = sigmoidf(opacity[i]);
+        float S[3][3];
+        cov3d_from_scale_rot(q, s, S);
+        cov3D[6 * (size_t)i + 0] = S[0][0]; cov3D[6 * (size_t)i + 1] = S[0][1]; cov3D[6 * (size_t)i + 2] = S[0][2];
+        cov3D[6 * (size_t)i + 3] = S[1][1]; cov3D[6 * (size_t)i + 4] = S[1][2]; cov3D[6 * (size_t)i + 5] = S[2][2];
+        float shl[NC * 3];
+        shl[0] = f_dc[3 * (size_t)i];
+        shl[1] = f_dc[3 * (size_t)i + 1];
+        shl[2] = f_dc[3 * (size_t)i + 2];
+        {
+            const float *rp = f_rest + (size_t)i * (M - 1) * 3;
+#pragma unroll
+            for (int k = 3; k < NC * 3; k++) shl[k] = rp[k - 3];
+        }
+        const Cam cam = load_cam_packed(cp);
+        const float tanfovx = cp[35], tanfovy = cp[36];
+        const float fx = W / (2.0f * tanfovx), fy = H / (2.0f * tanfovy);
+        int radius = 0;
+        float2 xy = make_float2(0.f, 0.f);
+        float depth = 0.f;
+        float4 co = make_float4(0.f, 0.f, 0.f, 0.f);
+        float col[3] = {0.f, 0.f, 0.f};
+        bool cl[3] = {false, false, false};
+        float t[3];
+        view_transform(cam.v, p, t);
+        do {
+            if (t[2] <= 0.2f) break;
+            Geom2D g;
+            if (!project_geometry<AA>(cam, tanfovx, tanfovy, fx, fy, W, H, gx, gy, p, t, S, g)) break;
+            shade<DEG>(cam.c, p, shl, col, cl);
+            radius = g.rad;
+            xy = g.xy;
+            depth = t[2];
+            co = make_float4(g.conic[0], g.conic[1], g.conic[2], AA ? op * g.rho : op);
+        } while (false);
+        radii[i] = radius;
+        means2D[i] = xy;
+        depths[i] = depth;
+        conic_opacity[i] = co;
+#pragma unroll
+        for (int k = 0; k < 3; k++) {
+            rgb[3 * (size_t)i + k] = col[k];
+            clamped[3 * (size_t)i + k] = cl[k] ? 1 : 0;
+        }
+        TileRect rect{0u, 0u, 0ull};
+        if (radius > 0) {
+            int minx, miny, maxx, maxy;
+            if (gsr_k3_rect(xy, co, radius, gx, gy, 0, gy, minx, miny, maxx, maxy)) {
+                gsr_rect_pack(minx, miny, maxx, maxy, rect);
+                rec_n = (uint32_t)((maxx - minx) * (maxy - miny));
+            }
+        }
+        rec.tt[i] = gsr_tt_word(rec_n, rect, true);
+        rec.rects[i] = rect;
+        rec_key = __float_as_uint(depth);
+    }
+    k1_record_row(rec, rec_n, rec_key);
 }
 
 #ifndef GSR_K11_CAMQ
@@ -1977,16 +2092,54 @@
     if (!xyz || !scaling || !rotation || !features_dc || !features_rest || !opacity || !cams || !means2D || !depths ||
         !radii || !cov3D || !conic_opacity || !rgb || !clamped)
         return GSR_EINVAL;
+    return gsr_preprocess_forward_raw_batched_record(P, B, sh_degree, sh_coeffs, xyz, scaling, scale_modifier, rotation,
+                                                     features_dc, features_rest, opacity, cams, width, height, means2D,
+                                                     depths, radii, cov3D, conic_opacity, rgb, clamped, nullptr, nullptr,
+                                                     nullptr, 0, stream);
+}
+
+extern "C" int gsr_preprocess_forward_raw_batched_record(int P, int B, int sh_degree, int sh_coeffs, const float *xyz,
+                                                         const float *scaling, float scale_modifier,
+                                                         const float *rotation, const float *features_dc,
+                                                         const float *features_rest, const float *opacity,
+                                                         const float *cams, int width, int height, float *means2D,
+                                                         float *depths, int32_t *radii, float *cov3D,
+                                                         float *conic_opacity, float *rgb, uint8_t *clamped,
+                                                         void *record_rects, uint32_t *record_tt,
+                                                         uint32_t *record_rows, int record_rows_n,
+                                                         gsr_stream_t stream) {
+    if (P < 0 || B < 1 || sh_degree < 0 || sh_degree > 3 || sh_coeffs < 2 ||
+        sh_coeffs < (sh_degree + 1) * (sh_degree + 1) || width <= 0 || height <= 0)
+        return GSR_EINVAL;
+    const bool record = record_rects || record_tt || record_rows;
+    if (record && (!record_rects || !record_tt || !record_rows || B != 1 || record_rows_n != gsr_k1_record_rows(P) ||
+                   gsr_div_up(width, GSR_BLOCK_X) > 256 || gsr_div_up(height, GSR_BLOCK_Y) > 256))
+        return GSR_EINVAL;
+    if (P == 0) return 0;
+    if (!xyz || !scaling || !rotation || !features_dc || !features_rest || !opacity || !cams || !means2D || !depths ||
+        !radii || !cov3D || !conic_opacity || !rgb || !clamped)
+        return GSR_EINVAL;
     const dim3 grid(gsr_div_up(P, GSR_ONE_DIM_BLOCK)), block(GSR_ONE_DIM_BLOCK);
-    GSR_DISPATCH_DEG_AA(sh_degree, gsr_antialiasing_mode(),
-                     hipLaunchKernelGGL((preprocess_forward_batched_kernel<DEG, AA>), grid, block, 0,
-                                        reinterpret_cast<hipStream_t>(stream), P, B, sh_coeffs, xyz, scaling,
-                                        scale_modifier, rotation, features_dc, features_rest, opacity, cams, width,
-                                        height, reinterpret_cast<float2 *>(means2D), depths, radii, cov3D,
-                                        reinterpret_cast<float4 *>(conic_opacity), rgb, clamped));
+    const K1Record rec{reinterpret_cast<TileRect *>(record_rects), record_tt, reinterpret_cast<uint4 *>(record_rows)};
+    hipStream_t st = reinterpret_cast<hipStream_t>(stream);
+    if (record) {
+        GSR_DISPATCH_DEG_AA(sh_degree, gsr_antialiasing_mode(),
+                         hipLaunchKernelGGL((preprocess_forward_record_kernel<DEG, AA>), grid, block, 0, st, P, sh_coeffs,
+                                            xyz, scaling, scale_modifier, rotation, features_dc, features_rest, opacity,
+                                            cams, width, height, reinterpret_cast<float2 *>(means2D), depths, radii, cov3D,
+                                            reinterpret_cast<float4 *>(conic_opacity), rgb, clamped, rec));
+    } else {
+        GSR_DISPATCH_DEG_AA(sh_degree, gsr_antialiasing_mode(),
+                         hipLaunchKernelGGL((preprocess_forward_batched_kernel<DEG, AA>), grid, block, 0, st, P, B,
+                                            sh_coeffs, xyz, scaling, scale_modifier, rotation, features_dc, features_rest,
+                                            opacity, cams, width, height, reinterpret_cast<float2 *>(means2D), depths,
+                                            radii, cov3D, reinterpret_cast<float4 *>(conic_opacity), rgb, clamped));
+    }
     GSR_LAUNCH_CHECK();
     return 0;
 }
+
+extern "C" int gsr_k1_record_rows(int P) { return P > 0 ? gsr_div_up(P, GSR_ONE_DIM_BLOCK) : 0; }
 
 extern "C" int gsr_preprocess_backward_raw_batched(int P, int B, int sh_degree, int sh_coeffs, const float *xyz,
                                                    const float *scaling, float scale_modifier, const float *rotation,
diff --git a/grendel-gs_amd/csrc/tile_rect.h b/grendel-gs_amd/csrc/tile_rect.h
--- /dev/null
+++ b/grendel-gs_amd/csrc/tile_rect.h
@@ -0,0 +1,49 @@
+#pragma once
+#include "common.h"
+
+namespace {
+
+constexpr int TT_SHIFT = 20;
+constexpr uint32_t TT_MASK = (1u << TT_SHIFT) - 1u;
+
+struct alignas(16) TileRect {
+    uint32_t xs, ys;
+    unsigned long long mask;
+};
+static_assert(sizeof(TileRect) == 16, "one 16-byte gather");
+
+__device__ __forceinline__ bool gsr_k3_rect(const float2 xy, const float4 co, int rad, int gx, int gy, int hull0,
+                                            int hull1, int &minx, int &miny, int &maxx, int &maxy) {
+    float ex, ey;
+    if (!gsr_alpha_extent(co, ex, ey)) return false;
+    gsr_get_rect(xy.x, xy.y, rad, gx, gy, minx, miny, maxx, maxy);
+    miny = max(miny, hull0);
+    maxy = min(maxy, hull1);
+    gsr_narrow_span(xy.x, ex, minx, maxx);
+    gsr_narrow_span(xy.y, ey, miny, maxy);
+    return maxx > minx && maxy > miny;
+}
+
+__device__ __forceinline__ void gsr_rect_pack(int minx, int miny, int maxx, int maxy, TileRect &out) {
+    out.xs = (uint32_t)minx | ((uint32_t)maxx << 16);
+    out.ys = (uint32_t)miny | ((uint32_t)maxy << 16);
+    out.mask = ~0ull;
+}
+
+__device__ __forceinline__ uint32_t gsr_tt_word(uint32_t n, const TileRect &rect, bool yx) {
+    return (yx && n) ? (n | (((rect.ys >> 16) - (rect.ys & 0xFFFFu)) << TT_SHIFT)) : n;
+}
+
+__device__ __forceinline__ void gsr_rect_hist(int32_t (*dxy)[257], int minx, int miny, int maxx, int maxy) {
+    const int w = maxx - minx, h = maxy - miny;
+    atomicAdd(&dxy[0][minx], h);
+    atomicAdd(&dxy[0][maxx], -h);
+    atomicAdd(&dxy[1][miny], w);
+    atomicAdd(&dxy[1][maxy], -w);
+    atomicAdd(&dxy[2][miny], 1);
+    atomicAdd(&dxy[2][maxy], -1);
+}
+
+constexpr int K1_RECORD_ROW_WORDS = 4;
+
+}
diff --git a/grendel-gs_amd/diff_gaussian_rasterization/__init__.py b/grendel-gs_amd/diff_gaussian_rasterization/__init__.py
--- a/grendel-gs_amd/diff_gaussian_rasterization/__init__.py
+++ b/grendel-gs_amd/diff_gaussian_rasterization/__init__.py
@@ -760,6 +760,26 @@
     return d_xyz, d_scaling, d_rot, d_dc, d_rest, d_opac
 
 
+_K1_RECORD_KEY = "_gsr_k1_record"
+
+
+def _k1_record_buffers(cuda_args_list, B, P, width, height, dev):
+    if not cuda_args_list or len(cuda_args_list) != 1 or not isinstance(cuda_args_list[0], dict):
+        return None
+    ca = cuda_args_list[0]
+    if ca.get(_K1_RECORD_KEY) is not True:
+        ca.pop(_K1_RECORD_KEY, None)
+        return None
+    ca.pop(_K1_RECORD_KEY)
+    offs = (ctypes.c_size_t * 2)()
+    if B != 1 or P == 0 or _CAPTURE[0] is not None or lib.gsr_bin_record_offsets(P, width, height, offs) != 0:
+        return None
+    prep_bytes = lib.gsr_bin_prepare_bytes(P, width, height)
+    prep = torch.empty((max(prep_bytes, 4),), dtype=torch.uint8, device=dev)
+    rows = torch.empty((int(lib.gsr_k1_record_rows(P)), 4), dtype=torch.int32, device=dev)
+    return prep, rows, (int(offs[0]), int(offs[1]))
+
+
 class _PreprocessGaussiansRawBatched(torch.autograd.Function):
 
     @staticmethod
@@ -787,13 +807,24 @@
         conic_opacity = torch.empty((B, P, 4), dtype=torch.float32, device=dev)
         rgb = torch.empty((B, P, 3), dtype=torch.float32, device=dev)
         clamped = torch.empty((B, P, 3), dtype=torch.uint8, device=dev)
+        record = _k1_record_buffers(cuda_args_list, B, P, int(width), int(height), dev)
         with _on(dev), kernel_timer.range("preprocess_forward", N=P, B=B, M=M), \
                 zhx_range(cuda_args_list, "10 preprocess time"):
-            check(lib.gsr_preprocess_forward_raw_batched(
-                P, B, int(sh_degree), M, _ptr(xyz), _ptr(scaling), float(scale_modifier), _ptr(rotation),
-                _ptr(features_dc), _ptr(features_rest), _ptr(opacity), _ptr(cams), int(width), int(height),
-                _ptr(means2D), _ptr(depths), _ptr(radii), _ptr(cov3D), _ptr(conic_opacity), _ptr(rgb), _ptr(clamped),
-                _stream()), "gsr_preprocess_forward_raw_batched")
+            if record is not None:
+                prep, rows, offs = record
+                check(lib.gsr_preprocess_forward_raw_batched_record(
+                    P, B, int(sh_degree), M, _ptr(xyz), _ptr(scaling), float(scale_modifier), _ptr(rotation),
+                    _ptr(features_dc), _ptr(features_rest), _ptr(opacity), _ptr(cams), int(width), int(height),
+                    _ptr(means2D), _ptr(depths), _ptr(radii), _ptr(cov3D), _ptr(conic_opacity), _ptr(rgb),
+                    _ptr(clamped), prep.data_ptr() + offs[0], prep.data_ptr() + offs[1], _ptr(rows), rows.shape[0],
+                    _stream()), "gsr_preprocess_forward_raw_batched_record")
+                cuda_args_list[0][_K1_RECORD_KEY] = (prep, rows, P, int(width), int(height), means2D.data_ptr())
+            else:
+                check(lib.gsr_preprocess_forward_raw_batched(
+                    P, B, int(sh_degree), M, _ptr(xyz), _ptr(scaling), float(scale_modifier), _ptr(rotation),
+                    _ptr(features_dc), _ptr(features_rest), _ptr(opacity), _ptr(cams), int(width), int(height),
+                    _ptr(means2D), _ptr(depths), _ptr(radii), _ptr(cov3D), _ptr(conic_opacity), _ptr(rgb),
+                    _ptr(clamped), _stream()), "gsr_preprocess_forward_raw_batched")
         ctx.meta = (int(sh_degree), float(scale_modifier), int(width), int(height), M, aa)
         ctx.m2_ptr = means2D.data_ptr()
         ctx.save_for_backward(xyz, scaling, rotation, features_dc, features_rest, opacity, cams, radii, cov3D, clamped)
@@ -1021,13 +1052,14 @@
                   file=__import__("sys").stderr, flush=True)
 
 
-def _bin_workspaces(means2D, depths, radii, conic_opacity, compute_locally, width, height):
+def _bin_workspaces(means2D, depths, radii, conic_opacity, compute_locally, width, height, prep=None):
     P = means2D.shape[0]
     dev = means2D.device
     tiles = ((width + BLOCK_X - 1) // BLOCK_X) * ((height + BLOCK_Y - 1) // BLOCK_Y)
     ranges = torch.empty((tiles + 1, 2), dtype=torch.int32, device=dev)[:tiles]
     prep_bytes = lib.gsr_bin_prepare_bytes(P, width, height)
-    prep = torch.empty((max(prep_bytes, 4),), dtype=torch.uint8, device=dev)
+    if prep is None:
+        prep = torch.empty((max(prep_bytes, 4),), dtype=torch.uint8, device=dev)
     args = (P, width, height, _ptr(means2D), _ptr(depths), _ptr(radii), _ptr(conic_opacity), _ptr(compute_locally),
             _ptr(prep), prep_bytes)
     return P, dev, ranges, prep, args
@@ -1094,7 +1126,11 @@
 def bin_gaussians(means2D, depths, radii, conic_opacity, compute_locally, width, height, cuda_args=None, defer=False):
     if _CAPTURE[0] is not None:
         return _bin_gaussians_captured(_CAPTURE[0], means2D, depths, radii, conic_opacity, compute_locally, width, height)
-    P, dev, ranges, prep, args = _bin_workspaces(means2D, depths, radii, conic_opacity, compute_locally, width, height)
+    rec = cuda_args.pop(_K1_RECORD_KEY, None) if isinstance(cuda_args, dict) else None
+    if not (isinstance(rec, tuple) and rec[2:] == (means2D.shape[0], width, height, means2D.data_ptr())):
+        rec = None
+    P, dev, ranges, prep, args = _bin_workspaces(means2D, depths, radii, conic_opacity, compute_locally, width, height,
+                                                 prep=rec[0] if rec else None)
     if _DEBUG_RANGES:
         _debug_overlap("prep", prep)
         _debug_overlap("means2D", means2D)
@@ -1117,10 +1153,10 @@
                       "gsr_bin_sort_bounded")
             sorted_.value = 1
     else:
-        check(lib.gsr_bin_speculative_async(*args, cap if cap > 0 else 0, _ptr(kept) if cap > 0 else None,
-                                            kept.numel() if cap > 0 else 0, _ptr(point_list) if cap > 0 else None,
-                                            _ptr(ranges), ctypes.byref(ticket), ctypes.byref(sorted_), stream),
-              "gsr_bin_speculative_async")
+        check(lib.gsr_bin_speculative_record_async(
+            *args, cap if cap > 0 else 0, _ptr(kept) if cap > 0 else None, kept.numel() if cap > 0 else 0,
+            _ptr(point_list) if cap > 0 else None, _ptr(ranges), ctypes.byref(ticket), ctypes.byref(sorted_),
+            _ptr(rec[1]) if rec else None, rec[1].shape[0] if rec else 0, stream), "gsr_bin_speculative_record_async")
     pend = PendingPairs(ticket.value, bool(sorted_.value), cap, P, width, height, compute_locally, prep, ranges, dev,
                         current_stream(dev), key, cuda_args)
     if kernel_timer.enabled and ticket.value:
diff --git a/grendel-gs_amd/diff_gaussian_rasterization/_lib.py b/grendel-gs_amd/diff_gaussian_rasterization/_lib.py
--- a/grendel-gs_amd/diff_gaussian_rasterization/_lib.py
+++ b/grendel-gs_amd/diff_gaussian_rasterization/_lib.py
@@ -127,6 +127,15 @@
     "gsr_bin_speculative_async": (c_int, [c_int, c_int, c_int, c_void_p, c_void_p, c_void_p, c_void_p, c_void_p,
                                           c_void_p, c_size_t, c_int64, c_void_p, c_size_t, c_void_p, c_void_p,
                                           ctypes.POINTER(ctypes.c_uint32), ctypes.POINTER(c_int), c_void_p]),
+    "gsr_bin_speculative_record_async": (c_int, [c_int, c_int, c_int, c_void_p, c_void_p, c_void_p, c_void_p, c_void_p,
+                                                 c_void_p, c_size_t, c_int64, c_void_p, c_size_t, c_void_p, c_void_p,
+                                                 ctypes.POINTER(ctypes.c_uint32), ctypes.POINTER(c_int), c_void_p, c_int,
+                                                 c_void_p]),
+    "gsr_bin_record_offsets": (c_int, [c_int, c_int, c_int, ctypes.POINTER(c_size_t)]),
+    "gsr_k1_record_rows": (c_int, [c_int]),
+    "gsr_preprocess_forward_raw_batched_record": (c_int, [c_int, c_int, c_int, c_int, c_void_p, c_void_p, c_float] +
+                                                  [c_void_p] * 5 + [c_int, c_int] + [c_void_p] * 7 +
+                                                  [c_void_p, c_void_p, c_void_p, c_int, c_void_p]),
     "gsr_set_bin_persistent": (c_int, [c_int]),
     "gsr_set_tile_cull": (c_int, [c_int]),
     "gsr_set_bin_rowmajor": (c_int, [c_int]),
diff --git a/grendel-gs_amd/gaussian_renderer/__init__.py b/grendel-gs_amd/gaussian_renderer/__init__.py
--- a/grendel-gs_amd/gaussian_renderer/__init__.py
+++ b/grendel-gs_amd/gaussian_renderer/__init__.py
@@ -778,6 +778,9 @@
             if len(_CAMERA_BLOCKS) > 1024:
                 _CAMERA_BLOCKS.clear()
             _CAMERA_BLOCKS[skey] = (cams_block, tuple(packed), tuple(t._version for t in packed))
+    if len(cuda_args_list) == 1 and utils.DEFAULT_GROUP.size() == 1 and \
+            not (_EXCHANGE_OPTIONS["forced"] and dist.is_initialized()):
+        cuda_args_list[0][_dgr._K1_RECORD_KEY] = True
     m2_all, rgb_all, co_all, radii_all, depths_all = _dgr.preprocess_gaussians_raw_batched(
         *raw, cams_block, pc.active_sh_degree,
         scaling_modifier, rs0.image_width, rs0.image_height, tanfov0=(rs0.tanfovx, rs0.tanfovy),
@@ -908,6 +911,8 @@
             else:
                 rows_of = getattr(strategy, "_my_rows", None)
                 cuda_args["_gsr_band"] = rows_of() if rows_of is not None else None
+                if cuda_args["_gsr_band"] is not None and tuple(cuda_args["_gsr_band"]) != (0, utils.TILE_Y):
+                    cuda_args.pop(_dgr._K1_RECORD_KEY, None)
                 cuda_args["_gsr_pending"] = late
                 try:
                     image, _, _, _ = pkg["batched_rasterizers"][k].render_gaussians(
diff --git a/include/gsraster.h b/include/gsraster.h
--- a/include/gsraster.h
+++ b/include/gsraster.h
@@ -70,6 +70,12 @@
                               const int32_t *radii, const float *conic_opacity, const uint8_t *compute_locally, void *prep,
                               size_t prep_bytes, int64_t capacity, void *scratch, size_t scratch_bytes,
                               uint32_t *point_list, int32_t *ranges, uint32_t *ticket, int *sorted, gsr_stream_t stream);
+int gsr_bin_speculative_record_async(int P, int width, int height, const float *means2D, const float *depths,
+                                     const int32_t *radii, const float *conic_opacity, const uint8_t *compute_locally,
+                                     void *prep, size_t prep_bytes, int64_t capacity, void *scratch,
+                                     size_t scratch_bytes, uint32_t *point_list, int32_t *ranges, uint32_t *ticket,
+                                     int *sorted, const uint32_t *record_rows, int record_rows_n, gsr_stream_t stream);
+int gsr_bin_record_offsets(int P, int width, int height, size_t *offsets);
 int gsr_set_bin_persistent(int mode);
 int gsr_set_bin_rowmajor(int mode);
 int gsr_set_tile_cull(int mode);
@@ -311,6 +317,15 @@
                                        const float *cams, int width, int height, float *means2D, float *depths,
                                        int32_t *radii, float *cov3D, float *conic_opacity, float *rgb,
                                        uint8_t *clamped, gsr_stream_t stream);
+int gsr_preprocess_forward_raw_batched_record(int P, int B, int sh_degree, int sh_coeffs, const float *xyz,
+                                              const float *scaling, float scale_modifier, const float *rotation,
+                                              const float *features_dc, const float *features_rest,
+                                              const float *opacity, const float *cams, int width, int height,
+                                              float *means2D, float *depths, int32_t *radii, float *cov3D,
+                                              float *conic_opacity, float *rgb, uint8_t *clamped, void *record_rects,
+                                              uint32_t *record_tt, uint32_t *record_rows, int record_rows_n,
+                                              gsr_stream_t stream);
+int gsr_k1_record_rows(int P);
 int gsr_preprocess_backward_raw_batched(int P, int B, int sh_degree, int sh_coeffs, const float *xyz,
                                         const float *scaling, float scale_modifier, const float *rotation,
                                         const float *features_dc, const float *features_rest, const float *opacity,
```

Result: no change. 851.1 (median of 2 runs) (-0.1%).
